# collabora/WhisperLive

Hardware: AMD Instinct MI355X
Metric: real-time factor (xRT), Whisper-small 30 s window (p50 chunk latency in p50_chunk_latency_ms) (higher is better)
Workload: dtype f16 (MFMA operands; f32 accumulate, f32 residual stream, f32 log-mel); 1 GPU; configs[1]: Whisper-small.en, 1 stream per GPU, one 30 s window per stream per step (480000 samples 16 kHz f32 resident in HBM -> log-mel -> encoder -> beam-5 decode, 64 generated tokens forced by suppressing EOT), seeded random weights; streams_per_gpu=1, beam_size=5, decode_steps=64

## Files before the change

include/wlx.h:

```cpp
#ifndef WLX_H
#define WLX_H

#include <stdint.h>

#ifdef __cplusplus
extern "C" {
#endif

#define WLX_ABI_VERSION 1

typedef enum {
    WLX_OK = 0,
    WLX_ERR_ARG = 1,
    WLX_ERR_HIP = 2,
    WLX_ERR_WEIGHT = 3,
    WLX_ERR_STATE = 4,
    WLX_ERR_NOMEM = 5
} wlx_status;

typedef struct {
    int32_t n_mels;
    int32_t d_model;
    int32_t n_heads;
    int32_t enc_layers;
// ... 66 lines not shown

int32_t wlx_generate(wlx_engine* e, int32_t slot, int32_t batch,
                     const int32_t* prompts, const int32_t* prompt_lens, int32_t prompt_stride,
                     const wlx_gen_opts* opts,
                     int32_t* tokens_out, int32_t tokens_stride ,
                     int32_t* n_tokens_out, float* scores_out, float* no_speech_prob_out);

int32_t wlx_generate_ex(wlx_engine* e, int32_t slot, int32_t batch, const int32_t* enc_items,
                        const int32_t* prompts, const int32_t* prompt_lens, int32_t prompt_stride,
                        const wlx_gen_opts* opts,
                        int32_t* tokens_out, int32_t tokens_stride,
                        int32_t* n_tokens_out, float* scores_out, float* no_speech_prob_out);

int32_t wlx_detect_language(wlx_engine* e, int32_t slot, int32_t batch, int32_t sot,
                            const int32_t* lang_ids, int32_t n_lang, float* probs_out);

int32_t wlx_timings_get(wlx_engine* e, int32_t slot, wlx_timings* out);
int32_t wlx_sync(wlx_engine* e, int32_t slot);

int32_t wlx_align(wlx_engine* e, int32_t slot, int32_t item, const int32_t* tokens, int32_t n_tokens, int32_t n_sot,
                  int32_t num_frames, int32_t median_filter_width, const int32_t* heads, int32_t n_heads, int32_t eot,
                  int32_t* text_indices, int32_t* time_indices, int32_t path_cap, int32_t* n_path_out,
                  float* text_token_probs);

typedef struct wlx_vad wlx_vad;
typedef struct {
    const float* stft_basis;
    const float* enc_w[4];
    const float* enc_b[4];
    const float* lstm_w_ih;
    const float* lstm_w_hh;
    const float* lstm_b_ih;
    const float* lstm_b_hh;
    const float* out_w;
    const float* out_b;
} wlx_vad_weights;
int32_t wlx_vad_create(const wlx_vad_weights* w, int32_t device, wlx_vad** out);
void    wlx_vad_destroy(wlx_vad* v);
int32_t wlx_vad_probs(wlx_vad* v, const float* pcm, int64_t n, float* probs_out, int32_t cap,
                      int32_t* n_windows_out, float* device_ms_out);

typedef struct wlx_ring wlx_ring;
int32_t wlx_ring_create(wlx_engine* e, int64_t capacity_samples , wlx_ring** out);
void    wlx_ring_destroy(wlx_ring* r);
int32_t wlx_ring_append(wlx_ring* r, const float* samples, int64_t n, int64_t max_resident, int64_t trim,
                        int64_t* dropped_out, int64_t* base_out, int64_t* resident_out);
int32_t wlx_ring_state(wlx_ring* r, int64_t* base_out, int64_t* resident_out);
int32_t wlx_vad_probs_resident(wlx_vad* v, wlx_ring* r, int64_t start, int64_t n, int32_t extra_zero_windows,
                               float* probs_out, int32_t cap, int32_t* n_windows_out, float* device_ms_out);
int32_t wlx_vad_segments(const float* probs, int32_t n_windows, int64_t n_samples, double thr, double neg, double min_speech,
                         double pad, double max_speech, double min_silence, double min_silence_at_max,
                         int64_t* start_end_out, int32_t cap, int32_t* n_out);
int32_t wlx_logmel_ring(wlx_engine* e, int32_t slot, int32_t item, wlx_ring* r, const int64_t* ranges, int32_t n_ranges,
                        int32_t* n_frames_out);

typedef struct {
    int32_t d_model, n_heads, enc_layers, dec_layers, ffn, vocab;
    int32_t max_positions;
    int32_t pad_id, eos_id, decoder_start_id;
    int32_t scale_embedding;
} wlx_mt_spec;
typedef struct wlx_mt wlx_mt;
typedef struct {
    int32_t num_beams;
    int32_t max_length;
    int32_t early_stopping;
    float   length_penalty;
    int32_t no_repeat_ngram_size;
    int32_t forced_eos_token_id;
} wlx_mt_gen_opts;
int32_t wlx_mt_create(const wlx_mt_spec* spec, const wlx_tensor* weights, int32_t n_weights, int32_t device, wlx_mt** out);
void    wlx_mt_destroy(wlx_mt* mt);
int32_t wlx_mt_slot_create(wlx_mt* mt, int32_t max_batch, int32_t max_rows_per_item, int32_t max_src, int32_t* slot_out);
int32_t wlx_mt_slot_destroy(wlx_mt* mt, int32_t slot);
int32_t wlx_mt_translate(wlx_mt* mt, int32_t slot, int32_t batch, const int32_t* src_ids, const int32_t* src_lens,
                         int32_t src_stride, const wlx_mt_gen_opts* opts, int32_t* tokens_out, int32_t tokens_stride,
                         int32_t* n_tokens_out, float* scores_out);

int32_t wlx_debug_logits_get(wlx_engine* e, int32_t slot, float* out, int32_t rows, int64_t cap_floats);
int32_t wlx_debug_decode_logits(wlx_engine* e, int32_t slot, const int32_t* tokens, int32_t n, float* out);
int32_t wlx_debug_search(wlx_engine* e, int32_t slot, const float* logits, int32_t steps,
                         const int32_t* prompt, int32_t prompt_len, const wlx_gen_opts* opts,
                         int32_t* tokens_out, int32_t tokens_stride, int32_t* n_tokens_out, float* scores_out);
int32_t wlx_debug_time_decode_step(wlx_engine* e, int32_t slot, int32_t rows, int32_t t, int32_t iters,
                                   float* avg_ms_out);

typedef struct {
    char name[64];
    float launches_per_step, avg_us, total_us_per_step;
    double bytes_per_launch;
} wlx_kernel_stat;
int32_t wlx_debug_trace_step(wlx_engine* e, int32_t slot, int32_t rows, int32_t t, int32_t with_search,
                             uint64_t* out, int64_t cap_u64, char* names, int32_t* n_launches_out);

int32_t wlx_debug_profile_step(wlx_engine* e, int32_t slot, int32_t rows, int32_t t, int32_t iters,
                               wlx_kernel_stat* out, int32_t cap, int32_t* n_out);

int32_t wlx_mt_debug_encode(wlx_mt* mt, int32_t slot, int32_t batch, const int32_t* src_ids, const int32_t* src_lens,
                            int32_t src_stride, float* out, int64_t cap_floats);
int32_t wlx_mt_debug_decode_logits(wlx_mt* mt, int32_t slot, const int32_t* src_ids, int32_t src_len, const int32_t* dec_tokens,
                                   int32_t n, float* out);
int32_t wlx_mt_debug_timings(wlx_mt* mt, int32_t slot, float* encode_ms, float* decode_ms, int32_t* steps);
int32_t wlx_mt_debug_attn(int32_t device, const uint16_t* q, int64_t ldq, int64_t q_rows, const uint16_t* k, int64_t ldk,
                          const uint16_t* v, int64_t ldv, int64_t kv_rows, const int32_t* groups, int32_t n_groups, int32_t max_nq,
                          int32_t heads, const int32_t* anc, int32_t ld_anc, int32_t tmax, uint16_t* o, int64_t ldo, int64_t o_rows);
int32_t wlx_mt_debug_topk(int32_t device, const float* logits, int32_t rows, int32_t vocab, const int32_t* ban, const int32_t* nban,
                          int32_t ban_ld, int32_t k, float* out_val, int32_t* out_idx);
int32_t wlx_mt_debug_embed(int32_t device, const float* E, int32_t vocab, int32_t d, const int32_t* tok, const int32_t* pos,
                           int32_t rows, float scale, const float* sinpos, int32_t n_pos, float* x);

int32_t wlx_debug_layernorm(int32_t device, const float* x, int64_t ldx, const float* gamma, const float* beta, int32_t M, int32_t d,
                            uint16_t* out16, float* out32, int64_t ldo);
int32_t wlx_debug_attn_encoder(int32_t device, const uint16_t* q, int64_t ldq, int64_t isq, const uint16_t* k, int64_t ldk, int64_t isk,
                               const uint16_t* vt, int64_t ldvt, int64_t isv, uint16_t* o, int64_t ldo, int64_t iso, int32_t T,
                               int32_t H, int32_t items);
typedef struct {
    int32_t zbatch, M, N, K, KT, conv3_cin, mode, force_form;
    int32_t d, rows_per_item;
    float qscale;
    int32_t reserved;
    int64_t lda, strideA, a_len;
    int64_t ldc, strideC, c_len;
    int64_t ldx, strideX, x_len;
    int64_t ldk, kv_item_stride_k, kv_layer_stride_k, k_len;
    int64_t ldvt, kv_item_stride_v, kv_layer_stride_v, v_len;
} wlx_debug_gemm_args;
int32_t wlx_debug_gemm(int32_t device, const wlx_debug_gemm_args* a, const uint16_t* A, const float* W, const float* bias,
                       const float* pos, uint16_t* C, float* X, uint16_t* kout, uint16_t* vt, int32_t* ran_out);
int32_t wlx_debug_dec_cross_attn(int32_t device, const uint16_t* q, int64_t ldq, const uint16_t* kp, const uint16_t* vp,
                                 int64_t item_stride, int32_t n_items, int32_t H, int32_t R, int32_t groups, int32_t rows,
                                 const int32_t* group_item, uint16_t* part_o, float* part_ml, uint16_t* out, int64_t ldo,
                                 int32_t align_item, int32_t align_head, float* align_out);
int32_t wlx_debug_dec_self_attn(int32_t device, const uint16_t* q, int64_t ldq, const uint16_t* kc, const uint16_t* vc,
                                int64_t cache_row_stride, int32_t cache_rows, int32_t d, int32_t H, int32_t rows, const int32_t* pos,
                                const int32_t* ancrow, const int16_t* anc, int32_t ident_ancestry, uint16_t* out, int64_t ldo);

#ifdef __cplusplus
}
#endif
#endif
```

whisperlive_amd/_lib.py:

```python
from __future__ import annotations

import ctypes as C
import os
import shutil
import subprocess
from pathlib import Path

import numpy as np

PKG_DIR = Path(__file__).resolve().parent
CSRC = PKG_DIR / "csrc"
DEFAULT_LIB = PKG_DIR / "libwlx.so"
LIB_PATH = Path(os.environ["WLX_LIB"]).resolve() if os.environ.get("WLX_LIB") else DEFAULT_LIB
SOURCES = ["pack.hip", "logmel.hip", "gemm.hip", "attention.hip", "decoder.hip", "search.hip", "host.hip", "engine.hip", "vad.hip", "mt.hip", "mt_engine.hip", "kernel_hooks.hip"]
EXPORTS = [
    "wlx_abi_version", "wlx_last_error", "wlx_engine_create", "wlx_engine_destroy", "wlx_engine_spec",
    "wlx_slot_create", "wlx_slot_destroy", "wlx_logmel", "wlx_pcm_put", "wlx_logmel_resident", "wlx_features_get", "wlx_features_set", "wlx_encode",
    "wlx_encoder_output_get", "wlx_generate", "wlx_generate_ex", "wlx_detect_language", "wlx_align", "wlx_timings_get", "wlx_sync",
    "wlx_vad_create", "wlx_vad_destroy", "wlx_vad_probs",
    "wlx_ring_create", "wlx_ring_destroy", "wlx_ring_append", "wlx_ring_state", "wlx_vad_probs_resident", "wlx_vad_segments", "wlx_logmel_ring",
    "wlx_mt_create", "wlx_mt_destroy", "wlx_mt_slot_create", "wlx_mt_slot_destroy", "wlx_mt_translate",
    "wlx_debug_logits_get", "wlx_debug_decode_logits", "wlx_debug_search", "wlx_debug_time_decode_step", "wlx_debug_profile_step", "wlx_debug_trace_step",
    "wlx_mt_debug_encode", "wlx_mt_debug_decode_logits", "wlx_mt_debug_timings", "wlx_mt_debug_attn", "wlx_mt_debug_topk",
    "wlx_mt_debug_embed",
    "wlx_debug_layernorm", "wlx_debug_attn_encoder", "wlx_debug_dec_cross_attn", "wlx_debug_dec_self_attn", "wlx_debug_gemm",
]


HIPCC_EXTRA = ["-mllvm", "-amdgpu-mfma-vgpr-form=1"]


class WlxError(RuntimeError):
    pass


class wlx_spec(C.Structure):
    _fields_ = [(n, C.c_int32) for n in
                ("n_mels", "d_model", "n_heads", "enc_layers", "dec_layers", "ffn", "vocab", "n_audio_ctx", "n_text_ctx")]


class wlx_tensor(C.Structure):
    _fields_ = [("name", C.c_char_p), ("data", C.c_void_p), ("ndim", C.c_int32), ("shape", C.c_int64 * 4),
                ("on_device", C.c_int32)]


class wlx_token_ids(C.Structure):
    _fields_ = [(n, C.c_int32) for n in ("sot", "eot", "no_timestamps", "timestamp_begin", "no_speech", "blank")]


class wlx_gen_opts(C.Structure):
    _fields_ = [
        ("beam_size", C.c_int32), ("patience", C.c_float), ("num_hypotheses", C.c_int32),
        ("length_penalty", C.c_float), ("repetition_penalty", C.c_float), ("no_repeat_ngram_size", C.c_int32),
        ("max_length", C.c_int32), ("suppress_blank", C.c_int32), ("suppress_tokens", C.POINTER(C.c_int32)),
        ("n_suppress_tokens", C.c_int32), ("max_initial_timestamp_index", C.c_int32), ("sampling_topk", C.c_int32),
        ("sampling_temperature", C.c_float), ("seed", C.c_uint64), ("ids", wlx_token_ids),
    ]


class wlx_timings(C.Structure):
    _fields_ = [("logmel_ms", C.c_float), ("encode_ms", C.c_float), ("generate_ms", C.c_float), ("decode_steps", C.c_int32)]


class wlx_kernel_stat(C.Structure):
    _fields_ = [("name", C.c_char * 64), ("launches_per_step", C.c_float), ("avg_us", C.c_float),
                ("total_us_per_step", C.c_float), ("bytes_per_launch", C.c_double)]


class wlx_vad_weights(C.Structure):
    _fields_ = [("stft_basis", C.POINTER(C.c_float)), ("enc_w", C.POINTER(C.c_float) * 4), ("enc_b", C.POINTER(C.c_float) * 4),
                ("lstm_w_ih", C.POINTER(C.c_float)), ("lstm_w_hh", C.POINTER(C.c_float)), ("lstm_b_ih", C.POINTER(C.c_float)),
                ("lstm_b_hh", C.POINTER(C.c_float)), ("out_w", C.POINTER(C.c_float)), ("out_b", C.POINTER(C.c_float))]


class wlx_mt_spec(C.Structure):
    _fields_ = [(n, C.c_int32) for n in ("d_model", "n_heads", "enc_layers", "dec_layers", "ffn", "vocab", "max_positions",
                                         "pad_id", "eos_id", "decoder_start_id", "scale_embedding")]


class wlx_debug_gemm_args(C.Structure):
    _fields_ = ([(n, C.c_int32) for n in ("zbatch", "M", "N", "K", "KT", "conv3_cin", "mode", "force_form", "d", "rows_per_item")] +
                [("qscale", C.c_float), ("reserved", C.c_int32)] +
                [(n, C.c_int64) for n in ("lda", "strideA", "a_len", "ldc", "strideC", "c_len", "ldx", "strideX", "x_len",
                                          "ldk", "kv_item_stride_k", "kv_layer_stride_k", "k_len",
                                          "ldvt", "kv_item_stride_v", "kv_layer_stride_v", "v_len")])


class wlx_mt_gen_opts(C.Structure):
    _fields_ = [("num_beams", C.c_int32), ("max_length", C.c_int32), ("early_stopping", C.c_int32),
                ("length_penalty", C.c_float), ("no_repeat_ngram_size", C.c_int32), ("forced_eos_token_id", C.c_int32)]


_extra_ok = None


def _hipcc() -> str:
    hipcc = shutil.which("hipcc") or "/opt/rocm/bin/hipcc"
    if not os.path.exists(hipcc):
        raise WlxError("hipcc not found: cannot build libwlx.so (ROCm toolchain required)")
    return hipcc


def _compile(out: Path, defines=(), verbose: bool = False, force: bool = False) -> Path:
    global _extra_ok
    from concurrent.futures import ThreadPoolExecutor
# ... 54 lines not shown
    deps = [CSRC / s for s in SOURCES] + list(CSRC.glob("*.h")) + [PKG_DIR.parent / "include" / "wlx.h"]
    return out.exists() and all(out.stat().st_mtime >= d.stat().st_mtime for d in deps)


def build_trace() -> Path:
    out = PKG_DIR / "libwlx_trace.so"
    return out if _fresh(out) else _compile(out, ["WLX_TRACE"])


def build_ab() -> Path:
    out = PKG_DIR / "libwlx_ab.so"
    return out if _fresh(out) else _compile(out, ["WLX_AB"])


def build_variant(name: str, defines) -> Path:
    out = PKG_DIR / name
    return out if _fresh(out) else _compile(out, list(defines))


def build(force: bool = False, verbose: bool = False) -> Path:
    if not force and _fresh(DEFAULT_LIB):
        return DEFAULT_LIB
    return _compile(DEFAULT_LIB, (), verbose, force=force)


_lib = None


def load() -> C.CDLL:
    global _lib
    if _lib is not None:
        return _lib
    if not LIB_PATH.exists():
        raise WlxError(f"{LIB_PATH} not built: run `python -c 'import __graft_entry__ as g; g.build()'` "
                       "(hipcc --offload-arch=gfx950). whisperlive_amd has no CPU fallback.")
    try:
        lib = C.CDLL(str(LIB_PATH))
    except OSError as e:
        raise WlxError(f"cannot load {LIB_PATH}: {e}") from e
    missing = [s for s in EXPORTS if not hasattr(lib, s)]
    if missing:
        raise WlxError(f"libwlx.so lacks symbols {missing}")
    i32, i64, f32p, i32p, vp = C.c_int32, C.c_int64, C.POINTER(C.c_float), C.POINTER(C.c_int32), C.c_void_p
    lib.wlx_abi_version.restype = i32
    lib.wlx_last_error.restype = C.c_char_p
    lib.wlx_engine_create.argtypes = [C.POINTER(wlx_spec), C.POINTER(wlx_tensor), i32, i32, C.POINTER(vp)]
    lib.wlx_engine_destroy.argtypes = [vp]
    lib.wlx_engine_destroy.restype = None
    lib.wlx_engine_spec.argtypes = [vp, C.POINTER(wlx_spec)]
    lib.wlx_slot_create.argtypes = [vp, i32, i32, i32p]
    lib.wlx_slot_destroy.argtypes = [vp, i32]
    lib.wlx_logmel.argtypes = [vp, i32, i32, f32p, i64, i32p]
    lib.wlx_pcm_put.argtypes = [vp, i32, i32, f32p, i64]
    lib.wlx_logmel_resident.argtypes = [vp, i32, i32, i32p]
    lib.wlx_features_get.argtypes = [vp, i32, i32, f32p, i64, i32p]
    lib.wlx_features_set.argtypes = [vp, i32, i32, f32p, i32, i32]
    lib.wlx_encode.argtypes = [vp, i32, i32, i32p, i32p]
    lib.wlx_encoder_output_get.argtypes = [vp, i32, i32, f32p, i64]
    lib.wlx_generate.argtypes = [vp, i32, i32, i32p, i32p, i32, C.POINTER(wlx_gen_opts), i32p, i32, i32p, f32p, f32p]
    lib.wlx_generate_ex.argtypes = [vp, i32, i32, i32p, i32p, i32p, i32, C.POINTER(wlx_gen_opts), i32p, i32, i32p, f32p, f32p]
    lib.wlx_detect_language.argtypes = [vp, i32, i32, i32, i32p, i32, f32p]
    lib.wlx_align.argtypes = [vp, i32, i32, i32p, i32, i32, i32, i32, i32p, i32, i32, i32p, i32p, i32, i32p, f32p]
    lib.wlx_timings_get.argtypes = [vp, i32, C.POINTER(wlx_timings)]
    lib.wlx_sync.argtypes = [vp, i32]
    lib.wlx_vad_create.argtypes = [C.POINTER(wlx_vad_weights), i32, C.POINTER(vp)]
    lib.wlx_vad_destroy.argtypes = [vp]
    lib.wlx_vad_destroy.restype = None
    lib.wlx_vad_probs.argtypes = [vp, f32p, i64, f32p, i32, i32p, f32p]
    i64p = C.POINTER(C.c_int64)
    lib.wlx_ring_create.argtypes = [vp, i64, C.POINTER(vp)]
    lib.wlx_ring_destroy.argtypes = [vp]
    lib.wlx_ring_destroy.restype = None
    lib.wlx_ring_append.argtypes = [vp, f32p, i64, i64, i64, i64p, i64p, i64p]
    lib.wlx_ring_state.argtypes = [vp, i64p, i64p]
    lib.wlx_vad_probs_resident.argtypes = [vp, vp, i64, i64, i32, f32p, i32, i32p, f32p]
    lib.wlx_vad_segments.argtypes = [f32p, i32, i64, C.c_double, C.c_double, C.c_double, C.c_double, C.c_double, C.c_double, C.c_double, i64p, i32, i32p]
    lib.wlx_logmel_ring.argtypes = [vp, i32, i32, vp, i64p, i32, i32p]
    lib.wlx_debug_logits_get.argtypes = [vp, i32, f32p, i32, i64]
    lib.wlx_debug_decode_logits.argtypes = [vp, i32, i32p, i32, f32p]
    lib.wlx_debug_search.argtypes = [vp, i32, f32p, i32, i32p, i32, C.POINTER(wlx_gen_opts), i32p, i32, i32p, f32p]
    lib.wlx_debug_time_decode_step.argtypes = [vp, i32, i32, i32, i32, f32p]
    lib.wlx_debug_profile_step.argtypes = [vp, i32, i32, i32, i32, C.POINTER(wlx_kernel_stat), i32, i32p]
    lib.wlx_debug_trace_step.argtypes = [vp, i32, i32, i32, i32, C.POINTER(C.c_uint64), i64, C.c_char_p, i32p]
    lib.wlx_mt_create.argtypes = [C.POINTER(wlx_mt_spec), C.POINTER(wlx_tensor), i32, i32, C.POINTER(vp)]
    lib.wlx_mt_destroy.argtypes = [vp]
    lib.wlx_mt_destroy.restype = None
    lib.wlx_mt_slot_create.argtypes = [vp, i32, i32, i32, i32p]
    lib.wlx_mt_slot_destroy.argtypes = [vp, i32]
    lib.wlx_mt_translate.argtypes = [vp, i32, i32, i32p, i32p, i32, C.POINTER(wlx_mt_gen_opts), i32p, i32, i32p, f32p]
    lib.wlx_mt_debug_encode.argtypes = [vp, i32, i32, i32p, i32p, i32, f32p, i64]
    lib.wlx_mt_debug_decode_logits.argtypes = [vp, i32, i32p, i32, i32p, i32, f32p]
    lib.wlx_mt_debug_timings.argtypes = [vp, i32, f32p, f32p, i32p]
    u16p = C.POINTER(C.c_uint16)
    lib.wlx_mt_debug_attn.argtypes = [i32, u16p, i64, i64, u16p, i64, u16p, i64, i64, i32p, i32, i32, i32, i32p, i32, i32, u16p, i64, i64]
    lib.wlx_mt_debug_topk.argtypes = [i32, f32p, i32, i32, i32p, i32p, i32, i32, f32p, i32p]
    lib.wlx_mt_debug_embed.argtypes = [i32, f32p, i32, i32, i32p, i32p, i32, C.c_float, f32p, i32, f32p]
    lib.wlx_debug_layernorm.argtypes = [i32, f32p, i64, f32p, f32p, i32, i32, u16p, f32p, i64]
    lib.wlx_debug_attn_encoder.argtypes = [i32, u16p, i64, i64, u16p, i64, i64, u16p, i64, i64, u16p, i64, i64, i32, i32, i32]
    lib.wlx_debug_dec_cross_attn.argtypes = [i32, u16p, i64, u16p, u16p, i64, i32, i32, i32, i32, i32, i32p, u16p, f32p, u16p, i64,
                                             i32, i32, f32p]
    lib.wlx_debug_dec_self_attn.argtypes = [i32, u16p, i64, u16p, u16p, i64, i32, i32, i32, i32, i32p, i32p, C.POINTER(C.c_int16), i32,
                                            u16p, i64]
    lib.wlx_debug_gemm.argtypes = [i32, C.POINTER(wlx_debug_gemm_args), u16p, f32p, f32p, f32p, u16p, f32p, u16p, u16p, i32p]
    for name in EXPORTS:
        fn = getattr(lib, name)
        if name not in ("wlx_last_error", "wlx_engine_destroy", "wlx_vad_destroy", "wlx_ring_destroy", "wlx_mt_destroy"):
            fn.restype = i32
    if lib.wlx_abi_version() != 1:
        raise WlxError("libwlx.so ABI version mismatch")
    _lib = lib
    return lib


def tensor_array(weights):
    keep = []
    arr = (wlx_tensor * len(weights))()
    for i, (name, t) in enumerate(weights.items()):
        on_dev = 0
        if hasattr(t, "data_ptr"):
            import torch
            t = t.detach().to(torch.float32).contiguous()
            on_dev = 1 if t.is_cuda else 0
            ptr, shape = t.data_ptr(), tuple(t.shape)
        else:
            t = np.ascontiguousarray(t, dtype=np.float32)
            ptr, shape = t.ctypes.data, t.shape
        keep.append(t)
        arr[i].name = name.encode()
        arr[i].data = ptr
        arr[i].ndim = len(shape)
        for j, s in enumerate(shape):
            arr[i].shape[j] = s
        arr[i].on_device = on_dev
    return arr, keep


def check(rc: int):
    if rc != 0:
        msg = load().wlx_last_error()
        raise WlxError(f"libwlx error {rc}: {msg.decode() if msg else '?'}")
```

whisperlive_amd/csrc/decoder.h:

```cpp
#pragma once
#include "kernels.h"

namespace wlx {

#define WLX_MAX_MT 4
#define WLX_MAX_DEC_ROWS 320
#define WLX_XSPLIT 8
#define WLX_MAX_CAND 32
#define WLX_MAX_HYP 32

struct RowTables {
    const int* token; const int* pos; const int* cache; const int* ancrow;
    const short* anc;
    int* intok;
};

void launch_dec_embed(const half_t* tok_emb, const float* pos_emb, int d, const RowTables& rt, int rows,
                      float* x, const int* done, hipStream_t s);

enum GemvIn : int { GEMV_IN_LN = 0, GEMV_IN_F16 = 1, GEMV_IN_XATTN = 2 };
enum GemvOut : int { GEMV_OUT_F16 = 0, GEMV_OUT_GELU_F16 = 1, GEMV_OUT_F32 = 2, GEMV_OUT_RESID = 3, GEMV_OUT_QKV = 4,
                     GEMV_OUT_SLAB = 5 };
enum GemvXsrc : int { GEMV_X_PLAIN = 0, GEMV_X_SLABS = 1, GEMV_X_EMBED = 2 };
#ifndef WLX_CQ_GB_LDS
#define WLX_CQ_GB_LDS 1
#endif
#ifndef WLX_CQ_SWAP
#define WLX_CQ_SWAP 1
#endif
#ifndef WLX_STAGE_WAVE
#define WLX_STAGE_WAVE 1
#endif
#ifndef WLX_XCOMB_WAVE
#define WLX_XCOMB_WAVE 1
#endif
#ifndef WLX_FC2_KS
#define WLX_FC2_KS 2
#endif

struct GemvParams {
    int in_mode, out_mode;
    int M;
    int Mtot;
    int chunk;
    int busy_device;
    int rt_nz, rt_tiles, rt_magic;
    int K, KT, N;
    int KTW;
    int NCH;
    int nwm;
    int xstage;
    const half_t* Wp; const float* bias;
    const float* X; long ldx; const float* gamma; const float* beta;
    const half_t* Xh; long ldxh;
    const half_t* part_o; const float* part_ml; int H; int R;
    half_t* Yh; long ldyh;
    float* Y; long ldy;
    float* Xres; long ldxres;
    int d; float qscale; half_t* Kc; half_t* Vc; long cache_row_stride;
    const int* row_cache; const int* row_pos;
    const int* done;
    int xsrc;
    float* slab; long slab_stride;
    int KTS;
    const half_t* tok_emb; const float* pos_emb; const int* emb_token; int* intok;
    WLX_TR_FIELD
};
#ifdef WLX_TRACE
extern unsigned long long* g_trace_buf;
extern int g_trace_seq;
extern const char* g_trace_names[512];
static inline WlxTrace trace_next(const char* name) {
    WlxTrace t{g_trace_buf, g_trace_seq};
    if (g_trace_seq < 512) g_trace_names[g_trace_seq] = name;
    ++g_trace_seq;
    return t;
}
#define WLX_TR_ARG(name) , trace_next(name)
#else
#define WLX_TR_ARG(name)
#endif
void launch_dec_gemv(const GemvParams& p, hipStream_t s);
const char* dec_gemv_kernel_name(const GemvParams& p);
extern bool g_decode_v1;
bool dec_gemv_is_lean(const GemvParams& p);
int dec_gemv_slab_split(int M, int K, int N);

void launch_dec_self_attn(const half_t* q, long ldq, const half_t* Kc, const half_t* Vc, long cache_row_stride,
                          int d, int H, const RowTables& rt, int rows, half_t* out, long ldo,
                          const int* done, bool ident_ancestry, hipStream_t s);
void launch_dec_cross_attn(const half_t* q, long ldq, const half_t* Kp, const half_t* Vp, long item_stride, int H, int R,
                           int groups, int rows, const int* group_item, half_t* part_o, float* part_ml, hipStream_t s);

bool dec_cq_cross_attn_eligible(int d, int H, int R);
void launch_dec_cq_cross_attn(const float* X, long ldx, const float* gamma, const float* beta, const half_t* Wp, const float* bias,
                              float qscale, int d, const half_t* Kp, const half_t* Vp, long item_stride, int H, int R, int groups,
                              int rows, const int* group_item, half_t* part_o, float* part_ml, hipStream_t s);
void launch_dec_xattn_combine(const half_t* part_o, const float* part_ml, int M, int H, int R, half_t* out, long ldo, hipStream_t s);
void launch_dec_align_scores(const half_t* q, long ldq, const half_t* Kp_item, int h, int rows, float* out, hipStream_t s);

struct SearchState {
    int* step;
    int* done;
    int* done_host;
    int* n_finished;
    int* item_done;
    int* plen;
    float* cum;
    int* row_done;
    float* cand_score; int* cand_tok;
    int* samp_tok; float* samp_lp;
    int* hyp_tokens;
    int* hyp_len;
    float* hyp_score;
    int* n_hyp;
    int* n_hyp_host;
    float* no_speech;
    int* nsp_row;
    int* token; int* pos; short* anc; int* intok;
    float* scan_stats;
    float* scan_cv; int* scan_ci;
    int* rule;
};
#define SC_THREADS 256
#define SC_NPT 8
#define SC_CHUNK (SC_THREADS * SC_NPT)
#define SC_MAXCH 27
#define SC_NSTAT 8
struct SearchParams {
    int V; long ldl;
    int items, R, rows;
    int sampling;
    int beam, ncand, max_cand_hyp , num_hyp;
    int allow_early_exit;
    float length_penalty, rep_penalty, temperature;
    int no_repeat_ngram, topk;
    int suppress_blank, apply_ts_rules, max_initial_ts;
    int sot, eot, no_timestamps, ts_begin, no_speech, blank;
    int max_length;
    unsigned long long seed;
    const unsigned* suppress_mask;
};
void launch_search_rows(const float* logits, const SearchParams* sp_dev, int rows, const SearchState& st, hipStream_t s);
void launch_search_update(const SearchParams* sp_dev, int items, const SearchState& st, hipStream_t s);
void launch_search_scan3(const float* logits, long ldl, int V, const SearchParams* sp_dev, int rows, const SearchState& st,
                         hipStream_t s);
void launch_search_merge_update3(const float* logits, long ldl, int V, const SearchParams* sp_dev, int items, int R,
                                 const SearchState& st, hipStream_t s);
void launch_search_reset(const SearchState& st, int items, int rows, hipStream_t s);
void launch_token_prob_rows(const float* logits, long ldl, int vlim, int rows, const int* toks, float* out, hipStream_t s);
void launch_token_prob(const float* logits, long ldl, int V, int rows, int tok, float* out, hipStream_t s);
void launch_lang_probs(const float* logits, long ldl, int rows, const int* ids, int n, float* probs, hipStream_t s);

}
```

whisperlive_amd/csrc/decoder.hip:

```cpp
#include "decoder.h"
#include <algorithm>
#include <cstdlib>
#include <cstdio>
#include <atomic>

namespace wlx {

__global__ __launch_bounds__(256) void dec_embed_kernel(const half_t* __restrict__ tok_emb,
                                                        const float* __restrict__ pos_emb, int d,
                                                        const int* __restrict__ token,
                                                        const int* __restrict__ pos,
                                                        const int* __restrict__ cache, int* __restrict__ intok,
                                                        float* __restrict__ x, const int* __restrict__ done WLX_TR_PARAM) {
    if (done && *done) return;
    WLX_TR_BEGIN();
    const int r = blockIdx.x;
    const int tok = token[r], p = pos[r];
    if (threadIdx.x == 0) intok[(long)cache[r] * WLX_T_TEXT + p] = tok;
    const half_t* te = tok_emb + (long)tok * d;
    const float* pe = pos_emb + (long)p * d;
    for (int i = threadIdx.x * 4; i < d; i += 256 * 4) {
        f16x4 t = ld_f16x4(te + i);
        float4 pv = *reinterpret_cast<const float4*>(pe + i);
        *reinterpret_cast<float4*>(x + (long)r * d + i) =
// ... 1151 lines not shown
}
static bool gemv2_ok(const GemvParams& p, Gemv2Cfg* out) {
    const Gemv2Cfg c = gemv2_cfg(p);
    if (!c.ok) return false;
    if (p.in_mode == GEMV_IN_LN && p.xsrc != GEMV_X_PLAIN) {
        const bool pair = (c.CH == 4 && c.LNV == 3) || (c.CH == 3 && c.LNV == 3) || (c.CH == 2 && c.LNV == 2) || (c.CH == 4 && c.LNV == 4) || (c.CH == 5 && c.LNV == 5) ||
                          (c.MT == 1 && ((c.CH == 6 && c.LNV == 3) || (c.CH == 8 && c.LNV == 4) || (c.CH == 10 && c.LNV == 5))) ||
                          (c.CH == 2 && c.LNV == 15 && c.MT == 1);
        if (!pair) return false;
    } else if (p.in_mode == GEMV_IN_LN) {
        const bool pair = (c.CH == 6 && c.LNV == 3) || (c.CH == 5 && c.LNV == 5) || (c.CH == 4 && c.LNV == 2) || (c.CH == 4 && c.LNV == 4) ||
                          (c.CH == 10 && c.LNV == 5 && c.MT == 1) || (c.CH == 8 && c.LNV == 4 && c.MT == 1) ||
                          (c.CH == 2 && c.LNV == 15 && c.MT == 1);
        if (!pair) return false;
    }
    if (out) *out = c;
    return true;
}
static GemvParams gemv_chunked(const GemvParams& p) {
    static const bool rt_on = [] { const char* e = wlx_ab("WLX_ROWTILE"); return !(e && e[0] == '0'); }();
    constexpr int rt_max = WLX_MAX_DEC_ROWS;
    static const int rt_chunk_env = [] { const char* e = wlx_ab("WLX_ROWTILE_CHUNK"); const int v = e ? atoi(e) : 0; return (v == 16 || v == 32 || v == 48) ? v : 0; }();
    int rt_chunk = 16;
    if (p.in_mode == GEMV_IN_F16 && p.out_mode == GEMV_OUT_RESID && p.xsrc == GEMV_X_PLAIN && !p.busy_device && p.M > 64) {
        static const int n_cu = [] { int dev = 0, n = 256; (void)hipGetDevice(&dev); hipDeviceProp_t pr; if (hipGetDeviceProperties(&pr, dev) == hipSuccess && pr.multiProcessorCount > 0) n = pr.multiProcessorCount; return n; }();
        const int tiles = (p.N + 15) / 16;
        double best = 1e300;
        for (int mt = 1; mt <= 3; ++mt) {
            const long wgs = (long)tiles * ((p.M + 16 * mt - 1) / (16 * mt));
            const double cost = (double)((wgs + n_cu - 1) / n_cu) * (1.0 + 0.35 * (mt - 1));
            if (cost < best - 1e-9) { best = cost; rt_chunk = 16 * mt; }
        }
    }
    if (rt_chunk_env) rt_chunk = rt_chunk_env;
    GemvParams q = p;
    if (p.Mtot != 0 || p.in_mode == GEMV_IN_XATTN) return q;
    const bool ln_wide4 = rt_chunk == 16 && p.M > 32 && p.in_mode == GEMV_IN_LN && p.xsrc == GEMV_X_PLAIN && (p.out_mode == GEMV_OUT_QKV || p.out_mode == GEMV_OUT_GELU_F16) &&
                          (p.N & 15) == 0 && ((p.N >> 4) & 3) == 0;
    const bool rt_shape = p.N <= 1536 || (long)p.N * p.K <= 3200000L || ln_wide4;
    if (rt_on && !g_decode_v1 && p.M > rt_chunk && p.M <= rt_max && rt_shape) { q.Mtot = p.M; q.M = rt_chunk; q.chunk = rt_chunk; q.rt_nz = (p.M + rt_chunk - 1) / rt_chunk; }
    else if (p.M > 48 && p.xsrc != GEMV_X_EMBED) { q.Mtot = p.M; q.M = 48; q.chunk = 48; }
    return q;
}
static bool vocab2_ok(const GemvParams& p);
bool dec_gemv_is_lean(const GemvParams& p) { return vocab2_ok(p) || gemv2_ok(gemv_chunked(p), nullptr); }

int dec_gemv_slab_split(int M, int K, int N) {
    if (WLX_FC2_KS < 2) return 0;
    if (g_decode_v1 || M < 1 || K % 32 || (K / 32) % WLX_FC2_KS || K < 2048) return 0;
    GemvParams p0{};
    p0.in_mode = GEMV_IN_F16; p0.out_mode = GEMV_OUT_SLAB; p0.M = M; p0.K = K; p0.KT = K / 32; p0.N = N; p0.KTS = p0.KT / WLX_FC2_KS;
    static const float dummy_bias = 0.f;
    p0.bias = &dummy_bias;
    const GemvParams p = gemv_chunked(p0);
    Gemv2Cfg c;
    if (!gemv2_ok(p, &c) || (p.M <= 16 && !c.xstage)) return 0;
    return WLX_FC2_KS;
}

static bool vocab2_ok(const GemvParams& p);
static int vocab2_chunk_rows(int K);
const char* dec_gemv_kernel_name(const GemvParams& p_any) {
    static thread_local char buf[64];
    if (vocab2_ok(p_any)) {
        snprintf(buf, sizeof(buf), "dec_vocab_kernel<%d, %d, %d>", p_any.KT, p_any.KT == 24 ? 6 : p_any.KT == 40 ? 5 : p_any.KT == 12 ? 3 : 4, (std::min(p_any.M, vocab2_chunk_rows(p_any.K)) + 15) / 16);
        return buf;
    }
    const GemvParams p = gemv_chunked(p_any);
    const int MT = (p.M + 15) / 16;
    Gemv2Cfg c2;
    if (gemv2_ok(p, &c2)) {
        snprintf(buf, sizeof(buf), "dec_gemv2_kernel<%d, %d, %d, %d, %d, %d, %d>", c2.CH, c2.LNV ? c2.LNV : 1, p.in_mode, p.out_mode, c2.NTB, c2.MT, p.xsrc);
        return buf;
    }
    snprintf(buf, sizeof(buf), "dec_gemv_kernel<%d, %d, %d>", MT > 4 ? 4 : MT, MT == 1 ? 2 : 1, p.in_mode);
    return buf;
}

struct VocabParams {
    const float* X; long ldx; const float* gamma; const float* beta;
    const half_t* Wp; int M, N, NT;
    float* Y; long ldy;
    const float* slab; long slab_stride;
    WLX_TR_FIELD
};
template <int KT, int KC, int MT, bool SLABS>
__global__ __launch_bounds__(512) void dec_vocab_kernel(VocabParams p) {
    static_assert(!SLABS || MT == 1, "slab rows: decode steps of one row tile");
    constexpr int K = KT * 32, LNV = (K + 255) / 256, NC = KT / KC, LDXS = K + 8;
    constexpr bool LNT = (K % 256) != 0;
    static_assert((K % 256 == 0 || K == 384) && KT % KC == 0 && NC % 2 == 0, "d_model a multiple of 256 (or 384); an even number of K chunks");
    constexpr int RPT = (MT == 1) ? 2 : 4;
    constexpr int NTRIP = (MT * 16 + 8 * RPT - 1) / (8 * RPT);
    extern __shared__ __attribute__((aligned(16))) half_t vxs[];
    const int tid = threadIdx.x, lane = tid & 63, c = lane & 15, g = lane >> 4;
    const int wave = __builtin_amdgcn_readfirstlane(tid >> 6);
    WLX_TR_BEGIN();
    const int pair = blockIdx.x * 8 + wave;
    const int t0 = (2 * pair < p.NT) ? 2 * pair : p.NT - 1, t1 = (2 * pair + 1 < p.NT) ? 2 * pair + 1 : p.NT - 1;
    const bool tail_on = !LNT || lane < 32;
    const int tback = LNT ? (tail_on ? 0 : lane) : 0;
    float4 x[RPT][LNV];
#pragma unroll
    for (int i = 0; i < RPT; ++i) {
        const int r = (wave + 8 * i < p.M) ? wave + 8 * i : p.M - 1;
        const float4* x4 = reinterpret_cast<const float4*>(p.X + (long)r * p.ldx) + lane;
#pragma unroll
        for (int j = 0; j < LNV; ++j) x[i][j] = x4[64 * j - ((j == LNV - 1) ? tback : 0)];
    }
    float4 xsl[SLABS ? WLX_FC2_KS : 1][RPT][LNV];
    if constexpr (SLABS) {
#pragma unroll
        for (int q = 0; q < WLX_FC2_KS; ++q)
#pragma unroll
            for (int i = 0; i < RPT; ++i) {
                const int r = (wave + 8 * i < p.M) ? wave + 8 * i : p.M - 1;
                const float4* s4 = reinterpret_cast<const float4*>(p.slab + q * p.slab_stride + (long)r * p.ldx) + lane;
#pragma unroll
                for (int j = 0; j < LNV; ++j) xsl[q][i][j] = s4[64 * j - ((j == LNV - 1) ? tback : 0)];
            }
    }
    float4 gq[LNV], bq[LNV];
    {
        const float4* g4 = reinterpret_cast<const float4*>(p.gamma) + lane;
        const float4* b4 = reinterpret_cast<const float4*>(p.beta) + lane;
#pragma unroll
        for (int j = 0; j < LNV; ++j) { const int tb = (j == LNV - 1) ? tback : 0; gq[j] = g4[64 * j - tb]; bq[j] = b4[64 * j - tb]; }
    }
    asm volatile("" ::: "memory");
    const half_t* wq[2] = {p.Wp + (long)t0 * KT * 512 + lane * 8, p.Wp + (long)t1 * KT * 512 + lane * 8};
    f16x8 wf[2][KC][2];
#pragma unroll
    for (int b = 0; b < 2; ++b)
#pragma unroll
        for (int j = 0; j < KC; ++j)
#pragma unroll
            for (int i = 0; i < 2; ++i) wf[b][j][i] = ld_nt_f16x8(wq[i] + (b * KC + j) * 512);
    constexpr float invK = 1.0f / (float)K;
    auto ln_row = [&](float4 (&xr)[LNV], int r, bool keep) {
        if constexpr (LNT) { if (!tail_on) xr[LNV - 1] = make_float4(0.f, 0.f, 0.f, 0.f); }
        float sm = 0.f;
#pragma unroll
        for (int j = 0; j < LNV; ++j) sm += (xr[j].x + xr[j].y) + (xr[j].z + xr[j].w);
        const float mean = dpp_wave_sum(sm) * invK;
        float q = 0.f;
#pragma unroll
        for (int j = 0; j < LNV; ++j) {
            xr[j].x -= mean; xr[j].y -= mean; xr[j].z -= mean; xr[j].w -= mean;
            if constexpr (LNT) { if (j == LNV - 1 && !tail_on) xr[j] = make_float4(0.f, 0.f, 0.f, 0.f); }
            q += (xr[j].x * xr[j].x + xr[j].y * xr[j].y) + (xr[j].z * xr[j].z + xr[j].w * xr[j].w);
        }
        const float rstd = rsqrtf(dpp_wave_sum(q) * invK + 1e-5f);
        half_t* dst = vxs + (long)r * LDXS + lane * 4;
#pragma unroll
        for (int j = 0; j < LNV; ++j) {
            const f16x4 hv = {(half_t)(xr[j].x * rstd * gq[j].x + bq[j].x), (half_t)(xr[j].y * rstd * gq[j].y + bq[j].y),
                              (half_t)(xr[j].z * rstd * gq[j].z + bq[j].z), (half_t)(xr[j].w * rstd * gq[j].w + bq[j].w)};
            if (keep && (j < LNV - 1 || tail_on)) *reinterpret_cast<f16x4*>(dst + 256 * j) = hv;
        }
    };
    if constexpr (SLABS) {
#pragma unroll
        for (int q = 0; q < WLX_FC2_KS; ++q)
#pragma unroll
            for (int i = 0; i < RPT; ++i)
#pragma unroll
                for (int j = 0; j < LNV; ++j) { x[i][j].x += xsl[q][i][j].x; x[i][j].y += xsl[q][i][j].y; x[i][j].z += xsl[q][i][j].z; x[i][j].w += xsl[q][i][j].w; }
    }
#pragma unroll
    for (int i = 0; i < RPT; ++i) ln_row(x[i], (wave + 8 * i < p.M) ? wave + 8 * i : p.M - 1, wave + 8 * i < p.M);
#pragma unroll 1
    for (int tr = 1; tr < NTRIP; ++tr) {
        const int rb = wave + 8 * RPT * tr;
        if (rb >= p.M) break;
        float4 y[RPT][LNV];
#pragma unroll
        for (int i = 0; i < RPT; ++i) {
            const int r = (rb + 8 * i < p.M) ? rb + 8 * i : p.M - 1;
            const float4* x4 = reinterpret_cast<const float4*>(p.X + (long)r * p.ldx) + lane;
#pragma unroll
            for (int j = 0; j < LNV; ++j) y[i][j] = x4[64 * j - ((j == LNV - 1) ? tback : 0)];
        }
#pragma unroll
        for (int i = 0; i < RPT; ++i) ln_row(y[i], (rb + 8 * i < p.M) ? rb + 8 * i : p.M - 1, rb + 8 * i < p.M);
    }
    WLX_TR_MARK(1);
    __syncthreads();
    const half_t* xr[MT];
#pragma unroll
    for (int mt = 0; mt < MT; ++mt) xr[mt] = vxs + (long)((mt * 16 + c < p.M) ? mt * 16 + c : p.M - 1) * LDXS + g * 8;
    f32x4 acc[2][MT];
#pragma unroll
    for (int i = 0; i < 2; ++i)
#pragma unroll
        for (int mt = 0; mt < MT; ++mt) acc[i][mt] = (f32x4){0.f, 0.f, 0.f, 0.f};
#pragma unroll
    for (int ch = 0; ch < NC; ++ch) {
#pragma unroll
        for (int j = 0; j < KC; ++j) {
            f16x8 xf[MT];
#pragma unroll
            for (int mt = 0; mt < MT; ++mt) xf[mt] = *reinterpret_cast<const f16x8*>(xr[mt] + (ch * KC + j) * 32);
#pragma unroll
            for (int i = 0; i < 2; ++i)
#pragma unroll
                for (int mt = 0; mt < MT; ++mt) acc[i][mt] = mfma16(wf[ch & 1][j][i], xf[mt], acc[i][mt]);
        }
        if (ch + 2 < NC) {
#pragma unroll
            for (int j = 0; j < KC; ++j)
#pragma unroll
                for (int i = 0; i < 2; ++i) wf[ch & 1][j][i] = ld_nt_f16x8(wq[i] + ((ch + 2) * KC + j) * 512);
        }
    }
    WLX_TR_MARK(2);
#pragma unroll
    for (int i = 0; i < 2; ++i) {
        const int nt = 2 * pair + i;
        if (nt >= p.NT) continue;
        const int n = nt * 16 + g * 4;
#pragma unroll
        for (int mt = 0; mt < MT; ++mt) {
            const int row = mt * 16 + c;
            if (row >= p.M) continue;
            float* yp = p.Y + (long)row * p.ldy + n;
            const f32x4 v = acc[i][mt];
            if (n + 3 < p.N) *reinterpret_cast<float4*>(yp) = make_float4(v[0], v[1], v[2], v[3]);
            else { if (n < p.N) yp[0] = v[0]; if (n + 1 < p.N) yp[1] = v[1]; if (n + 2 < p.N) yp[2] = v[2]; }
        }
    }
    WLX_TR_END(p.trc);
}

template <int KT, int KC, int MT, bool SLABS = false>
static void vocab_go(const VocabParams& p, hipStream_t s) {
    const size_t shm = (size_t)p.M * (KT * 32 + 8) * sizeof(half_t);
    if (shm > 64 * 1024) {
        static std::atomic<signed char> granted[64] = {};
        int dev = 0;
        (void)hipGetDevice(&dev);
        if (dev >= 0 && dev < 64 && granted[dev].load(std::memory_order_acquire) == 0) {
            if (hipFuncSetAttribute(reinterpret_cast<const void*>(&dec_vocab_kernel<KT, KC, MT, SLABS>), hipFuncAttributeMaxDynamicSharedMemorySize,
                                    WLX_G2_LDS_MAX) == hipSuccess) granted[dev].store(1, std::memory_order_release);
            else {
                (void)hipGetLastError();
                g_lds_optin_refused.store(true);
                fprintf(stderr, "[wlx] device %d refused %d KiB of dynamic LDS: the batched vocabulary projection falls back to the general kernel\n", dev, WLX_G2_LDS_MAX / 1024);
            }
        }
    }
    const int pairs = (p.NT + 1) / 2;
    hipLaunchKernelGGL((dec_vocab_kernel<KT, KC, MT, SLABS>), dim3((pairs + 7) / 8), dim3(512), shm, s, p);
}
template <int KT, int KC>
static void vocab_go_mt(const VocabParams& p, hipStream_t s) {
    if (p.slab) { vocab_go<KT, KC, 1, true>(p, s); return; }
    switch ((p.M + 15) / 16) {
        case 1: vocab_go<KT, KC, 1>(p, s); break;
        case 2: vocab_go<KT, KC, 2>(p, s); break;
        case 3: vocab_go<KT, KC, 3>(p, s); break;
        default: vocab_go<KT, KC, 4>(p, s); break;
    }
}
static int vocab2_chunk_rows(int K) {
    int r = 64;
    while (r > 16 && (size_t)r * (K + 8) * sizeof(half_t) > WLX_G2_LDS_MAX) r -= 16;
    return r;
}
static bool vocab2_ok(const GemvParams& p) {
    if (g_decode_v1 || p.in_mode != GEMV_IN_LN || p.out_mode != GEMV_OUT_F32 || p.bias || p.Mtot != 0) return false;
    if (p.xsrc != GEMV_X_PLAIN && !(p.xsrc == GEMV_X_SLABS && p.M <= 16 && p.slab != nullptr)) return false;
    if (p.M < 1 || p.M > WLX_MAX_DEC_ROWS || p.K != p.KT * 32 || p.N < 256) return false;
    if (!(p.KT == 12 || p.KT == 16 || p.KT == 24 || p.KT == 32 || p.KT == 40)) return false;
    const int rows = std::min(p.M, vocab2_chunk_rows(p.K));
    const size_t shm = (size_t)rows * (p.K + 8) * sizeof(half_t);
    if (shm > 64 * 1024 && g_lds_optin_refused.load(std::memory_order_relaxed)) return false;
    return shm <= WLX_G2_LDS_MAX;
}
static void vocab2_launch(const GemvParams& g, hipStream_t s) {
    const int CH = vocab2_chunk_rows(g.K);
    for (int r0 = 0; r0 < g.M; r0 += CH) {
        VocabParams p{};
        p.X = g.X + (long)r0 * g.ldx; p.ldx = g.ldx; p.gamma = g.gamma; p.beta = g.beta; p.Wp = g.Wp; p.M = std::min(CH, g.M - r0); p.N = g.N; p.NT = (g.N + 15) / 16;
        p.Y = g.Y + (long)r0 * g.ldy; p.ldy = g.ldy;
        if (g.xsrc == GEMV_X_SLABS) { p.slab = g.slab; p.slab_stride = g.slab_stride; }
#ifdef WLX_TRACE
        p.trc = trace_next("vocab2");
#endif
        switch (g.KT) {
            case 12: vocab_go_mt<12, 3>(p, s); break;
            case 16: vocab_go_mt<16, 4>(p, s); break;
            case 24: vocab_go_mt<24, 6>(p, s); break;
            case 32: vocab_go_mt<32, 4>(p, s); break;
            default: vocab_go_mt<40, 5>(p, s); break;
        }
    }
}

template <int MT, int NTB>
static void gemv_dispatch_in(const GemvParams& p, dim3 grid, dim3 block, size_t shm, hipStream_t s) {
    switch (p.in_mode) {
        case GEMV_IN_LN: hipLaunchKernelGGL((dec_gemv_kernel<MT, NTB, GEMV_IN_LN>), grid, block, shm, s, p); break;
        case GEMV_IN_F16: hipLaunchKernelGGL((dec_gemv_kernel<MT, NTB, GEMV_IN_F16>), grid, block, shm, s, p); break;
        default: hipLaunchKernelGGL((dec_gemv_kernel<MT, NTB, GEMV_IN_XATTN>), grid, block, shm, s, p); break;
    }
}

void launch_dec_gemv(const GemvParams& p_any, hipStream_t s) {
    if (vocab2_ok(p_any)) { vocab2_launch(p_any, s); return; }
    Gemv2Cfg c2;
    const GemvParams pc = gemv_chunked(p_any);
    if (gemv2_ok(pc, &c2) && gemv2_launch(pc, c2, s)) return;
    if (p_any.M > 16 * WLX_MAX_MT) {
        const int CHK = (p_any.in_mode == GEMV_IN_XATTN && p_any.R > 0) ? (16 * WLX_MAX_MT / p_any.R) * p_any.R : 16 * WLX_MAX_MT;
        for (int r0 = 0; r0 < p_any.M; r0 += CHK) {
            GemvParams q = p_any;
            q.M = std::min(CHK, p_any.M - r0);
            if (q.X) q.X += (long)r0 * q.ldx;
            if (q.Xh) q.Xh += (long)r0 * q.ldxh;
            if (q.Yh) q.Yh += (long)r0 * q.ldyh;
            if (q.Y) q.Y += (long)r0 * q.ldy;
            if (q.Xres) q.Xres += (long)r0 * q.ldxres;
            if (q.row_cache) q.row_cache += r0;
            if (q.row_pos) q.row_pos += r0;
            if (q.in_mode == GEMV_IN_XATTN) {
                const int items0 = r0 / q.R;
                q.part_o += (long)items0 * q.H * WLX_XSPLIT * 16 * 64;
                q.part_ml += (long)items0 * q.H * 16 * WLX_XSPLIT * 2;
            }
            launch_dec_gemv(q, s);
        }
        return;
    }
    const GemvParams& p0 = p_any;
    const GemvParams& p = p0;
    const int MT = (p.M + 15) / 16;
    const int NT_total = (p.N + 15) / 16;
    int nw = (p.KT + GV_CH - 1) / GV_CH;
    if (nw < 1) nw = 1;
    if (nw > 8) nw = 8;
    const int NTB = (MT == 1) ? 2 : 1;
    dim3 grid((NT_total + NTB - 1) / NTB), block(nw * 64);
    const size_t shm = sizeof(float) * ((size_t)2 * nw * MT * 16 + (size_t)nw * NTB * MT * 256);
    switch (MT) {
        case 1: gemv_dispatch_in<1, 2>(p, grid, block, shm, s); break;
        case 2: gemv_dispatch_in<2, 1>(p, grid, block, shm, s); break;
        case 3: gemv_dispatch_in<3, 1>(p, grid, block, shm, s); break;
        default: gemv_dispatch_in<4, 1>(p, grid, block, shm, s); break;
    }
}

#define SA_PF_NW 4
#ifndef SA_NW
#define SA_NW 8
#endif
template <bool IDENT, int NW>
__global__ __launch_bounds__(64 * NW) void dec_self_attn2_kernel(const half_t* __restrict__ q, long ldq,
                                                                    const half_t* __restrict__ Kc,
                                                                    const half_t* __restrict__ Vc, long crs, int d,
                                                                    const int* __restrict__ pos,
                                                                    const int* __restrict__ ancrow,
                                                                    const short* __restrict__ anc,
                                                                    half_t* __restrict__ out, long ldo WLX_TR_PARAM) {
    __shared__ int crow_s[NW][64];
    __shared__ float part_s[NW][8][64];
    __shared__ float ml_s[NW][2];
    const int lane = threadIdx.x & 63;
    const int w = __builtin_amdgcn_readfirstlane(threadIdx.x >> 6);
// ... 507 lines not shown
```

whisperlive_amd/csrc/engine.h:

```cpp
#pragma once
#include <hip/hip_runtime.h>
#include <map>
#include <mutex>
#include <string>
#include <vector>
#include "../../include/wlx.h"
#include "decoder.h"
#include "host.h"

namespace wlx {

struct StepGraphKey {
    int rows, R, groups;
    bool operator<(const StepGraphKey& o) const {
        if (rows != o.rows) return rows < o.rows;
        if (R != o.R) return R < o.R;
        return groups < o.groups;
    }
};

struct ProfRec { std::string name; double bytes; };
struct Prof { std::vector<ProfRec> recs; bool list_only = true; std::string only; int t = 0; };

struct Slot {
    std::mutex call_mu;
    int B = 0, R = 0, rows_cap = 0, cache_rows = 0, groups_cap = 0;
    hipStream_t stream = nullptr;
    bool dedicated_queue = false;
    int device_of = -1;
    bool counted = false;
    unsigned promote_epoch = 0;
    hipEvent_t ev0 = nullptr, ev1 = nullptr;
    hipEvent_t ev_lm0 = nullptr, ev_lm1 = nullptr;
    hipEvent_t ev_en0 = nullptr, ev_en1 = nullptr;
    bool en_pending = false;
    bool lm_pending = false;
    bool gen_pending = false;
    std::vector<int> lm_items;
    bool busy_variant = false;
    std::vector<void*> allocs, host_allocs;
    float* pcm = nullptr; size_t pcm_cap = 0;
    float* feats = nullptr; long feat_ld = 0;
    std::vector<int> nframes;
    std::vector<int64_t> npcm;
    unsigned* gmax = nullptr;
    long long* d_rng = nullptr;
    half_t *featT = nullptr, *h1 = nullptr, *ln = nullptr, *q = nullptr, *k = nullptr, *vt = nullptr,
           *attn = nullptr, *h2 = nullptr, *enc16 = nullptr;
    float *x = nullptr, *enc32 = nullptr;
    long featT_stride = 0, h1_stride = 0;
    half_t *ck = nullptr, *cvt = nullptr;
    int enc_batch = 0;
    half_t *kc = nullptr, *vc = nullptr;
    float* xd = nullptr; half_t *qd = nullptr, *attnd = nullptr, *hd = nullptr;
    float* slab = nullptr;
    half_t* part_o = nullptr;
    float *part_ml = nullptr, *logits = nullptr;
    long ldl = 0;
    int *d_token = nullptr, *d_pos = nullptr, *d_cache = nullptr, *d_ancrow = nullptr, *d_group_item = nullptr;
    struct DecBufs {
        float* xd; half_t *qd, *attnd, *hd; float* slab; int slab_rows; half_t* part_o; float* part_ml;
        int *d_token, *d_pos, *d_cache, *d_ancrow, *d_group_item;
    };
    DecBufs pf{};
    bool pf_one_pass = false;
    bool pf_ok = false;
    short* d_anc = nullptr; int* d_intok = nullptr;
    bool anc_ident = false;
    SearchState st{};
    SearchParams* d_sp = nullptr;
    unsigned* d_suppress = nullptr;
    int* d_lang_ids = nullptr; float* d_probs = nullptr; float* d_tokprob = nullptr;
    int* h_stage = nullptr; size_t h_stage_ints = 0;
    unsigned char* h_gen = nullptr; size_t h_gen_bytes = 0;
    int* h_pf = nullptr; bool h_pf_used = false;
    int* h_hyp = nullptr;
    int max_items = 0;
    std::vector<int> last_suppress; bool suppress_valid = false;
    std::map<StepGraphKey, hipGraphExec_t> graphs;
    wlx_timings tm{};
    Prof* prof = nullptr;
    struct AlignCapture { float* scores; const int32_t* heads; int n_heads, n_tok, row0, item; }* align = nullptr;
    float* align_scores = nullptr; size_t align_cap = 0;
    int* d_align_tgt = nullptr; float* d_align_prob = nullptr;
};

struct Ring {
    std::mutex mu;
    int device = 0;
    float* buf = nullptr; size_t cap = 0;
    int64_t base = 0, resident = 0;
    hipStream_t stream = nullptr;
    hipEvent_t last_read = nullptr; bool read_pending = false; hipStream_t last_read_stream = nullptr;
};

struct Engine {
    wlx_spec spec{};
    int device = 0;
    int H = 0;
    std::vector<void*> allocs;
    LogmelConsts lm{};
    half_t *conv1_w = nullptr, *conv2_w = nullptr;
    float *conv1_b = nullptr, *conv2_b = nullptr, *enc_pos = nullptr, *enc_ln_g = nullptr, *enc_ln_b = nullptr;
    int conv1_KT = 0;
    std::vector<LayerW> enc;
    half_t* Wckv = nullptr; float* bckv = nullptr;
    half_t *tok_emb16 = nullptr, *Wvocab = nullptr;
    float *dec_pos = nullptr, *dec_ln_g = nullptr, *dec_ln_b = nullptr;
    std::vector<LayerW> dec;
    std::mutex mu;
    std::vector<Slot*> slots;
    bool use_graph = true;
};

}

struct wlx_engine : public wlx::Engine {};
struct wlx_ring : public wlx::Ring {};
```

whisperlive_amd/csrc/engine.hip:

```cpp
#include "engine.h"
#include <sched.h>
#include <atomic>
#include <limits>
#include <algorithm>
#include <cmath>
#include <cstdio>
#include <cstdlib>
#include <cstring>
#include <chrono>
#include <thread>

using namespace wlx;

static inline void cpu_relax() {
#if defined(__x86_64__) || defined(__i386__)
    __builtin_ia32_pause();
#elif defined(__aarch64__)
    asm volatile("yield" ::: "memory");
#else
    asm volatile("" ::: "memory");
#endif
}
extern "C" int32_t wlx_abi_version(void) { return WLX_ABI_VERSION; }

static void build_mel_filters(int n_mels, std::vector<float>& w, std::vector<int>& range) {
    const int nb = 201;
    std::vector<double> fft(nb), melf(n_mels + 2);
    for (int i = 0; i < nb; ++i) fft[i] = (double)i * 8000.0 / 200.0;
    const double max_mel = 45.245640471924965, f_sp = 200.0 / 3.0, min_log_hz = 1000.0;
    const double min_log_mel = min_log_hz / f_sp, logstep = std::log(6.4) / 27.0;
    const double step = max_mel / (double)(n_mels + 1);
    for (int i = 0; i < n_mels + 2; ++i) {
        double m = (i == n_mels + 1) ? max_mel : (double)i * step;
        melf[i] = (m >= min_log_mel) ? min_log_hz * std::exp(logstep * (m - min_log_mel)) : f_sp * m;
    }
    w.assign((size_t)n_mels * nb, 0.f);
    range.assign((size_t)n_mels * 2, 0);
    for (int i = 0; i < n_mels; ++i) {
        const double fd0 = melf[i + 1] - melf[i], fd1 = melf[i + 2] - melf[i + 1];
        const double enorm = 2.0 / (melf[i + 2] - melf[i]);
        int lo = nb, hi = 0;
        for (int b = 0; b < nb; ++b) {
            const double lower = -(melf[i] - fft[b]) / fd0, upper = (melf[i + 2] - fft[b]) / fd1;
            const double v = std::max(0.0, std::min(lower, upper));
            const float f = (float)((double)(float)v * enorm);
            w[(size_t)i * nb + b] = f;
            if (f != 0.f) { lo = std::min(lo, b); hi = std::max(hi, b + 1); }
        }
        if (lo >= hi) { lo = 0; hi = 0; }
        range[2 * i] = lo; range[2 * i + 1] = hi;
    }
}

static int build_logmel_consts(Engine* e) {
    std::vector<float> win(400), tw(800), filt;
    std::vector<int> range;
    const double PI2 = 6.283185307179586476925286766559;
    for (int i = 0; i < 400; ++i) {
        win[i] = (float)(0.5 - 0.5 * std::cos(PI2 * (double)i / 400.0));
        tw[2 * i] = (float)std::cos(PI2 * (double)i / 400.0);
        tw[2 * i + 1] = (float)std::sin(PI2 * (double)i / 400.0);
    }
    build_mel_filters(e->spec.n_mels, filt, range);
    float *dwin, *dtw, *dfilt; int* drange;
    CKR(dalloc(e->allocs, &dwin, 400, true)); CKR(dalloc(e->allocs, &dtw, 800, true));
    CKR(dalloc(e->allocs, &dfilt, filt.size(), true)); CKR(dalloc(e->allocs, &drange, range.size(), true));
    CKR(upload_sync(dwin, win.data(), 400 * 4));
    CKR(upload_sync(dtw, tw.data(), 800 * 4));
    CKR(upload_sync(dfilt, filt.data(), filt.size() * 4));
    CKR(upload_sync(drange, range.data(), range.size() * 4));
    e->lm.window = dwin; e->lm.twiddle = dtw; e->lm.filters = dfilt; e->lm.frange = drange;
    return WLX_OK;
}

static int engine_load(Engine* e, const wlx_tensor* weights, int n_weights) {
    const wlx_spec& sp = e->spec;
    const int d = sp.d_model, F = sp.ffn, V = sp.vocab;
    std::vector<void*>& A = e->allocs;
    Weights ws;
    CKR(ws.open(weights, n_weights));
    CKR(build_logmel_consts(e));
    const wlx_tensor* t; const float* src;
    auto conv = [&](const char* name, int cin, half_t** W, int* KT) -> int {
        CKR(ws.need(name, {d, cin, 3}, &t));
        CKR(alloc_packed(A, d, 3 * cin, W, KT, true));
        CKR(ws.device_f32(t, &src));
        launch_pack_conv3(src, d, cin, *W, *KT, ws.st);
        return WLX_OK;
    };
    auto positions = [&](const char* name, int rows, float** out) -> int {
        CKR(ws.need(name, {rows, d}, &t));
        CKR(dalloc(A, out, (size_t)rows * d, true));
        CKR(ws.device_f32(t, &src));
        CK(hipMemcpyAsync(*out, src, (size_t)rows * d * 4, hipMemcpyDeviceToDevice, ws.st));
        return WLX_OK;
    };
    int KT;
    CKR(conv("model.encoder.conv1.weight", sp.n_mels, &e->conv1_w, &e->conv1_KT));
    CKR(conv("model.encoder.conv2.weight", d, &e->conv2_w, &KT));
    CKR(ws.alloc_vec(A, "model.encoder.conv1.bias", d, &e->conv1_b, true));
    CKR(ws.alloc_vec(A, "model.encoder.conv2.bias", d, &e->conv2_b, true));
    CKR(positions("model.encoder.embed_positions.weight", sp.n_audio_ctx, &e->enc_pos));
    LayerOpts o{false, 1.f, true};
    e->enc.resize(sp.enc_layers);
    for (int l = 0; l < sp.enc_layers; ++l)
        CKR(load_layer(ws, A, "model.encoder.layers." + std::to_string(l) + ".", d, F, o, e->enc[l]));
    CKR(ws.alloc_vec(A, "model.encoder.layer_norm.weight", d, &e->enc_ln_g, true));
    CKR(ws.alloc_vec(A, "model.encoder.layer_norm.bias", d, &e->enc_ln_b, true));
    CKR(ws.need("model.decoder.embed_tokens.weight", {V, d}, &t));
    CKR(dalloc(A, &e->tok_emb16, (size_t)V * d, true));
    CKR(ws.device_f32(t, &src));
    launch_f32_to_f16(src, e->tok_emb16, (long)V * d, ws.st);
    CKR(alloc_packed(A, V, d, &e->Wvocab, &KT, true));
    launch_pack_linear(src, V, d, d, e->Wvocab, KT, 0, ws.st);
    CKR(positions("model.decoder.embed_positions.weight", sp.n_text_ctx, &e->dec_pos));
    CKR(alloc_packed(A, (int64_t)sp.dec_layers * 2 * d, d, &e->Wckv, nullptr, true));
    CKR(dalloc(A, &e->bckv, (size_t)sp.dec_layers * 2 * d, true));
    o.Wckv = e->Wckv; o.bckv = e->bckv;
    e->dec.resize(sp.dec_layers);
    for (o.l = 0; o.l < sp.dec_layers; ++o.l)
        CKR(load_layer(ws, A, "model.decoder.layers." + std::to_string(o.l) + ".", d, F, o, e->dec[o.l]));
    CKR(ws.alloc_vec(A, "model.decoder.layer_norm.weight", d, &e->dec_ln_g, true));
    CKR(ws.alloc_vec(A, "model.decoder.layer_norm.bias", d, &e->dec_ln_b, true));
    return ws.finish();
}

static std::atomic<bool> g_embedded_device_memory{false};
extern "C" int32_t wlx_engine_create(const wlx_spec* spec, const wlx_tensor* weights, int32_t n_weights,
                                     int32_t device, wlx_engine** out) {
    if (!spec || !weights || !out) return set_error(WLX_ERR_ARG, "null argument");
    if (spec->d_model % 64 || spec->d_model / 64 != spec->n_heads)
        return set_error(WLX_ERR_ARG, "d_model must be 64*n_heads");
    if (spec->d_model % 128 || spec->d_model > 1536) return set_error(WLX_ERR_ARG, "d_model must be a multiple of 128, <= 1536");
    if (spec->ffn % 128) return set_error(WLX_ERR_ARG, "ffn must be a multiple of 128");
    if (spec->n_mels != 80 && spec->n_mels != 128) return set_error(WLX_ERR_ARG, "n_mels must be 80 or 128");
    if (spec->n_audio_ctx != WLX_T_AUDIO || spec->n_text_ctx != WLX_T_TEXT)
        return set_error(WLX_ERR_ARG, "n_audio_ctx/n_text_ctx must be 1500/448");
    if (spec->vocab > 1024 * 52) return set_error(WLX_ERR_ARG, "vocab too large");
    int ndev = 0;
    CK(hipGetDeviceCount(&ndev));
    if (device < 0 || device >= ndev) return set_error(WLX_ERR_ARG, "device %d out of range (%d)", device, ndev);
    CK(hipSetDevice(device));
    if (int pe = gemm_prepare_device()) return set_error(WLX_ERR_HIP, "GEMM kernel set-up failed on device %d (hip error %d)", device, pe);
    wlx_engine* e = new wlx_engine();
    e->spec = *spec;
    e->device = device;
    e->H = spec->n_heads;
    for (int i = 0; i < n_weights; ++i)
        if (weights[i].on_device) { g_embedded_device_memory.store(true); break; }
    const char* ng = getenv("WLX_NO_GRAPH");
    e->use_graph = !(ng && ng[0] == '1');
    const char* v1 = wlx_ab("WLX_DECODE_V1");
    g_decode_v1 = (v1 && v1[0] == '1');
    int rc = engine_load(e, weights, n_weights);
    if (rc != WLX_OK) {
        for (void* p : e->allocs) (void)hipFree(p);
        delete e;
        return rc;
    }
    *out = e;
    return WLX_OK;
}

static int max_dedicated_queues() {
    static const int v = [] { const char* e = getenv("WLX_DEDICATED_QUEUES"); return e ? atoi(e) : 4; }();
    return v;
}
static std::atomic<int> g_dedicated_live[64];
static std::atomic<int> g_slots_live[64];
static std::atomic<bool> g_demote[64];
static std::atomic<unsigned> g_promote_epoch[64];
static void slot_free(Slot* s) {
    if (!s) return;
    if (s->device_of >= 0 && s->device_of < 64) {
        if (s->dedicated_queue) g_dedicated_live[s->device_of].fetch_sub(1);
        if (s->counted && g_slots_live[s->device_of].fetch_sub(1) - 1 <= max_dedicated_queues()) {
            if (g_demote[s->device_of].exchange(false)) g_promote_epoch[s->device_of].fetch_add(1);
        }
    }
    if (s->align_scores) (void)hipFree(s->align_scores);
    for (auto& kv : s->graphs) (void)hipGraphExecDestroy(kv.second);
    for (void* p : s->allocs) (void)hipFree(p);
    for (void* p : s->host_allocs) (void)hipHostFree(p);
    if (s->ev0) (void)hipEventDestroy(s->ev0);
    if (s->ev1) (void)hipEventDestroy(s->ev1);
    if (s->ev_lm0) (void)hipEventDestroy(s->ev_lm0);
    if (s->ev_lm1) (void)hipEventDestroy(s->ev_lm1);
    if (s->ev_en0) (void)hipEventDestroy(s->ev_en0);
    if (s->ev_en1) (void)hipEventDestroy(s->ev_en1);
    if (s->stream) (void)hipStreamDestroy(s->stream);
    delete s;
}

extern "C" void wlx_engine_destroy(wlx_engine* e) {
    if (!e) return;
    (void)hipSetDevice(e->device);
    (void)hipDeviceSynchronize();
    for (Slot* s : e->slots) slot_free(s);
    for (void* p : e->allocs) (void)hipFree(p);
    delete e;
}

extern "C" int32_t wlx_engine_spec(const wlx_engine* e, wlx_spec* out) {
    if (!e || !out) return set_error(WLX_ERR_ARG, "null argument");
    *out = e->spec;
    return WLX_OK;
}

struct SlotGuard {
    Slot* s = nullptr;
    ~SlotGuard() { if (s) s->call_mu.unlock(); }
};
static int create_slot_stream(int device, hipStream_t* out, bool* dedicated_out);
static bool dedicated_streams_possible();
static int slot_acquire(wlx_engine* e, int slot, SlotGuard& g) {
    if (!e) return set_error(WLX_ERR_ARG, "null engine");
    Slot* s = nullptr;
    {
        std::lock_guard<std::mutex> lk(e->mu);
        if (slot < 0 || slot >= (int)e->slots.size() || !e->slots[slot]) return set_error(WLX_ERR_ARG, "bad slot %d", slot);
        s = e->slots[slot];
        if (!s->call_mu.try_lock())
            return set_error(WLX_ERR_STATE, "slot %d is busy in another call (a slot serves one call at a time)", slot);
        g.s = s;
    }
    const int dv = s->device_of;
    if (dv < 0 || dv >= 64) return WLX_OK;
    if (s->dedicated_queue && (g_demote[dv].load() || !dedicated_streams_possible())) {
        hipStream_t ns = nullptr;
        if (hipSetDevice(dv) == hipSuccess && hipStreamSynchronize(s->stream) == hipSuccess &&
            hipStreamCreateWithFlags(&ns, hipStreamNonBlocking) == hipSuccess) {
            (void)hipStreamDestroy(s->stream);
            s->stream = ns;
            s->dedicated_queue = false;
            g_dedicated_live[dv].fetch_sub(1);
        } else {
// ... 131 lines not shown
            CKR(create_slot_stream(e->device, &s->stream, &s->dedicated_queue));
        }
        CK(hipEventCreate(&s->ev0)); CK(hipEventCreate(&s->ev1));
        CK(hipEventCreate(&s->ev_lm0)); CK(hipEventCreate(&s->ev_lm1));
        CK(hipEventCreate(&s->ev_en0)); CK(hipEventCreate(&s->ev_en1));
        CKR(slot_grow_audio(e, s, 480000));
        CKR(dalloc(s->allocs, &s->gmax, (size_t)B, true));
        CKR(dalloc(s->allocs, &s->d_rng, (size_t)2 * WLX_LM_MAXRANGES, true));
        s->featT_stride = (long)(WLX_N_FRAMES + 2) * sp.n_mels + 64;
        s->h1_stride = (long)(WLX_N_FRAMES + 2) * d;
        CKR(dalloc(s->allocs, &s->featT, (size_t)B * s->featT_stride, true));
        CKR(dalloc(s->allocs, &s->h1, (size_t)B * s->h1_stride, true));
        const size_t TB = (size_t)B * WLX_T_AUDIO;
        CKR(dalloc(s->allocs, &s->x, TB * d, true));
        CKR(dalloc(s->allocs, &s->ln, TB * d, true));
        CKR(dalloc(s->allocs, &s->q, TB * d, true));
        CKR(dalloc(s->allocs, &s->k, (size_t)B * WLX_T_AUDIO_PAD * d, true));
        CKR(dalloc(s->allocs, &s->vt, (size_t)B * d * WLX_T_AUDIO_PAD, true));
        CKR(dalloc(s->allocs, &s->attn, TB * d, true));
        CKR(dalloc(s->allocs, &s->h2, TB * F, true));
        CKR(dalloc(s->allocs, &s->enc16, TB * d, true));
        CKR(dalloc(s->allocs, &s->enc32, TB * d, true));
        CKR(dalloc(s->allocs, &s->ck, (size_t)L * B * WLX_T_AUDIO_PAD * d, true));
        CKR(dalloc(s->allocs, &s->cvt, (size_t)L * B * d * WLX_T_AUDIO_PAD, true));
        CKR(dalloc(s->allocs, &s->kc, (size_t)L * s->cache_rows * WLX_T_TEXT * d, true));
        CKR(dalloc(s->allocs, &s->vc, (size_t)L * s->cache_rows * WLX_T_TEXT * d, true));
        const int RC = s->rows_cap;
        CKR(dalloc(s->allocs, &s->xd, (size_t)RC * d, true));
        CKR(dalloc(s->allocs, &s->qd, (size_t)RC * d, true));
        CKR(dalloc(s->allocs, &s->attnd, (size_t)RC * d, true));
        CKR(dalloc(s->allocs, &s->hd, (size_t)RC * F, true));
        CKR(dalloc(s->allocs, &s->slab, (size_t)WLX_FC2_KS * RC * d, true));
        CKR(dalloc(s->allocs, &s->part_o, (size_t)s->groups_cap * e->H * WLX_XSPLIT * 16 * 64, true));
        CKR(dalloc(s->allocs, &s->part_ml, (size_t)s->groups_cap * e->H * WLX_XSPLIT * 16 * 2, true));
        {
            const size_t PR = WLX_T_TEXT, PG = (WLX_T_TEXT + 15) / 16;
            Slot::DecBufs& b = s->pf;
            b.slab_rows = (int)PR;
            CKR(dalloc(s->allocs, &b.xd, PR * d, true)); CKR(dalloc(s->allocs, &b.qd, PR * d, true)); CKR(dalloc(s->allocs, &b.attnd, PR * d, true));
            CKR(dalloc(s->allocs, &b.hd, PR * F, true)); CKR(dalloc(s->allocs, &b.slab, (size_t)WLX_FC2_KS * PR * d, true));
            CKR(dalloc(s->allocs, &b.part_o, PG * e->H * WLX_XSPLIT * 16 * 64, true));
            CKR(dalloc(s->allocs, &b.part_ml, PG * e->H * WLX_XSPLIT * 16 * 2, true));
            CKR(dalloc(s->allocs, &b.d_token, PR, true)); CKR(dalloc(s->allocs, &b.d_pos, PR, true)); CKR(dalloc(s->allocs, &b.d_cache, PR, true));
            CKR(dalloc(s->allocs, &b.d_ancrow, PR, true)); CKR(dalloc(s->allocs, &b.d_group_item, PG, true));
            GemvParams q{};
            static const float dummy_bias = 0.f;
            q.M = 96; q.bias = &dummy_bias; q.xsrc = GEMV_X_PLAIN;
            auto lean = [&](int in, int out, int N, int K) { q.in_mode = in; q.out_mode = out; q.N = N; q.K = K; q.KT = K / 32; return dec_gemv_is_lean(q); };
            s->pf_ok = lean(GEMV_IN_LN, GEMV_OUT_QKV, 3 * d, d) && lean(GEMV_IN_F16, GEMV_OUT_RESID, d, d) && lean(GEMV_IN_LN, GEMV_OUT_F16, d, d) &&
                       lean(GEMV_IN_LN, GEMV_OUT_GELU_F16, F, d) && lean(GEMV_IN_F16, GEMV_OUT_RESID, d, F);
        }
        s->ldl = ((sp.vocab + 15) / 16) * 16;
        CKR(dalloc(s->allocs, &s->logits, (size_t)RC * s->ldl, true));
        CKR(dalloc(s->allocs, &s->d_token, (size_t)RC, true));
        CKR(dalloc(s->allocs, &s->d_pos, (size_t)RC, true));
        CKR(dalloc(s->allocs, &s->d_cache, (size_t)RC, true));
        CKR(dalloc(s->allocs, &s->d_ancrow, (size_t)RC, true));
        CKR(dalloc(s->allocs, &s->d_group_item, (size_t)RC, true));
        const int CR = std::max(s->cache_rows, RC);
        CKR(dalloc(s->allocs, &s->d_anc, (size_t)CR * WLX_T_TEXT, true));
        CKR(dalloc(s->allocs, &s->d_intok, (size_t)CR * WLX_T_TEXT, true));
        SearchState& st = s->st;
        CKR(dalloc(s->allocs, &st.step, 1, true)); CKR(dalloc(s->allocs, &st.done, 1, true)); CKR(dalloc(s->allocs, &st.n_finished, 1, true));
        CKR(dalloc(s->allocs, &st.item_done, (size_t)B, true)); CKR(dalloc(s->allocs, &st.plen, (size_t)B, true));
        CKR(dalloc(s->allocs, &st.cum, (size_t)RC, true)); CKR(dalloc(s->allocs, &st.row_done, (size_t)RC, true));
        CKR(dalloc(s->allocs, &st.cand_score, (size_t)RC * WLX_MAX_CAND, true));
        CKR(dalloc(s->allocs, &st.cand_tok, (size_t)RC * WLX_MAX_CAND, true));
        CKR(dalloc(s->allocs, &st.samp_tok, (size_t)RC, true)); CKR(dalloc(s->allocs, &st.samp_lp, (size_t)RC, true));
        {
            const size_t ints = (size_t)B * (2 + 2 * WLX_MAX_HYP + (size_t)WLX_MAX_HYP * WLX_T_TEXT);
            CKR(halloc(s->host_allocs, &s->h_hyp, ints));
            memset(s->h_hyp, 0, ints * sizeof(int));
            s->max_items = B;
            CKR(halloc(s->host_allocs, &s->h_pf, (size_t)(5 * WLX_T_TEXT + 64)));
            st.n_hyp_host = s->h_hyp;
            st.hyp_len = st.n_hyp_host + B;
            st.hyp_score = reinterpret_cast<float*>(st.hyp_len + (size_t)B * WLX_MAX_HYP);
            st.no_speech = st.hyp_score + (size_t)B * WLX_MAX_HYP;
            st.hyp_tokens = reinterpret_cast<int*>(st.no_speech + B);
        }
        CKR(dalloc(s->allocs, &st.n_hyp, (size_t)B, true));
        CKR(dalloc(s->allocs, &st.nsp_row, (size_t)RC, true));
        st.token = s->d_token; st.pos = s->d_pos; st.anc = s->d_anc; st.intok = s->d_intok;
        CKR(dalloc(s->allocs, &st.scan_stats, (size_t)RC * SC_MAXCH * SC_NSTAT, true));
        CKR(dalloc(s->allocs, &st.scan_cv, (size_t)RC * (SC_MAXCH + 1) * WLX_MAX_CAND, true));
        CKR(dalloc(s->allocs, &st.scan_ci, (size_t)RC * (SC_MAXCH + 1) * WLX_MAX_CAND, true));
        CKR(dalloc(s->allocs, &st.rule, (size_t)RC * 4, true));
        CKR(dalloc(s->allocs, &s->d_align_tgt, (size_t)WLX_T_TEXT, true));
        CKR(dalloc(s->allocs, &s->d_align_prob, (size_t)WLX_T_TEXT, true));
        CKR(dalloc(s->allocs, &s->d_sp, 1, true));
        CKR(dalloc(s->allocs, &s->d_suppress, (size_t)(1024 * 52 / 32), true));
        CKR(dalloc(s->allocs, &s->d_lang_ids, 256, true));
        CKR(dalloc(s->allocs, &s->d_probs, (size_t)B * 256, true));
        CKR(dalloc(s->allocs, &s->d_tokprob, (size_t)RC, true));
        s->h_stage_ints = 1 << 16;
        CKR(halloc(s->host_allocs, &s->h_stage, s->h_stage_ints));
        s->st.done_host = s->h_stage + (s->h_stage_ints - 4);
        s->h_gen_bytes = 4096 + (size_t)RC * (4 + 16 + 4) + (size_t)B * 4 + (size_t)RC * WLX_T_TEXT * 2 + 256 + ((size_t)RC * 4 + B) * 4 + 128 +
                         (size_t)B * (4 + WLX_MAX_HYP * 8 + 4) + 64 + (size_t)B * WLX_MAX_HYP * WLX_T_TEXT * 4;
        CKR(halloc(s->host_allocs, &s->h_gen, s->h_gen_bytes));
        CK(hipStreamSynchronize(s->stream));
        return WLX_OK;
    }();
    if (rc != WLX_OK) { slot_free(s); return rc; }
    std::lock_guard<std::mutex> g(e->mu);
    e->slots.push_back(s);
    const int id = (int)e->slots.size() - 1;
    *slot_out = id;
    return WLX_OK;
}

extern "C" int32_t wlx_slot_destroy(wlx_engine* e, int32_t slot) {
    if (!e) return set_error(WLX_ERR_ARG, "null engine");
    Slot* s = nullptr;
    for (;;) {
        {
            std::lock_guard<std::mutex> g(e->mu);
            if (slot < 0 || slot >= (int)e->slots.size() || !e->slots[slot]) return set_error(WLX_ERR_ARG, "bad slot %d", slot);
            if (e->slots[slot]->call_mu.try_lock()) {
                s = e->slots[slot];
                e->slots[slot] = nullptr;
                break;
            }
        }
        std::this_thread::sleep_for(std::chrono::milliseconds(1));
    }
    s->call_mu.unlock();
    (void)hipSetDevice(e->device);
    (void)hipStreamSynchronize(s->stream);
    slot_free(s);
    return WLX_OK;
}

static int flush_logmel(Engine* e, Slot* s) {
    if (s->lm_items.empty()) return WLX_OK;
    CK(hipSetDevice(e->device));
    CK(hipEventRecord(s->ev_lm0, s->stream));
    for (size_t i0 = 0; i0 < s->lm_items.size(); i0 += WLX_LM_MAXB) {
        LogmelBatch lb{};
        for (size_t i = i0; i < s->lm_items.size() && i < i0 + WLX_LM_MAXB; ++i) {
            const int item = s->lm_items[i], k = lb.n_items++;
            const int64_t n = s->npcm[item];
            lb.pcm[k] = s->pcm + (size_t)item * s->pcm_cap; lb.n[k] = (long)n;
            lb.feats[k] = s->feats + (size_t)item * e->spec.n_mels * s->feat_ld; lb.T[k] = (int)((n + 160) / 160);
            lb.gmax[k] = s->gmax + item;
        }
        launch_logmel_batch(lb, e->spec.n_mels, e->lm, s->feat_ld, s->stream);
    }
    s->lm_items.clear();
    CK(hipGetLastError());
    CK(hipEventRecord(s->ev_lm1, s->stream));
    s->lm_pending = true;
    return WLX_OK;
}

extern "C" int32_t wlx_sync(wlx_engine* e, int32_t slot) {
    SlotGuard sg_;
    CKR(slot_acquire(e, slot, sg_));
    Slot* s = sg_.s;
    CK(hipSetDevice(e->device));
    CKR(flush_logmel(e, s));
    CK(hipStreamSynchronize(s->stream));
    return WLX_OK;
}

extern "C" int32_t wlx_timings_get(wlx_engine* e, int32_t slot, wlx_timings* out) {
// ... 289 lines not shown
    launch_layernorm_f16_f32(s->x, d, e->enc_ln_g, e->enc_ln_b, s->enc16, s->enc32, d, M, d, st);
    g = GemmParams{};
    g.A = s->enc16; g.lda = d; g.Wp = e->Wckv; g.KT = d / 32; g.M = M; g.N = sp.dec_layers * 2 * d; g.mode = GEMM_CROSS_KV;
    g.bias = e->bckv; g.d = d; g.Kout = s->ck; g.ldk = d; g.Vt = s->cvt; g.ldvt = WLX_T_AUDIO_PAD; g.rows_per_item = T;
    g.kv_item_stride_k = (long)WLX_T_AUDIO_PAD * d; g.kv_item_stride_v = (long)d * WLX_T_AUDIO_PAD;
    g.kv_layer_stride_k = (long)s->B * WLX_T_AUDIO_PAD * d; g.kv_layer_stride_v = (long)s->B * d * WLX_T_AUDIO_PAD;
    launch_gemm(g, 1, st);
    CK(hipGetLastError());
    CK(hipEventRecord(s->ev_en1, st));
    s->en_pending = true;
    s->enc_batch = batch;
    return WLX_OK;
}

extern "C" int32_t wlx_encoder_output_get(wlx_engine* e, int32_t slot, int32_t item, float* out, int64_t cap_floats) {
    SlotGuard sg_;
    CKR(slot_acquire(e, slot, sg_));
    Slot* s = sg_.s;
    if (item < 0 || item >= s->enc_batch) return set_error(WLX_ERR_STATE, "item %d not encoded", item);
    const size_t n = (size_t)WLX_T_AUDIO * e->spec.d_model;
    if (!out || (int64_t)n > cap_floats) return set_error(WLX_ERR_ARG, "output buffer too small");
    CK(hipSetDevice(e->device));
    CK(hipMemcpyAsync(out, s->enc32 + (size_t)item * n, n * 4, hipMemcpyDeviceToHost, s->stream));
    CK(hipStreamSynchronize(s->stream));
    return WLX_OK;
}

template <class F>
static inline void plaunch(Slot* s, const char* name, double bytes, F&& f) {
    if (!s->prof) { f(); return; }
    if (s->prof->list_only) { s->prof->recs.push_back(ProfRec{name, bytes}); return; }
    if (s->prof->only == name) f();
}
static double gemv_bytes(const GemvParams& p) { return 2.0 * (double)p.N * (double)p.K + (p.bias ? 4.0 * p.N : 0.0); }
static bool device_is_busy(const Slot* s) {
    return s->device_of >= 0 && s->device_of < 64 && g_slots_live[s->device_of].load(std::memory_order_relaxed) >= 3;
}
static void pgemv(Slot* s, const GemvParams& p0) {
    GemvParams p = p0;
    p.busy_device = s->busy_variant ? 1 : 0;
    if (!s->prof) { launch_dec_gemv(p, s->stream); return; }
    const std::string nm = dec_gemv_kernel_name(p);
    plaunch(s, nm.c_str(), gemv_bytes(p), [&] { launch_dec_gemv(p, s->stream); });
}

static void decoder_pass(Engine* e, Slot* s_, int rows, int R, int groups, bool with_logits, bool check_done, const Slot::DecBufs* alt = nullptr) {
    const wlx_spec& sp = e->spec;
    const int d = sp.d_model, F = sp.ffn, H = e->H;
    struct View {
        Slot* base; float* xd; half_t *qd, *attnd, *hd; float* slab; long slab_rows; half_t* part_o; float* part_ml;
        int *d_token, *d_pos, *d_cache, *d_ancrow, *d_group_item;
        Slot* operator->() const { return base; }
    } s{s_, alt ? alt->xd : s_->xd, alt ? alt->qd : s_->qd, alt ? alt->attnd : s_->attnd, alt ? alt->hd : s_->hd,
        alt ? alt->slab : s_->slab, alt ? (long)alt->slab_rows : (long)s_->rows_cap, alt ? alt->part_o : s_->part_o, alt ? alt->part_ml : s_->part_ml,
        alt ? alt->d_token : s_->d_token, alt ? alt->d_pos : s_->d_pos, alt ? alt->d_cache : s_->d_cache,
        alt ? alt->d_ancrow : s_->d_ancrow, alt ? alt->d_group_item : s_->d_group_item};
    hipStream_t st = s->stream;
    const int* done = (check_done && g_decode_v1) ? s->st.done : nullptr;
    RowTables rt{s.d_token, s.d_pos, s.d_cache, s.d_ancrow, s->d_anc, s->d_intok};
    const long crs = (long)WLX_T_TEXT * d;
    auto qkv_params = [&](int l, int xsrc) {
        const LayerW& w = e->dec[l];
        GemvParams p{};
        p.in_mode = GEMV_IN_LN; p.out_mode = GEMV_OUT_QKV; p.M = rows; p.K = d; p.KT = d / 32; p.N = 3 * d;
        p.Wp = w.Wqkv; p.bias = w.bqkv; p.X = s.xd; p.ldx = d; p.gamma = w.ln1_g; p.beta = w.ln1_b;
        p.Yh = s.qd; p.ldyh = d; p.d = d; p.qscale = 0.125f;
        p.Kc = s->kc + (size_t)l * s->cache_rows * crs; p.Vc = s->vc + (size_t)l * s->cache_rows * crs; p.cache_row_stride = crs;
        p.row_cache = s.d_cache; p.row_pos = s.d_pos; p.done = done;
        p.xsrc = xsrc; p.slab = s.slab; p.slab_stride = s.slab_rows * d;
        if (xsrc == GEMV_X_EMBED) {
            p.tok_emb = e->tok_emb16; p.pos_emb = e->dec_pos; p.emb_token = s.d_token; p.intok = s->d_intok;
            p.Xres = s.xd; p.ldxres = d;
        }
        return p;
    };
    auto oproj_params = [&](int l, int xsrc) {
        const LayerW& w = e->dec[l];
        GemvParams p{};
        p.in_mode = GEMV_IN_F16; p.out_mode = GEMV_OUT_RESID; p.M = rows; p.K = d; p.KT = d / 32; p.N = d;
        p.Wp = w.Wo; p.bias = w.bo; p.Xh = s.attnd; p.ldxh = d; p.Xres = s.xd; p.ldxres = d; p.qscale = 1.f; p.done = done;
        p.xsrc = xsrc; p.slab = s.slab; p.slab_stride = s.slab_rows * d;
        return p;
    };
    auto vocab_params = [&](int xsrc) {
        GemvParams p{};
        p.in_mode = GEMV_IN_LN; p.out_mode = GEMV_OUT_F32; p.M = rows; p.K = d; p.KT = d / 32; p.N = sp.vocab;
        p.Wp = e->Wvocab; p.bias = nullptr; p.X = s.xd; p.ldx = d; p.gamma = e->dec_ln_g; p.beta = e->dec_ln_b;
        p.Y = s->logits; p.ldy = s->ldl; p.qscale = 1.f; p.done = done;
        p.xsrc = xsrc; p.slab = s.slab; p.slab_stride = s.slab_rows * d;
        return p;
    };
    int KS = dec_gemv_slab_split(rows, F, d);
    if (rows > s.slab_rows) KS = 0;
    if (rows > 16 && !alt) KS = 0;
    if (alt && s->pf_one_pass) KS = 0;
    if (KS && !(dec_gemv_is_lean(qkv_params(0, GEMV_X_SLABS)) && dec_gemv_is_lean(oproj_params(0, GEMV_X_SLABS)))) KS = 0;
    const bool fold_embed = (rows <= 16 || (alt != nullptr && rows <= 64)) && dec_gemv_is_lean(qkv_params(0, GEMV_X_EMBED));
    if (!fold_embed)
        plaunch(s.base, "dec_embed_kernel", (double)rows * d * (2 + 4), [&] { launch_dec_embed(e->tok_emb16, e->dec_pos, d, rt, rows, s.xd, done, st); });
    bool slabs_pending = false;
    for (int l = 0; l < sp.dec_layers; ++l) {
        const LayerW& w = e->dec[l];
        half_t* kc = s->kc + (size_t)l * s->cache_rows * crs;
        half_t* vc = s->vc + (size_t)l * s->cache_rows * crs;
        {
            GemvParams pq = qkv_params(l, (l == 0 && fold_embed) ? GEMV_X_EMBED : (slabs_pending ? GEMV_X_SLABS : GEMV_X_PLAIN));
            pgemv(s.base, pq);
        }
        plaunch(s.base, "dec_self_attn2_kernel", 4.0 * rows * d * (s->prof ? s->prof->t + 1 : 1), [&] { launch_dec_self_attn(s.qd, d, kc, vc, crs, d, H, rt, rows, s.attnd, d, done, s->anc_ident, st); });
        pgemv(s.base, oproj_params(l, slabs_pending ? GEMV_X_SLABS : GEMV_X_PLAIN));
        slabs_pending = false;
        GemvParams p{};
        const half_t* ckl = s->ck + (size_t)l * s->B * WLX_T_AUDIO_PAD * d;
        const half_t* cvl = s->cvt + (size_t)l * s->B * d * WLX_T_AUDIO_PAD;
        const bool fused = !s->align && rows <= 48 && dec_cq_cross_attn_eligible(d, H, R);
        if (fused)
            plaunch(s.base, "dec_cq_cross_attn_kernel", 2.0 * d * d + 4.0 * groups * WLX_T_AUDIO * d, [&] {
                launch_dec_cq_cross_attn(s.xd, d, w.ln2_g, w.ln2_b, w.Wcq, w.bcq, 0.125f, d, ckl, cvl, (long)WLX_T_AUDIO_PAD * d, H, R,
                                         groups, rows, s.d_group_item, s.part_o, s.part_ml, st);
            });
        if (!fused) {
            p = GemvParams{};
            p.in_mode = GEMV_IN_LN; p.out_mode = GEMV_OUT_F16; p.M = rows; p.K = d; p.KT = d / 32; p.N = d;
            p.Wp = w.Wcq; p.bias = w.bcq; p.X = s.xd; p.ldx = d; p.gamma = w.ln2_g; p.beta = w.ln2_b;
            p.Yh = s.qd; p.ldyh = d; p.qscale = 0.125f; p.done = done;
            pgemv(s.base, p);
            if (s->align) {
                const Slot::AlignCapture& a = *s->align;
                for (int hi = 0; hi < a.n_heads; ++hi)
                    if (a.heads[2 * hi] == l)
                        launch_dec_align_scores(s.qd, d, s->ck + ((size_t)l * s->B + a.item) * WLX_T_AUDIO_PAD * d, a.heads[2 * hi + 1], rows,
                                                a.scores + ((size_t)hi * a.n_tok + a.row0) * WLX_T_AUDIO_PAD, st);
            }
            plaunch(s.base, "dec_cross_attn_kernel", 4.0 * groups * WLX_T_AUDIO * d, [&] {
                launch_dec_cross_attn(s.qd, d, ckl, cvl, (long)WLX_T_AUDIO_PAD * d, H, R, groups, rows, s.d_group_item, s.part_o, s.part_ml, st);
            });
        }
        p = GemvParams{};
        p.in_mode = GEMV_IN_XATTN; p.out_mode = GEMV_OUT_RESID; p.M = rows; p.K = d; p.KT = d / 32; p.N = d;
        p.Wp = w.Wco; p.bias = w.bco; p.part_o = s.part_o; p.part_ml = s.part_ml; p.H = H; p.R = R;
        p.Xres = s.xd; p.ldxres = d; p.qscale = 1.f; p.done = done;
        if (rows > 16) {
            plaunch(s.base, "dec_xattn_combine_kernel", 0.0, [&] { launch_dec_xattn_combine(s.part_o, s.part_ml, rows, H, R, s.attnd, d, st); });
            p.in_mode = GEMV_IN_F16; p.Xh = s.attnd; p.ldxh = d;
        }
        pgemv(s.base, p);
        p = GemvParams{};
        p.in_mode = GEMV_IN_LN; p.out_mode = GEMV_OUT_GELU_F16; p.M = rows; p.K = d; p.KT = d / 32; p.N = F;
        p.Wp = w.W1; p.bias = w.b1; p.X = s.xd; p.ldx = d; p.gamma = w.ln3_g; p.beta = w.ln3_b;
        p.Yh = s.hd; p.ldyh = F; p.qscale = 1.f; p.done = done;
        pgemv(s.base, p);
        p = GemvParams{};
        p.in_mode = GEMV_IN_F16; p.out_mode = GEMV_OUT_RESID; p.M = rows; p.K = F; p.KT = F / 32; p.N = d;
        p.Wp = w.W2; p.bias = w.b2; p.Xh = s.hd; p.ldxh = F; p.Xres = s.xd; p.ldxres = d; p.qscale = 1.f; p.done = done;
        const bool last_split = with_logits && dec_gemv_is_lean(vocab_params(GEMV_X_SLABS));
        if (KS && (l + 1 < sp.dec_layers || last_split)) {
            p.out_mode = GEMV_OUT_SLAB; p.KTS = p.KT / KS; p.slab = s.slab; p.slab_stride = s.slab_rows * d;
            slabs_pending = true;
        }
        pgemv(s.base, p);
    }
    if (with_logits) pgemv(s.base, vocab_params(slabs_pending ? GEMV_X_SLABS : GEMV_X_PLAIN));
}

static int upload_rows(Slot* s, const std::vector<int>& token, const std::vector<int>& pos,
                       const std::vector<int>& cache, const std::vector<int>& ancrow, const std::vector<int>& group_item,
                       int* own_staging = nullptr) {
    const size_t rows = token.size(), ng = group_item.size();
    if (4 * rows + ng > s->h_stage_ints) return set_error(WLX_ERR_ARG, "row table too large");
    s->anc_ident = true;
    for (size_t i = 0; i < rows; ++i) s->anc_ident = s->anc_ident && ancrow[i] == (int)i;
    if (!own_staging) CK(hipStreamSynchronize(s->stream));
    int* h = own_staging ? own_staging : s->h_stage;
    memcpy(h, token.data(), rows * 4); memcpy(h + rows, pos.data(), rows * 4);
    memcpy(h + 2 * rows, cache.data(), rows * 4); memcpy(h + 3 * rows, ancrow.data(), rows * 4);
    memcpy(h + 4 * rows, group_item.data(), ng * 4);
    CK(hipMemcpyAsync(s->d_token, h, rows * 4, hipMemcpyHostToDevice, s->stream));
    CK(hipMemcpyAsync(s->d_pos, h + rows, rows * 4, hipMemcpyHostToDevice, s->stream));
    CK(hipMemcpyAsync(s->d_cache, h + 2 * rows, rows * 4, hipMemcpyHostToDevice, s->stream));
    CK(hipMemcpyAsync(s->d_ancrow, h + 3 * rows, rows * 4, hipMemcpyHostToDevice, s->stream));
    CK(hipMemcpyAsync(s->d_group_item, h + 4 * rows, ng * 4, hipMemcpyHostToDevice, s->stream));
    return WLX_OK;
}

static int prefill_tokens(Engine* e, Slot* s, int item, int crow, const int* tokens, int pos0, int n,
                          float* logits_host, int nsp_index, int nsp_token, float* nsp_out) {
    const bool one_pass = [] { const char* v = getenv("WLX_PREFILL_ONE_PASS"); return !(v && v[0] == '0'); }();
    if (one_pass && s->pf_ok && !logits_host && !s->align && !s->prof && n > 48 && n <= WLX_T_TEXT && !g_decode_v1) {
        const int rows = n, groups = (rows + 15) / 16;
        if (s->h_pf_used) CK(hipStreamSynchronize(s->stream));
        s->h_pf_used = true;
        int* h = s->h_pf;
        for (int i = 0; i < rows; ++i) { h[i] = tokens[i]; h[rows + i] = pos0 + i; h[2 * rows + i] = crow; h[3 * rows + i] = crow; }
        for (int g = 0; g < groups; ++g) h[4 * rows + g] = item;
        const Slot::DecBufs& b = s->pf;
        CK(hipMemcpyAsync(b.d_token, h, rows * 4, hipMemcpyHostToDevice, s->stream));
        CK(hipMemcpyAsync(b.d_pos, h + rows, rows * 4, hipMemcpyHostToDevice, s->stream));
        CK(hipMemcpyAsync(b.d_cache, h + 2 * rows, rows * 4, hipMemcpyHostToDevice, s->stream));
        CK(hipMemcpyAsync(b.d_ancrow, h + 3 * rows, rows * 4, hipMemcpyHostToDevice, s->stream));
        CK(hipMemcpyAsync(b.d_group_item, h + 4 * rows, groups * 4, hipMemcpyHostToDevice, s->stream));
        s->anc_ident = false;
        s->pf_one_pass = true;
        decoder_pass(e, s, rows, 16, groups, false, false, &b);
        s->pf_one_pass = false;
        CK(hipGetLastError());
        if (nsp_index >= 0 && nsp_index < rows) {
            const int d = e->spec.d_model;
            GemvParams p{};
            p.in_mode = GEMV_IN_LN; p.out_mode = GEMV_OUT_F32; p.M = 1; p.K = d; p.KT = d / 32; p.N = e->spec.vocab;
            p.Wp = e->Wvocab; p.bias = nullptr; p.X = b.xd + (size_t)nsp_index * d; p.ldx = d; p.gamma = e->dec_ln_g; p.beta = e->dec_ln_b;
            p.Y = s->logits; p.ldy = s->ldl; p.qscale = 1.f; p.xsrc = GEMV_X_PLAIN;
            launch_dec_gemv(p, s->stream);
            launch_token_prob(s->logits, s->ldl, e->spec.vocab, 1, nsp_token, s->d_tokprob, s->stream);
            CK(hipMemcpyAsync(nsp_out, s->d_tokprob, 4, hipMemcpyDefault, s->stream));
            CK(hipGetLastError());
        }
        return WLX_OK;
    }
    const int chunk = std::min(s->rows_cap, [] { const char* v = getenv("WLX_PREFILL_ROWS"); const int c = v ? atoi(v) : 48; return (c >= 16 && c <= WLX_MAX_DEC_ROWS) ? c : 48; }());
    for (int c0 = 0; c0 < n; c0 += chunk) {
        const int rows = std::min(chunk, n - c0);
        const int groups = (rows + 15) / 16;
        std::vector<int> tk(rows), ps(rows), ca(rows, crow), an(rows, crow), gi(groups, item);
        for (int i = 0; i < rows; ++i) { tk[i] = tokens[c0 + i]; ps[i] = pos0 + c0 + i; }
        CKR(upload_rows(s, tk, ps, ca, an, gi));
        const bool want_nsp = nsp_index >= c0 && nsp_index < c0 + rows;
        const bool lg = (logits_host != nullptr) || want_nsp;
        decoder_pass(e, s, rows, 16, groups, lg, false);
        CK(hipGetLastError());
        if (logits_host) {
            CK(hipMemcpy2DAsync(logits_host + (size_t)c0 * e->spec.vocab, (size_t)e->spec.vocab * 4, s->logits,
                                (size_t)s->ldl * 4, (size_t)e->spec.vocab * 4, rows, hipMemcpyDeviceToHost, s->stream));
        }
        if (want_nsp) {
            launch_token_prob(s->logits + (size_t)(nsp_index - c0) * s->ldl, s->ldl, e->spec.vocab, 1, nsp_token,
                              s->d_tokprob, s->stream);
            CK(hipMemcpyAsync(nsp_out, s->d_tokprob, 4, hipMemcpyDeviceToDevice, s->stream));
        }
    }
    return WLX_OK;
}

static int set_anc_rows(Slot* s, const std::vector<short>& anc_host, int first_row, int nrows) {
    CK(hipMemcpyAsync(s->d_anc + (size_t)first_row * WLX_T_TEXT, anc_host.data(), (size_t)nrows * WLX_T_TEXT * sizeof(short),
                      hipMemcpyHostToDevice, s->stream));
    CK(hipStreamSynchronize(s->stream));
    return WLX_OK;
}

static void launch_search(Engine* e, Slot* s, int rows, int R, int groups, bool sampling) {
    if (sampling || g_decode_v1) {
        launch_search_rows(s->logits, s->d_sp, rows, s->st, s->stream);
        launch_search_update(s->d_sp, groups, s->st, s->stream);
    } else {
        launch_search_scan3(s->logits, s->ldl, e->spec.vocab, s->d_sp, rows, s->st, s->stream);
        launch_search_merge_update3(s->logits, s->ldl, e->spec.vocab, s->d_sp, groups, R, s->st, s->stream);
    }
}

static int graph_steps_for(const Slot* s, int rows) {
    static const int env = [] { const char* v = wlx_ab("WLX_GRAPH_STEPS"); const int n = v ? atoi(v) : 2; return (n == 1 || n == 2) ? n : 2; }();
    if (env == 1 || rows > 16) return 1;
    const bool alone = s->device_of >= 0 && s->device_of < 64 && g_slots_live[s->device_of].load(std::memory_order_relaxed) <= 1;
    return alone ? 2 : 1;
}

static int get_step_graph(Engine* e, Slot* s, int rows, int R, int groups, bool sampling, int nsteps, hipGraphExec_t* out) {
    s->busy_variant = device_is_busy(s);
    StepGraphKey key{rows, R, groups * 8 + (nsteps == 2 ? 4 : 0) + (s->busy_variant ? 2 : 0) + (sampling ? 1 : 0)};
    auto it = s->graphs.find(key);
    if (it != s->graphs.end()) { *out = it->second; return WLX_OK; }
    hipGraph_t graph;
    decoder_pass(e, s, rows, R, groups, true, true);
    CK(hipGetLastError());
    CK(hipStreamBeginCapture(s->stream, hipStreamCaptureModeThreadLocal));
    for (int k = 0; k < nsteps; ++k) {
        decoder_pass(e, s, rows, R, groups, true, true);
        launch_search(e, s, rows, R, groups, sampling);
    }
    const hipError_t ce = hipStreamEndCapture(s->stream, &graph);
    if (ce != hipSuccess) {
        (void)hipGetLastError();
        hipStream_t ns = nullptr;
        bool ded = false;
        if (s->dedicated_queue) { g_dedicated_live[e->device].fetch_sub(1); s->dedicated_queue = false; }
        if (create_slot_stream(e->device, &ns, &ded) == WLX_OK) {
            s->dedicated_queue = ded;
            (void)hipStreamDestroy(s->stream);
            s->stream = ns;
        }
        return set_error(WLX_ERR_HIP, "decode-step graph capture failed: %s (slot stream replaced)", hipGetErrorString(ce));
    }
    hipGraphExec_t exec;
    CK(hipGraphInstantiate(&exec, graph, nullptr, nullptr, 0));
    CK(hipGraphDestroy(graph));
    s->graphs[key] = exec;
    *out = exec;
    return WLX_OK;
}

static int run_step(Engine* e, Slot* s, int rows, int R, int groups, bool sampling, int nsteps = 1) {
    if (e->use_graph) {
        hipGraphExec_t exec;
        CKR(get_step_graph(e, s, rows, R, groups, sampling, nsteps, &exec));
        CK(hipGraphLaunch(exec, s->stream));
    } else {
        s->busy_variant = device_is_busy(s);
        for (int k = 0; k < nsteps; ++k) {
            decoder_pass(e, s, rows, R, groups, true, true);
            launch_search(e, s, rows, R, groups, sampling);
        }
        CK(hipGetLastError());
    }
    return WLX_OK;
}

static int fill_search_params(Engine* e, Slot* s, int batch, int R, const wlx_gen_opts* o, bool apply_ts, SearchParams* sp) {
    memset(sp, 0, sizeof(*sp));
    sp->V = e->spec.vocab; sp->ldl = s->ldl; sp->items = batch; sp->R = R; sp->rows = batch * R;
    sp->sampling = (o->sampling_temperature > 0.f || o->beam_size <= 1) ? 1 : 0;
    sp->beam = sp->sampling ? 1 : o->beam_size;
    sp->ncand = sp->sampling ? 1 : 2 * o->beam_size;
    sp->max_cand_hyp = std::max(1, (int)std::lround((double)o->beam_size * (double)o->patience));
    sp->num_hyp = std::max(1, o->num_hypotheses);
    sp->allow_early_exit = (o->length_penalty == 0.f) ? 1 : 0;
    sp->length_penalty = o->length_penalty; sp->rep_penalty = (o->repetition_penalty > 0.f) ? o->repetition_penalty : 1.f;
    sp->temperature = o->sampling_temperature; sp->no_repeat_ngram = o->no_repeat_ngram_size;
    sp->topk = (o->sampling_temperature > 0.f) ? o->sampling_topk : 1;
    sp->suppress_blank = o->suppress_blank; sp->apply_ts_rules = apply_ts ? 1 : 0;
    sp->max_initial_ts = o->max_initial_timestamp_index;
    sp->sot = o->ids.sot; sp->eot = o->ids.eot; sp->no_timestamps = o->ids.no_timestamps; sp->ts_begin = o->ids.timestamp_begin;
    sp->no_speech = o->ids.no_speech; sp->blank = o->ids.blank;
    sp->max_length = o->max_length; sp->seed = o->seed; sp->suppress_mask = s->d_suppress;
    return WLX_OK;
}

static int validate_opts(Engine* e, Slot* s, int batch, const wlx_gen_opts* o) {
    if (!o) return set_error(WLX_ERR_ARG, "null opts");
    const int V = e->spec.vocab;
    auto bad = [&](int id) { return id < 0 || id >= V; };
    if (bad(o->ids.sot) || bad(o->ids.eot) || bad(o->ids.no_timestamps) || bad(o->ids.timestamp_begin) || bad(o->ids.no_speech))
        return set_error(WLX_ERR_ARG, "token ids out of vocabulary");
    if (o->max_length < 2 || o->max_length > WLX_T_TEXT) return set_error(WLX_ERR_ARG, "max_length must be 2..448");
    const bool sampling = (o->sampling_temperature > 0.f || o->beam_size <= 1);
    const int R = sampling ? std::max(1, o->num_hypotheses) : o->beam_size;
    if (R < 1 || R > s->R) return set_error(WLX_ERR_ARG, "beam_size/num_hypotheses %d exceeds slot rows per item %d", R, s->R);
    if (!sampling && o->num_hypotheses > o->beam_size) return set_error(WLX_ERR_ARG, "num_hypotheses > beam_size");
    if (!sampling && 2 * o->beam_size > WLX_MAX_CAND) return set_error(WLX_ERR_ARG, "beam_size too large");
    if (batch * R > s->rows_cap) return set_error(WLX_ERR_ARG, "too many decoder rows");
    if (o->n_suppress_tokens < 0 || (o->n_suppress_tokens > 0 && !o->suppress_tokens)) return set_error(WLX_ERR_ARG, "bad suppress_tokens");
    return WLX_OK;
}

static int upload_suppress(Engine* e, Slot* s, const wlx_gen_opts* o) {
    const int V = e->spec.vocab, words = (V + 31) / 32;
    if (s->suppress_valid && (int)s->last_suppress.size() == o->n_suppress_tokens &&
        (o->n_suppress_tokens == 0 || memcmp(s->last_suppress.data(), o->suppress_tokens, (size_t)o->n_suppress_tokens * 4) == 0))
        return WLX_OK;
    s->suppress_valid = false;
    std::vector<unsigned> mask(words, 0u);
    for (int i = 0; i < o->n_suppress_tokens; ++i) {
        const int id = o->suppress_tokens[i];
        if (id >= 0 && id < V) mask[id >> 5] |= 1u << (id & 31);
    }
    CK(hipMemcpyAsync(s->d_suppress, mask.data(), words * 4, hipMemcpyHostToDevice, s->stream));
    CK(hipStreamSynchronize(s->stream));
    s->last_suppress.assign(o->suppress_tokens, o->suppress_tokens + o->n_suppress_tokens);
    s->suppress_valid = true;
    return WLX_OK;
}

struct HypOut { std::vector<int> tokens; float score; };

static int generate_impl(Engine* e, Slot* s, int batch, const int32_t* prompts, const int32_t* plens, int pstride,
                         const int32_t* enc_items, const wlx_gen_opts* o, bool injected_logits, const float* inj, int inj_steps,
                         int32_t* tokens_out, int tstride, int32_t* n_tokens_out, float* scores_out, float* nsp_out) {
    CKR(validate_opts(e, s, batch, o));
    static const bool gen_trace = getenv("WLX_GEN_TRACE") != nullptr;
    auto now_us = [] { return std::chrono::duration<double, std::micro>(std::chrono::steady_clock::now().time_since_epoch()).count(); };
    const double tg0 = now_us();
    double tg_launch = 0.0, tg_wait = 0.0;
    s->h_pf_used = false;
    const bool sampling = (o->sampling_temperature > 0.f || o->beam_size <= 1);
    const int R = sampling ? std::max(1, o->num_hypotheses) : o->beam_size;
    const int rows = batch * R, V = e->spec.vocab;
    hipStream_t st = s->stream;
    int max_steps = 0;
    bool apply_ts = true;
    for (int b = 0; b < batch; ++b) {
        const int pl = plens[b];
        if (pl < 1 || pl >= o->max_length) return set_error(WLX_ERR_ARG, "item %d: prompt length %d vs max_length %d", b, pl, o->max_length);
        const int32_t* pr = prompts + (size_t)b * pstride;
        for (int i = 0; i < pl; ++i) {
            if (pr[i] < 0 || pr[i] >= V) return set_error(WLX_ERR_ARG, "prompt token out of vocabulary");
            if (pr[i] == o->ids.no_timestamps) apply_ts = false;
        }
        max_steps = std::max(max_steps, o->max_length - pl);
    }
    CK(hipEventRecord(s->ev0, st));
    CKR(upload_suppress(e, s, o));
    SearchState& S = s->st;
    unsigned char* hg = s->h_gen;
    SearchParams* h_sp = reinterpret_cast<SearchParams*>(hg);                       hg += 4096;
    float* h_cum = reinterpret_cast<float*>(hg);                                    hg += (size_t)s->rows_cap * 4;
    int* h_rule = reinterpret_cast<int*>(hg);                                       hg += (size_t)s->rows_cap * 16;
    int* h_nsp = reinterpret_cast<int*>(hg);                                        hg += (size_t)s->rows_cap * 4;
    int* h_plen = reinterpret_cast<int*>(hg);                                       hg += (size_t)s->B * 4;
    short* h_anc = reinterpret_cast<short*>(hg);                                    hg += (size_t)s->rows_cap * WLX_T_TEXT * 2 + 192;
    int* h_rows = reinterpret_cast<int*>(hg);                                       hg += ((size_t)s->rows_cap * 4 + s->B) * 4 + 64;
    unsigned char* h_res = s->h_gen + ((hg - s->h_gen + 63) / 64) * 64;
    static_assert(sizeof(SearchParams) <= 4096, "SearchParams staging");
    CKR(fill_search_params(e, s, batch, R, o, apply_ts, h_sp));
    CK(hipMemcpyAsync(s->d_sp, h_sp, sizeof(SearchParams), hipMemcpyHostToDevice, st));
    launch_search_reset(S, batch, rows, st);
    std::vector<int> nsp(rows, 0), pl(batch);
    memset(h_anc, 0, (size_t)rows * WLX_T_TEXT * 2);
    for (int b = 0; b < batch; ++b) {
        pl[b] = plens[b];
        h_plen[b] = plens[b];
        for (int r = 0; r < R; ++r) {
            const int row = b * R + r;
            h_cum[row] = (sampling || r == 0) ? 0.f : -INFINITY;
            short* a = h_anc + (size_t)row * WLX_T_TEXT;
            for (int p = 0; p < pl[b] - 1; ++p) a[p] = (short)(b * R);
            a[pl[b] - 1] = (short)row;
            h_rule[4 * row] = 0; h_rule[4 * row + 1] = 1; h_rule[4 * row + 2] = -1; h_rule[4 * row + 3] = 0;
        }
    }
    CK(hipMemcpyAsync(S.cum, h_cum, rows * 4, hipMemcpyHostToDevice, st));
    CK(hipMemcpyAsync(S.rule, h_rule, (size_t)rows * 16, hipMemcpyHostToDevice, st));
    CK(hipMemcpyAsync(S.plen, h_plen, batch * 4, hipMemcpyHostToDevice, st));
    CK(hipMemcpyAsync(s->d_anc, h_anc, (size_t)rows * WLX_T_TEXT * sizeof(short), hipMemcpyHostToDevice, st));
    if (!injected_logits) {
        std::vector<int> sot_at(batch, -1);
        int longest = 0, with_prompt = 0;
        for (int b = 0; b < batch; ++b) {
            const int32_t* pr = prompts + (size_t)b * pstride;
            for (int i = 0; i < pl[b]; ++i) if (pr[i] == o->ids.sot) sot_at[b] = i;
            if (sot_at[b] == pl[b] - 1) { for (int r = 0; r < (sampling ? R : 1); ++r) nsp[b * R + r] = (r == 0) ? 1 : 0; }
            longest = std::max(longest, pl[b] - 1);
            with_prompt += pl[b] > 1 ? 1 : 0;
        }
        static const bool joint = [] { const char* v = wlx_ab("WLX_PREFILL_JOINT"); return !(v && v[0] == '0'); }();
        if (joint && batch > 1 && with_prompt > 1 && longest <= 16 && s->pf_ok && !s->align && !s->prof && !g_decode_v1) {
            const int IB = WLX_T_TEXT / 16;
            const Slot::DecBufs& pb = s->pf;
            const int d = e->spec.d_model;
            for (int b0 = 0; b0 < batch; b0 += IB) {
                const int nb = std::min(IB, batch - b0), prow = 16 * nb;
                if ((size_t)(4 * prow + nb) > s->h_stage_ints - 8) return set_error(WLX_ERR_ARG, "batch too large");
                CK(hipStreamSynchronize(st));
                int* h = s->h_stage;
                for (int bi = 0; bi < nb; ++bi) {
                    const int b = b0 + bi;
                    const int32_t* pr = prompts + (size_t)b * pstride;
                    const int np_ = pl[b] - 1;
                    for (int i = 0; i < 16; ++i) {
                        const int j = np_ > 0 ? std::min(i, np_ - 1) : 0;
                        h[bi * 16 + i] = pr[j]; h[prow + bi * 16 + i] = j; h[2 * prow + bi * 16 + i] = b * R; h[3 * prow + bi * 16 + i] = b * R;
                    }
                    h[4 * prow + bi] = enc_items ? enc_items[b] : b;
                }
                CK(hipMemcpyAsync(pb.d_token, h, prow * 4, hipMemcpyHostToDevice, st));
                CK(hipMemcpyAsync(pb.d_pos, h + prow, prow * 4, hipMemcpyHostToDevice, st));
                CK(hipMemcpyAsync(pb.d_cache, h + 2 * prow, prow * 4, hipMemcpyHostToDevice, st));
                CK(hipMemcpyAsync(pb.d_ancrow, h + 3 * prow, prow * 4, hipMemcpyHostToDevice, st));
                CK(hipMemcpyAsync(pb.d_group_item, h + 4 * prow, nb * 4, hipMemcpyHostToDevice, st));
                s->anc_ident = false;
                decoder_pass(e, s, prow, 16, nb, false, false, &pb);
                CK(hipGetLastError());
                for (int bi = 0; bi < nb; ++bi) {
                    const int b = b0 + bi;
                    if (!(sot_at[b] >= 0 && sot_at[b] < pl[b] - 1)) continue;
                    GemvParams p{};
                    p.in_mode = GEMV_IN_LN; p.out_mode = GEMV_OUT_F32; p.M = 1; p.K = d; p.KT = d / 32; p.N = V;
                    p.Wp = e->Wvocab; p.bias = nullptr; p.X = pb.xd + (size_t)(bi * 16 + sot_at[b]) * d; p.ldx = d; p.gamma = e->dec_ln_g; p.beta = e->dec_ln_b;
                    p.Y = s->logits; p.ldy = s->ldl; p.qscale = 1.f; p.xsrc = GEMV_X_PLAIN;
                    launch_dec_gemv(p, st);
                    launch_token_prob(s->logits, s->ldl, V, 1, o->ids.no_speech, s->d_tokprob, st);
                    CK(hipMemcpyAsync(S.no_speech + b, s->d_tokprob, 4, hipMemcpyDefault, st));
                }
                CK(hipGetLastError());
            }
        } else {
            for (int b = 0; b < batch; ++b) {
                const int32_t* pr = prompts + (size_t)b * pstride;
                if (pl[b] > 1)
                    CKR(prefill_tokens(e, s, enc_items ? enc_items[b] : b, b * R, pr, 0, pl[b] - 1, nullptr, (sot_at[b] >= 0 && sot_at[b] < pl[b] - 1) ? sot_at[b] : -1,
                                       o->ids.no_speech, S.no_speech + b));
            }
        }
    }
    {
        std::vector<int> tk(rows), ps(rows), ca(rows), an(rows), gi(batch);
        for (int b = 0; b < batch; ++b) {
// ... 258 lines not shown
    if (eot < 1 || eot > e->spec.vocab || median_filter_width < 1 || (median_filter_width & 1) == 0) return set_error(WLX_ERR_ARG, "align: bad eot / filter width");
    int nf = num_frames / 2;
    if (nf < 1) nf = 1;
    if (nf > WLX_T_AUDIO) nf = WLX_T_AUDIO;
    const int n_text = n_tokens - n_sot - 2;
    CK(hipSetDevice(e->device));
    hipStream_t st = s->stream;
    const size_t need = (size_t)n_heads * n_tokens * WLX_T_AUDIO_PAD;
    if (need > s->align_cap) {
        CK(hipStreamSynchronize(st));
        if (s->align_scores) CK(hipFree(s->align_scores));
        s->align_scores = nullptr; s->align_cap = 0;
        CK(hipMalloc(reinterpret_cast<void**>(&s->align_scores), need * sizeof(float)));
        s->align_cap = need;
    }
    const int crow = item * s->R;
    std::vector<short> anc((size_t)WLX_T_TEXT, (short)crow);
    CKR(set_anc_rows(s, anc, crow, 1));
    Slot::AlignCapture cap{s->align_scores, heads, n_heads, n_tokens, 0, item};
    std::vector<float> probs(n_tokens, 0.f);
    int rc = WLX_OK;
    s->align = &cap;
    for (int c0 = 0; c0 < n_tokens && rc == WLX_OK; c0 += 64) {
        const int rows = std::min(64, n_tokens - c0);
        const int groups = (rows + 15) / 16;
        std::vector<int> tk(rows), ps(rows), ca(rows, crow), an(rows, crow), gi(groups, item), tgt(rows, -1);
        for (int i = 0; i < rows; ++i) {
            tk[i] = tokens[c0 + i]; ps[i] = c0 + i;
            const int p = c0 + i;
            if (p >= n_sot && p < n_sot + n_text) tgt[i] = tokens[p + 1];
        }
        rc = upload_rows(s, tk, ps, ca, an, gi);
        if (rc != WLX_OK) break;
        cap.row0 = c0;
        decoder_pass(e, s, rows, 16, groups, true, false);
        if (hipMemcpyAsync(s->d_align_tgt, tgt.data(), (size_t)rows * 4, hipMemcpyHostToDevice, st) != hipSuccess) { rc = WLX_ERR_HIP; break; }
        launch_token_prob_rows(s->logits, s->ldl, eot, rows, s->d_align_tgt, s->d_align_prob, st);
        if (hipMemcpyAsync(probs.data() + c0, s->d_align_prob, (size_t)rows * 4, hipMemcpyDeviceToHost, st) != hipSuccess) { rc = WLX_ERR_HIP; break; }
        if (hipStreamSynchronize(st) != hipSuccess) { rc = WLX_ERR_HIP; break; }
    }
    s->align = nullptr;
    if (rc != WLX_OK) return set_error(rc, "align: decoder pass failed");
    CK(hipGetLastError());
    std::vector<float> scores(need);
    CK(hipMemcpyAsync(scores.data(), s->align_scores, need * sizeof(float), hipMemcpyDeviceToHost, st));
    CK(hipStreamSynchronize(st));
    std::vector<int32_t> ti, fi;
    align_postprocess(scores, n_heads, n_tokens, n_sot, nf, median_filter_width, ti, fi);
    if ((int)ti.size() > path_cap) return set_error(WLX_ERR_ARG, "align: path of %d steps exceeds the caller's capacity %d", (int)ti.size(), path_cap);
    memcpy(text_indices, ti.data(), ti.size() * 4);
    memcpy(time_indices, fi.data(), fi.size() * 4);
    *n_path_out = (int32_t)ti.size();
    for (int i = 0; i < n_text; ++i) text_token_probs[i] = probs[n_sot + i];
    return WLX_OK;
}

extern "C" int32_t wlx_debug_logits_get(wlx_engine* e, int32_t slot, float* out, int32_t rows, int64_t cap_floats) {
    SlotGuard sg_;
    CKR(slot_acquire(e, slot, sg_));
    Slot* s = sg_.s;
    const int V = e->spec.vocab;
    if (!out || rows < 1 || rows > s->rows_cap || (int64_t)rows * V > cap_floats) return set_error(WLX_ERR_ARG, "bad rows/cap");
    CK(hipSetDevice(e->device));
    CK(hipMemcpy2DAsync(out, (size_t)V * 4, s->logits, (size_t)s->ldl * 4, (size_t)V * 4, rows, hipMemcpyDeviceToHost, s->stream));
    CK(hipStreamSynchronize(s->stream));
    return WLX_OK;
}

extern "C" int32_t wlx_debug_decode_logits(wlx_engine* e, int32_t slot, const int32_t* tokens, int32_t n, float* out) {
    SlotGuard sg_;
    CKR(slot_acquire(e, slot, sg_));
    Slot* s = sg_.s;
    if (!tokens || !out || n < 1 || n > WLX_T_TEXT) return set_error(WLX_ERR_ARG, "bad tokens");
    if (s->enc_batch < 1) return set_error(WLX_ERR_STATE, "decode before encode");
    for (int i = 0; i < n; ++i) if (tokens[i] < 0 || tokens[i] >= e->spec.vocab) return set_error(WLX_ERR_ARG, "token out of vocabulary");
    CK(hipSetDevice(e->device));
    std::vector<short> anc(WLX_T_TEXT, 0);
    CKR(set_anc_rows(s, anc, 0, 1));
    CKR(prefill_tokens(e, s, 0, 0, tokens, 0, n, out, -1, 0, nullptr));
    CK(hipStreamSynchronize(s->stream));
    return WLX_OK;
}

extern "C" int32_t wlx_debug_time_decode_step(wlx_engine* e, int32_t slot, int32_t rows, int32_t t, int32_t iters,
                                              float* avg_ms_out) {
    SlotGuard sg_;
    CKR(slot_acquire(e, slot, sg_));
    Slot* s = sg_.s;
    if (rows < 1 || rows > s->cache_rows || rows > s->rows_cap || t < 0 || t >= WLX_T_TEXT || iters < 1 || !avg_ms_out)
        return set_error(WLX_ERR_ARG, "bad arguments");
    if (rows > 16 && (rows % s->R != 0 || rows / s->R > s->B)) return set_error(WLX_ERR_ARG, "more than 16 rows: a multiple of the slot's rows per item");
    if (s->enc_batch < 1) return set_error(WLX_ERR_STATE, "decode before encode");
    s->busy_variant = device_is_busy(s);
    CK(hipSetDevice(e->device));
    hipStream_t st = s->stream;
    const int tR = rows > 16 ? s->R : rows, tG = rows / tR;
    std::vector<int> tk(rows, 0), ps(rows, t), ca(rows), an(rows), gi(tG, 0);
    for (int g = 0; g < tG; ++g) gi[g] = g % std::max(1, s->enc_batch);
    std::vector<short> anc((size_t)rows * WLX_T_TEXT);
    for (int r = 0; r < rows; ++r) { ca[r] = an[r] = r; for (int p = 0; p < WLX_T_TEXT; ++p) anc[(size_t)r * WLX_T_TEXT + p] = (short)r; }
    CKR(set_anc_rows(s, anc, 0, rows));
    CKR(upload_rows(s, tk, ps, ca, an, gi));
    CK(hipMemsetAsync(s->st.done, 0, 4, st));
    hipGraph_t graph; hipGraphExec_t exec;
    decoder_pass(e, s, rows, tR, tG, true, true);
    constexpr int passes = 1;
    CK(hipStreamBeginCapture(st, hipStreamCaptureModeThreadLocal));
    for (int q = 0; q < passes; ++q) decoder_pass(e, s, rows, tR, tG, true, true);
    CK(hipStreamEndCapture(st, &graph));
    CK(hipGraphInstantiate(&exec, graph, nullptr, nullptr, 0));
    CK(hipGraphDestroy(graph));
    for (int i = 0; i < 3; ++i) CK(hipGraphLaunch(exec, st));
    CK(hipEventRecord(s->ev0, st));
    for (int i = 0; i < iters; ++i) CK(hipGraphLaunch(exec, st));
    CK(hipEventRecord(s->ev1, st));
    CK(hipStreamSynchronize(st));
    float ms = 0.f;
    CK(hipEventElapsedTime(&ms, s->ev0, s->ev1));
    *avg_ms_out = ms / (float)iters / (float)passes;
    CK(hipGraphExecDestroy(exec));
    return WLX_OK;
}

extern "C" int32_t wlx_debug_trace_step(wlx_engine* e, int32_t slot, int32_t rows, int32_t t, int32_t with_search,
                                        uint64_t* out, int64_t cap_u64, char* names, int32_t* n_launches_out) {
#ifndef WLX_TRACE
    (void)e; (void)slot; (void)rows; (void)t; (void)with_search; (void)out; (void)cap_u64; (void)names; (void)n_launches_out;
    return set_error(WLX_ERR_STATE, "libwlx.so was built without -DWLX_TRACE (use libwlx_trace.so, scripts/trace_step.py)");
#else
    SlotGuard sg_;
    CKR(slot_acquire(e, slot, sg_));
    Slot* s = sg_.s;
    if (rows < 1 || rows > s->cache_rows || rows > s->rows_cap || t < 0 || t >= WLX_T_TEXT || !out || !names || !n_launches_out)
        return set_error(WLX_ERR_ARG, "bad arguments");
    if (rows > 16 && (rows % s->R != 0 || rows / s->R > s->B)) return set_error(WLX_ERR_ARG, "more than 16 rows: a multiple of the slot's rows per item");
    if (s->enc_batch < 1) return set_error(WLX_ERR_STATE, "decode before encode");
    CK(hipSetDevice(e->device));
    hipStream_t st = s->stream;
    const int tR = rows > 16 ? s->R : rows, tG = rows / tR;
    std::vector<int> tk(rows, 0), ps(rows, t), ca(rows), an(rows), gi(tG, 0);
    for (int g = 0; g < tG; ++g) gi[g] = g % std::max(1, s->enc_batch);
    std::vector<short> anc((size_t)rows * WLX_T_TEXT);
    for (int r = 0; r < rows; ++r) { ca[r] = an[r] = r; for (int p = 0; p < WLX_T_TEXT; ++p) anc[(size_t)r * WLX_T_TEXT + p] = (short)r; }
    const size_t max_launch = 320;
    unsigned long long* buf = nullptr;
    CK(hipMalloc(&buf, max_launch * WLX_TR_STRIDE * 8));
    g_trace_buf = buf; g_trace_seq = 0;
    hipGraph_t graph; hipGraphExec_t exec;
    auto reset_state = [&]() -> int {
        CKR(set_anc_rows(s, anc, 0, rows));
        CKR(upload_rows(s, tk, ps, ca, an, gi));
        CK(hipMemsetAsync(s->st.done, 0, 4, st)); CK(hipMemsetAsync(s->st.item_done, 0, 4, st));
        CK(hipMemsetAsync(s->st.n_hyp, 0, 4, st)); CK(hipMemsetAsync(s->st.n_finished, 0, 4, st));
        static const int rule0[16 * 4] = {0, 1, -1, 0, 0, 1, -1, 0, 0, 1, -1, 0, 0, 1, -1, 0, 0, 1, -1, 0, 0, 1, -1, 0, 0, 1, -1, 0, 0, 1, -1, 0,
                                          0, 1, -1, 0, 0, 1, -1, 0, 0, 1, -1, 0, 0, 1, -1, 0, 0, 1, -1, 0, 0, 1, -1, 0, 0, 1, -1, 0, 0, 1, -1, 0};
        CK(hipMemcpyAsync(s->st.rule, rule0, (size_t)rows * 16, hipMemcpyHostToDevice, st));
        return WLX_OK;
    };
    CKR(reset_state());
    { const int seq0 = g_trace_seq; unsigned long long* b0 = g_trace_buf; g_trace_buf = nullptr;
      decoder_pass(e, s, rows, tR, tG, true, true); g_trace_seq = seq0; g_trace_buf = b0; }
    CK(hipStreamBeginCapture(st, hipStreamCaptureModeThreadLocal));
    decoder_pass(e, s, rows, tR, tG, true, true);
    if (with_search) launch_search(e, s, rows, tR, tG, false);
    CK(hipStreamEndCapture(st, &graph));
    CK(hipGraphInstantiate(&exec, graph, nullptr, nullptr, 0));
    CK(hipGraphDestroy(graph));
    const int n = g_trace_seq;
    g_trace_buf = nullptr;
    if (n > (int)max_launch) { (void)hipGraphExecDestroy(exec); (void)hipFree(buf); return set_error(WLX_ERR_ARG, "trace: %d launches exceed the trace buffer (%d)", n, (int)max_launch); }
    for (int i = 0; i < 3; ++i) { CKR(reset_state()); CK(hipGraphLaunch(exec, st)); }
    CKR(reset_state());
    CK(hipMemsetAsync(buf, 0, max_launch * WLX_TR_STRIDE * 8, st));
    CK(hipStreamSynchronize(st));
    CK(hipGraphLaunch(exec, st));
    CK(hipStreamSynchronize(st));
    CK(hipGraphExecDestroy(exec));
    if ((int64_t)n * WLX_TR_STRIDE > cap_u64) { (void)hipFree(buf); return set_error(WLX_ERR_ARG, "trace buffer too small"); }
    CK(hipMemcpyAsync(out, buf, (size_t)n * WLX_TR_STRIDE * 8, hipMemcpyDeviceToHost, st));
    CK(hipStreamSynchronize(st));
    CK(hipFree(buf));
    for (int i = 0; i < n; ++i) { strncpy(names + (size_t)i * 48, g_trace_names[i] ? g_trace_names[i] : "?", 47); names[(size_t)i * 48 + 47] = 0; }
    *n_launches_out = n;
    return WLX_OK;
#endif
}

extern "C" int32_t wlx_debug_profile_step(wlx_engine* e, int32_t slot, int32_t rows, int32_t t, int32_t iters,
                                          wlx_kernel_stat* out, int32_t cap, int32_t* n_out) {
    SlotGuard sg_;
    CKR(slot_acquire(e, slot, sg_));
    Slot* s = sg_.s;
    if (rows < 1 || rows > s->cache_rows || rows > s->rows_cap || t < 0 || t >= WLX_T_TEXT || iters < 1 || !out || !n_out || cap < 1)
        return set_error(WLX_ERR_ARG, "bad arguments");
    if (rows > 16 && (rows % s->R != 0 || rows / s->R > s->B)) return set_error(WLX_ERR_ARG, "more than 16 rows: a multiple of the slot's rows per item");
    if (s->enc_batch < 1) return set_error(WLX_ERR_STATE, "decode before encode");
    s->busy_variant = device_is_busy(s);
    CK(hipSetDevice(e->device));
    hipStream_t st = s->stream;
    const int tR = rows > 16 ? s->R : rows, tG = rows / tR;
    std::vector<int> tk(rows, 0), ps(rows, t), ca(rows), an(rows), gi(tG, 0);
    for (int g = 0; g < tG; ++g) gi[g] = g % std::max(1, s->enc_batch);
    std::vector<short> anc((size_t)rows * WLX_T_TEXT);
    for (int r = 0; r < rows; ++r) { ca[r] = an[r] = r; for (int p = 0; p < WLX_T_TEXT; ++p) anc[(size_t)r * WLX_T_TEXT + p] = (short)r; }
    CKR(set_anc_rows(s, anc, 0, rows));
    CKR(upload_rows(s, tk, ps, ca, an, gi));
    CK(hipMemsetAsync(s->st.done, 0, 4, st));
    for (int i = 0; i < 2; ++i) decoder_pass(e, s, rows, tR, tG, true, true);
    CK(hipStreamSynchronize(st));
    Prof prof;
    prof.t = t;
    s->prof = &prof;
    decoder_pass(e, s, rows, tR, tG, true, true);
    struct Agg { int launches = 0; double bytes = 0, us = 0; };
    std::map<std::string, Agg> agg;
    for (auto& r : prof.recs) { Agg& a = agg[r.name]; a.launches += 1; a.bytes += r.bytes; }
    prof.list_only = false;
    int rc = WLX_OK;
    for (auto& kv : agg) {
        prof.only = kv.first;
        hipGraph_t graph; hipGraphExec_t exec;
        if (hipStreamBeginCapture(st, hipStreamCaptureModeThreadLocal) != hipSuccess) { rc = WLX_ERR_HIP; break; }
        decoder_pass(e, s, rows, tR, tG, true, true);
        if (hipStreamEndCapture(st, &graph) != hipSuccess) { rc = WLX_ERR_HIP; break; }
        if (hipGraphInstantiate(&exec, graph, nullptr, nullptr, 0) != hipSuccess) { (void)hipGraphDestroy(graph); rc = WLX_ERR_HIP; break; }
        (void)hipGraphDestroy(graph);
        for (int i = 0; i < 3; ++i) (void)hipGraphLaunch(exec, st);
        (void)hipEventRecord(s->ev0, st);
        for (int i = 0; i < iters; ++i) (void)hipGraphLaunch(exec, st);
        (void)hipEventRecord(s->ev1, st);
        (void)hipStreamSynchronize(st);
        float ms = 0.f;
        (void)hipEventElapsedTime(&ms, s->ev0, s->ev1);
        (void)hipGraphExecDestroy(exec);
        kv.second.us = 1000.0 * ms / iters;
    }
    s->prof = nullptr;
    if (rc != WLX_OK) return set_error(rc, "profile capture failed");
    CK(hipGetLastError());
    int n = 0;
    for (auto& kv : agg) {
        if (n >= cap) break;
        wlx_kernel_stat& o = out[n++];
        memset(&o, 0, sizeof(o));
        snprintf(o.name, sizeof(o.name), "%s", kv.first.c_str());
        o.launches_per_step = (float)kv.second.launches;
        o.avg_us = (float)(kv.second.us / kv.second.launches);
// ... 7 lines not shown
```

whisperlive_amd/csrc/search.hip:

```cpp
#include "decoder.h"

namespace wlx {

#define SR_THREADS 1024
#define SR_NPT 52

__device__ __forceinline__ float block_max(float v, float* scratch) {
    v = wave_max(v);
    __syncthreads();
    if ((threadIdx.x & 63) == 0) scratch[threadIdx.x >> 6] = v;
    __syncthreads();
    float r = scratch[0];
#pragma unroll
    for (int w = 1; w < SR_THREADS / 64; ++w) r = fmaxf(r, scratch[w]);
    return r;
}
__device__ __forceinline__ float block_sum(float v, float* scratch) {
    v = wave_sum(v);
    __syncthreads();
    if ((threadIdx.x & 63) == 0) scratch[threadIdx.x >> 6] = v;
    __syncthreads();
    float r = 0.f;
#pragma unroll
    for (int w = 0; w < SR_THREADS / 64; ++w) r += scratch[w];
// ... 455 lines not shown
    else id = dpp_wave_min_i32((v == m) ? i : 0x7fffffff);
    i = id;
    v = m;
}
__device__ __forceinline__ void s3_row_argmax(float& v, int& i) {
    float m = v;
    WLX_DPP_REDUCE_ROW("v_max_f32_dpp", m);
    int t = (v == m) ? i : 0x7fffffff;
    WLX_DPP_REDUCE_ROW("v_min_i32_dpp", t);
    v = m; i = t;
}

__device__ __forceinline__ void s3_chunk(int chunk, int ts_begin, int V, int& id0, int& lim, int& nct, int& nch) {
    nct = (ts_begin + SC_CHUNK - 1) / SC_CHUNK;
    nch = nct + (V - ts_begin + SC_CHUNK - 1) / SC_CHUNK;
    const bool is_ts = chunk >= nct;
    id0 = is_ts ? ts_begin + (chunk - nct) * SC_CHUNK : chunk * SC_CHUNK;
    lim = is_ts ? V : ts_begin;
}

__global__ __launch_bounds__(SC_THREADS) void search_scan3_kernel(const float* __restrict__ logits, long ldl, int V,
                                                                  const SearchParams* __restrict__ spp, SearchState st WLX_TR_PARAM) {
    const int chunk = blockIdx.x, r = blockIdx.y, tid = threadIdx.x, lane = tid & 63;
    const int wave = __builtin_amdgcn_readfirstlane(tid >> 6);
    WLX_TR_BEGIN();
    const SearchParams sp = *spp;
    int id0, lim, nct, nch_;
    s3_chunk(chunk, sp.ts_begin, V, id0, lim, nct, nch_);
    if (chunk >= nch_) return;
    const float* lrow = logits + (long)r * ldl + id0 + tid;
    float v[SC_NPT];
#pragma unroll
    for (int i = 0; i < SC_NPT; ++i) v[i] = (id0 + i * SC_THREADS + tid < lim) ? lrow[i * SC_THREADS] : WLX_NEG_INF;
    const int item = r / sp.R;
    const int rb = r - item * sp.R;
    const int4 rule = *reinterpret_cast<const int4*>(st.rule + 4 * r);
    const int p = st.pos[r], plen = st.plen[item], nsp = st.nsp_row[r];
    if (st.item_done[item] || rb >= sp.beam) return;
    const int ngen = p + 1 - plen;

    __shared__ float fs[6][4];
    __shared__ float wv_s[4][WLX_MAX_CAND];
    __shared__ int wi_s[4][WLX_MAX_CAND];

    if (sp.rep_penalty != 1.0f || sp.no_repeat_ngram > 0) {
        __shared__ int hist[WLX_T_TEXT];
        const short* ar = st.anc + (long)r * WLX_T_TEXT;
        for (int j = tid; j < ngen; j += SC_THREADS) hist[j] = st.intok[(long)ar[plen + j] * WLX_T_TEXT + plen + j];
        __syncthreads();
        if (sp.rep_penalty != 1.0f) {
#pragma unroll
            for (int i = 0; i < SC_NPT; ++i) {
                const int id = id0 + i * SC_THREADS + tid;
                bool hit = false;
                for (int j = 0; j < ngen; ++j) hit = hit || (hist[j] == id);
                if (hit && id < lim) v[i] = (v[i] < 0.f) ? v[i] * sp.rep_penalty : v[i] / sp.rep_penalty;
            }
        }
        if (sp.no_repeat_ngram > 0 && ngen >= sp.no_repeat_ngram - 1) {
            const int n = sp.no_repeat_ngram;
            for (int j = 0; j + n - 1 < ngen; ++j) {
                bool match = true;
                for (int q = 0; q < n - 1; ++q) match = match && (hist[j + q] == hist[ngen - (n - 1) + q]);
                if (match) {
                    const int banned = hist[j + n - 1];
#pragma unroll
                    for (int i = 0; i < SC_NPT; ++i)
                        if (id0 + i * SC_THREADS + tid == banned) v[i] = WLX_NEG_INF;
                }
            }
        }
    }
    WLX_TR_MARK(1);

    float raw_m = WLX_NEG_INF, raw_s = 0.f;
    if (nsp > 0) {
        float mx = v[0];
#pragma unroll
        for (int i = 1; i < SC_NPT; ++i) mx = fmaxf(mx, v[i]);
        raw_m = mx;
    }
    const float raw_local = raw_m;

    const bool ts = sp.apply_ts_rules != 0;
    const bool last_was_ts = ts && rule.x != 0;
    const bool penult_was_ts = ts && rule.y != 0;
    int ts_last = -1;
    if (ts && rule.z >= 0) ts_last = (last_was_ts && !penult_was_ts) ? rule.z : rule.z + 1;
    const bool first = (ngen == 0);
    const int last_allowed = (sp.max_initial_ts >= 0) ? sp.ts_begin + sp.max_initial_ts : 0x7fffffff;
    float w[SC_NPT];
#pragma unroll
    for (int i = 0; i < SC_NPT; ++i) {
        const int id = id0 + i * SC_THREADS + tid;
        bool kill = id >= lim;
        if (!kill) kill = (sp.suppress_mask[id >> 5] >> (id & 31)) & 1u;
        if (first && sp.suppress_blank && (id == sp.blank || id == sp.eot)) kill = true;
        if (ts) {
            if (id == sp.no_timestamps) kill = true;
            if (last_was_ts) {
                if (penult_was_ts) { if (id >= sp.ts_begin) kill = true; }
                else if (id < sp.eot) kill = true;
            }
            if (id >= sp.ts_begin && id < ts_last) kill = true;
            if (first) {
                if (id < sp.ts_begin) kill = true;
                if (id > last_allowed) kill = true;
            }
        }
        w[i] = kill ? WLX_NEG_INF : v[i];
    }

    const bool ts_chunk = chunk >= nct;
    float mx = w[0];
#pragma unroll
    for (int i = 1; i < SC_NPT; ++i) mx = fmaxf(mx, w[i]);
    mx = s3_wave_max(mx);
    const float raw_wm = (nsp > 0) ? s3_wave_max(raw_local) : WLX_NEG_INF;
    if (lane == 0) { fs[0][wave] = mx; fs[2][wave] = raw_wm; }
    __syncthreads();
    mx = fmaxf(fmaxf(fs[0][0], fs[0][1]), fmaxf(fs[0][2], fs[0][3]));
    raw_m = fmaxf(fmaxf(fs[2][0], fs[2][1]), fmaxf(fs[2][2], fs[2][3]));
    float sm = 0.f;
#pragma unroll
    for (int i = 0; i < SC_NPT; ++i) {
        if (mx > WLX_NEG_INF) sm += __expf(w[i] - mx);
        if (nsp > 0 && raw_m > WLX_NEG_INF) raw_s += __expf(v[i] - raw_m);
    }
    sm = s3_wave_sum(sm);
    if (nsp > 0) raw_s = s3_wave_sum(raw_s);
    if (lane == 0) { fs[3][wave] = sm; fs[5][wave] = raw_s; }
    WLX_TR_MARK(2);

    float* cv = st.scan_cv + ((long)r * (SC_MAXCH + 1) + chunk) * WLX_MAX_CAND;
    int* ci = st.scan_ci + ((long)r * (SC_MAXCH + 1) + chunk) * WLX_MAX_CAND;
    {
        float bv = WLX_NEG_INF, cv2 = WLX_NEG_INF; int bi = 0x7fffffff, ci2 = 0x7fffffff;
#pragma unroll
        for (int i = 0; i < SC_NPT; ++i) {
            const int id = id0 + i * SC_THREADS + tid;
            if (w[i] > bv) { cv2 = bv; ci2 = bi; bv = w[i]; bi = id; }
            else if (w[i] > cv2) { cv2 = w[i]; ci2 = id; }
        }
        int won = 0;
#pragma unroll 1
        for (int k = 0; k < sp.ncand; ++k) {
            float gv = bv; int gi = bi;
            s3_wave_argmax(gv, gi);
            if (lane == 0) { wv_s[wave][k] = gv; wi_s[wave][k] = gi; }
            if (gi != 0x7fffffff && ((gi - id0) & (SC_THREADS - 1)) == tid) {
#pragma unroll
                for (int i = 0; i < SC_NPT; ++i)
                    if (id0 + i * SC_THREADS + tid == gi) w[i] = WLX_NEG_INF;
                if (won == 0) { bv = cv2; bi = ci2; }
                else {
                    float tv[SC_NPT]; int ti_[SC_NPT];
#pragma unroll
                    for (int i = 0; i < SC_NPT; ++i) {
                        const int id = id0 + i * SC_THREADS + tid;
                        tv[i] = w[i]; ti_[i] = (w[i] > WLX_NEG_INF) ? id : 0x7fffffff;
                    }
#pragma unroll
                    for (int stp = 1; stp < SC_NPT; stp <<= 1)
#pragma unroll
                        for (int i = 0; i + stp < SC_NPT; i += 2 * stp)
                            if (tv[i + stp] > tv[i]) { tv[i] = tv[i + stp]; ti_[i] = ti_[i + stp]; }
                    bv = tv[0]; bi = ti_[0];
                }
                ++won;
            }
        }
        WLX_TR_MARK(3);
        __syncthreads();
        WLX_TR_MARK(4);
        if (wave == 0) {
            if (lane == 0) {
                float* so = st.scan_stats + ((long)r * SC_MAXCH + chunk) * SC_NSTAT;
                const float ssum = fs[3][0] + fs[3][1] + fs[3][2] + fs[3][3];
                so[0] = ts_chunk ? WLX_NEG_INF : mx; so[1] = ts_chunk ? 0.f : ssum;
                so[2] = ts_chunk ? mx : WLX_NEG_INF; so[3] = ts_chunk ? ssum : 0.f;
                so[4] = raw_m;   so[5] = fs[5][0] + fs[5][1] + fs[5][2] + fs[5][3];
            }
            const int nc = sp.ncand;
            const int e0 = lane, e1 = lane + 64;
            float x0 = WLX_NEG_INF, x1 = WLX_NEG_INF; int i0 = 0x7fffffff, i1 = 0x7fffffff;
            if (e0 < 4 * nc) { const int q = e0 / nc, k = e0 - q * nc; x0 = wv_s[q][k]; i0 = wi_s[q][k]; }
            if (e1 < 4 * nc) { const int q = e1 / nc, k = e1 - q * nc; x1 = wv_s[q][k]; i1 = wi_s[q][k]; }
#pragma unroll 1
            for (int k = 0; k < nc; ++k) {
                const bool f1 = (x1 > x0) || (x1 == x0 && i1 < i0);
                float gv = f1 ? x1 : x0; int gi = f1 ? i1 : i0;
                s3_wave_argmax(gv, gi);
                if (lane == 0) { cv[k] = gv; ci[k] = gi; }
                if (gi != 0x7fffffff) {
                    if (i0 == gi) { x0 = WLX_NEG_INF; i0 = 0x7fffffff; }
                    if (i1 == gi) { x1 = WLX_NEG_INF; i1 = 0x7fffffff; }
                }
            }
        }
    }
    WLX_TR_MARK(5);
    WLX_TR_END(trc);
}

void launch_search_scan3(const float* logits, long ldl, int V, const SearchParams* sp_dev, int rows, const SearchState& st,
                         hipStream_t s) {
    hipLaunchKernelGGL(search_scan3_kernel, dim3(SC_MAXCH, rows), dim3(SC_THREADS), 0, s, logits, ldl, V, sp_dev, st WLX_TR_ARG("search_scan3"));
}

#define MU3_THREADS 384
__global__ __launch_bounds__(MU3_THREADS) void search_merge_update3_kernel(const float* __restrict__ logits, long ldl, int V,
                                                                           const SearchParams* __restrict__ spp, SearchState st, int R WLX_TR_PARAM) {
    const int item = blockIdx.x;
    const int tid = threadIdx.x, lane = tid & 63;
    const int wave = __builtin_amdgcn_readfirstlane(tid >> 6);
    constexpr int NW = MU3_THREADS / 64;
    constexpr int PQ = 3;
    const int r0 = item * R;
    const int done_v = *st.done;
    const int idone = st.item_done[item];
    const int plen = st.plen[item];
    const int p = st.pos[r0];
    const int n_hyp0 = st.n_hyp[item];
    const int rp = r0 + (wave < R ? wave : R - 1);
    const int lc = lane < SC_MAXCH ? lane : SC_MAXCH - 1;
    const float4* pso = reinterpret_cast<const float4*>(st.scan_stats + ((long)rp * SC_MAXCH + lc) * SC_NSTAT);
    const float4 ps0 = pso[0], ps1 = pso[1];
    const float4* pcv = reinterpret_cast<const float4*>(st.scan_cv + ((long)rp * (SC_MAXCH + 1) + lc) * WLX_MAX_CAND);
    const int4* pci = reinterpret_cast<const int4*>(st.scan_ci + ((long)rp * (SC_MAXCH + 1) + lc) * WLX_MAX_CAND);
    float4 pa[PQ]; int4 pb[PQ];
#pragma unroll
    for (int k = 0; k < PQ; ++k) { pa[k] = pcv[k]; pb[k] = pci[k]; }
    const float pcum = st.cum[rp];
    const int pnsp = st.nsp_row[rp];
    const SearchParams sp = *spp;
    if (done_v) return;
    WLX_TR_BEGIN();
    int step_no = 0;
    if (item == 0 && tid == 0) step_no = atomicAdd(st.step, 1) + 1;
    if (idone) { if (step_no) step_mirror(st, step_no); return; }
    int id0_, lim_, nct, nch;
    s3_chunk(0, sp.ts_begin, V, id0_, lim_, nct, nch);

    __shared__ float cand_s[16][WLX_MAX_CAND];
    __shared__ int cand_t[16][WLX_MAX_CAND];
    __shared__ float lv[NW][SC_MAXCH + 1][WLX_MAX_CAND];
    __shared__ int li[NW][SC_MAXCH + 1][WLX_MAX_CAND];
    __shared__ short anc_s[16 * WLX_T_TEXT];
    __shared__ int parent[16], newtok[16];
    __shared__ float newcum[16];
    __shared__ int hyp_src[16], hyp_extra[16], hyp_slot[16], hyp_n;
    __shared__ int n_active_s, finished_s;
    __shared__ int ord_b[WLX_MAX_CAND], ord_t[WLX_MAX_CAND];
    __shared__ float ord_s[WLX_MAX_CAND];
    __shared__ int4 rule_old[16];

    for (int i = tid; i < sp.beam * (p + 1); i += MU3_THREADS) {
        const int b = i / (p + 1), q = i - b * (p + 1);
        anc_s[b * WLX_T_TEXT + q] = st.anc[(long)(r0 + b) * WLX_T_TEXT + q];
    }
    if (tid < sp.beam) rule_old[tid] = *reinterpret_cast<const int4*>(st.rule + 4 * (r0 + tid));

    const bool ts = sp.apply_ts_rules != 0;
    const int nc4 = (sp.ncand + 3) >> 2;
#pragma unroll 1
    for (int rb = wave; rb < sp.beam; rb += NW) {
        const int r = r0 + rb;
        const bool first = rb == wave;
        const bool have = lane < nch;
        float4 s0 = make_float4(WLX_NEG_INF, 0.f, WLX_NEG_INF, 0.f), s1 = make_float4(WLX_NEG_INF, 0.f, 0.f, 0.f);
        float cum_r; int nsp_r;
        {
            const float4* cv = reinterpret_cast<const float4*>(st.scan_cv + ((long)r * (SC_MAXCH + 1) + lc) * WLX_MAX_CAND);
            const int4* ci = reinterpret_cast<const int4*>(st.scan_ci + ((long)r * (SC_MAXCH + 1) + lc) * WLX_MAX_CAND);
            float4 a[WLX_MAX_CAND / 4]; int4 b[WLX_MAX_CAND / 4];
            if (first) {
#pragma unroll
                for (int k = 0; k < PQ; ++k) { a[k] = pa[k]; b[k] = pb[k]; }
#pragma unroll
                for (int k = PQ; k < WLX_MAX_CAND / 4; ++k)
                    if (k < nc4) { a[k] = cv[k]; b[k] = ci[k]; }
                if (have) { s0 = ps0; s1 = ps1; }
                cum_r = pcum; nsp_r = pnsp;
            } else {
#pragma unroll
                for (int k = 0; k < WLX_MAX_CAND / 4; ++k)
                    if (k < nc4) { a[k] = cv[k]; b[k] = ci[k]; }
                const float4* so = reinterpret_cast<const float4*>(st.scan_stats + ((long)r * SC_MAXCH + lc) * SC_NSTAT);
                const float4 t0 = so[0], t1 = so[1];
                if (have) { s0 = t0; s1 = t1; }
                cum_r = st.cum[r]; nsp_r = st.nsp_row[r];
            }
#pragma unroll
            for (int k = 0; k < WLX_MAX_CAND / 4; ++k)
                if (k < nc4 && have) {
                    *reinterpret_cast<float4*>(&lv[wave][lane][4 * k]) = have ? a[k] : make_float4(WLX_NEG_INF, WLX_NEG_INF, WLX_NEG_INF, WLX_NEG_INF);
                    *reinterpret_cast<int4*>(&li[wave][lane][4 * k]) = have ? b[k] : make_int4(0x7fffffff, 0x7fffffff, 0x7fffffff, 0x7fffffff);
                }
        }
        const float mt = s0.x, st_ = s0.y, mts = s0.z, sts = s0.w, rm = s1.x, rs = s1.y;
        const float Mtext = s3_wave_max(mt), Mts = s3_wave_max(mts);
        if (nsp_r > 0) {
            const float RM = s3_wave_max(rm);
            const float RS = s3_wave_sum((rm > WLX_NEG_INF) ? rs * __expf(rm - RM) : 0.f);
            if (lane == 0) st.no_speech[item] = __expf(logits[(long)r * ldl + sp.no_speech] - RM) / RS;
        }
        const float S_ts = s3_wave_sum((mts > WLX_NEG_INF) ? sts * __expf(mts - Mts) : 0.f);
        const float lse_ts = (Mts > WLX_NEG_INF) ? Mts + __logf(S_ts) : WLX_NEG_INF;
        const bool text_masked = ts && (lse_ts > Mtext);
        float lse_sel;
        if (text_masked) {
            lse_sel = lse_ts;
        } else {
            const float mx_all = fmaxf(Mtext, Mts);
            const float a = ((mt > WLX_NEG_INF) ? st_ * __expf(mt - mx_all) : 0.f) +
                            ((mts > WLX_NEG_INF) ? sts * __expf(mts - mx_all) : 0.f);
            lse_sel = mx_all + __logf(s3_wave_sum(a));
        }
        const bool usable = (lane < nch) && (!text_masked || lane >= nct);
        const float base = cum_r - lse_sel;
        int hp = 0;
        float hv = usable ? lv[wave][lane][0] : WLX_NEG_INF;
        int hi = usable ? li[wave][lane][0] : 0x7fffffff;
#pragma unroll 1
        for (int k = 0; k < sp.ncand; ++k) {
            float gv = hv; int gi = hi;
            s3_wave_argmax(gv, gi);
            if (lane == 0) {
                cand_s[rb][k] = (gi < V) ? gv + base : WLX_NEG_INF;
                cand_t[rb][k] = (gi < V) ? gi : sp.eot;
            }
            if (usable && gi != 0x7fffffff && hi == gi) {
                ++hp;
                hv = (hp < sp.ncand) ? lv[wave][lane][hp] : WLX_NEG_INF;
                hi = (hp < sp.ncand) ? li[wave][lane][hp] : 0x7fffffff;
            }
        }
    }
    __syncthreads();
    WLX_TR_MARK(1);

    const int ngen = p + 1 - plen;
    const int max_new = sp.max_length - plen;
    const bool is_last = (ngen + 1 >= max_new);
    if (wave == 0) {
        const int b = lane;
        const bool own = b < sp.beam;
        int hp = 0;
#pragma unroll 1
        for (int k = 0; k < sp.ncand; ++k) {
            const bool alive = own && hp < sp.ncand;
            float kv = alive ? cand_s[b][hp] : WLX_NEG_INF;
            int kb = alive ? b : 0x7fffffff;
            s3_row_argmax(kv, kb);
            if (lane == 0) ord_b[k] = (kb == 0x7fffffff) ? -1 : kb;
            if (alive && b == kb) { ord_s[k] = cand_s[b][hp]; ord_t[k] = cand_t[b][hp]; ++hp; }
        }
        const int k = lane;
        const bool in_list = k < sp.ncand;
        const int bb = in_list ? ord_b[k] : -1;
        const float bs = in_list ? ord_s[k] : 0.f;
        const int tok = in_list ? ord_t[k] : 0;
        const unsigned long long stop = __ballot(!in_list || bb < 0);
        const bool live = k < (int)__builtin_ctzll(stop);
        const bool fin_k = live && (tok == sp.eot || is_last);
        const bool act_k = live && !fin_k;
        const unsigned long long below = (1ull << k) - 1ull;
        const unsigned long long finm = __ballot(fin_k && k < sp.beam);
        const unsigned long long actm = __ballot(act_k);
        int cap = WLX_MAX_HYP - n_hyp0; cap = cap < 16 ? cap : 16; cap = cap > 0 ? cap : 0;
        const int hidx = __builtin_popcountll(finm & below), aidx = __builtin_popcountll(actm & below);
        if (fin_k && k < sp.beam && hidx < cap) {
            const int len = ngen + ((tok == sp.eot) ? 0 : 1);
            const int slot = n_hyp0 + hidx;
            hyp_src[hidx] = bb;
            hyp_extra[hidx] = (tok == sp.eot) ? -1 : tok;
            hyp_slot[hidx] = slot;
            st.hyp_len[item * WLX_MAX_HYP + slot] = len;
            const float flen = (float)(len > 0 ? len : 1);
            const float denom = (sp.length_penalty == 1.0f) ? flen : powf(flen, sp.length_penalty);
            st.hyp_score[item * WLX_MAX_HYP + slot] = bs / denom;
        }
        if (act_k && aidx < sp.beam) { parent[aidx] = bb; newtok[aidx] = tok; newcum[aidx] = bs; }
        if (lane == 0) {
            int nh_new = __builtin_popcountll(finm); nh_new = nh_new < cap ? nh_new : cap;
            int n_active = __builtin_popcountll(actm); n_active = n_active < sp.beam ? n_active : sp.beam;
            const bool top_beam_finished = fin_k;
            const int n_hyp = n_hyp0 + nh_new;
            st.n_hyp[item] = n_hyp; st.n_hyp_host[item] = n_hyp;
            hyp_n = nh_new;
            n_active_s = n_active;
            bool fin = is_last || n_active == 0;
            if (sp.allow_early_exit) fin = fin || (top_beam_finished && n_hyp >= sp.num_hyp);
            else fin = fin || (n_hyp >= sp.max_cand_hyp);
            finished_s = fin ? 1 : 0;
        }
    }
    __syncthreads();
    WLX_TR_MARK(2);
    for (int hh = 0; hh < hyp_n; ++hh) {
        const int b = hyp_src[hh];
        int* dst = st.hyp_tokens + ((long)item * WLX_MAX_HYP + hyp_slot[hh]) * WLX_T_TEXT;
        for (int j = tid; j < ngen; j += MU3_THREADS)
            dst[j] = st.intok[(long)anc_s[b * WLX_T_TEXT + plen + j] * WLX_T_TEXT + plen + j];
        if (tid == 0 && hyp_extra[hh] >= 0) dst[ngen] = hyp_extra[hh];
    }
    if (finished_s) {
        __syncthreads();
        if (tid == 0) {
            if (step_no) step_mirror(st, step_no);
            finish_item(st, item, sp.items);
        }
        return;
    }
    const int na = n_active_s;
    for (int i = tid; i < na * (p + 1); i += MU3_THREADS) {
        const int j = i / (p + 1), q = i - j * (p + 1);
        st.anc[(long)(r0 + j) * WLX_T_TEXT + q] = anc_s[parent[j] * WLX_T_TEXT + q];
    }
    if (tid < sp.beam) {
        const int j = tid;
        st.anc[(long)(r0 + j) * WLX_T_TEXT + p + 1] = (short)(r0 + j);
        int4 ru = make_int4(0, 1, -1, 0);
        if (j < na) {
            const int tok = newtok[j];
            const int4 po = rule_old[parent[j]];
            const int is_ts = tok >= sp.ts_begin ? 1 : 0;
            ru.x = is_ts;
            ru.y = (ngen + 1 < 2) ? 1 : po.x;
            ru.z = is_ts ? tok : po.z;
            st.token[r0 + j] = tok; st.cum[r0 + j] = newcum[j];
        } else { st.token[r0 + j] = sp.eot; st.cum[r0 + j] = WLX_NEG_INF; }
        *reinterpret_cast<int4*>(st.rule + 4 * (r0 + j)) = ru;
        st.pos[r0 + j] = p + 1;
        st.nsp_row[r0 + j] = 0;
    }
    if (step_no) step_mirror(st, step_no);
    WLX_TR_END(trc);
}

void launch_search_merge_update3(const float* logits, long ldl, int V, const SearchParams* sp_dev, int items, int R,
                                 const SearchState& st, hipStream_t s) {
    hipLaunchKernelGGL(search_merge_update3_kernel, dim3(items), dim3(MU3_THREADS), 0, s, logits, ldl, V, sp_dev, st, R WLX_TR_ARG("search_merge_update3"));
}

__global__ __launch_bounds__(256) void search_reset_kernel(SearchState st, int items, int rows) {
    const int t = threadIdx.x;
    if (t == 0) { *st.step = 0; *st.done = 0; *st.n_finished = 0; step_mirror(st, 0); }
    for (int i = t; i < items; i += 256) { st.item_done[i] = 0; st.n_hyp[i] = 0; st.n_hyp_host[i] = 0; st.no_speech[i] = 0.f; }
    for (int i = t; i < rows; i += 256) st.row_done[i] = 0;
    for (int i = t; i < items * WLX_MAX_HYP; i += 256) st.hyp_len[i] = 0;
}
void launch_search_reset(const SearchState& st, int items, int rows, hipStream_t s) {
    hipLaunchKernelGGL(search_reset_kernel, dim3(1), dim3(256), 0, s, st, items, rows);
}

__global__ __launch_bounds__(SR_THREADS) void token_prob_kernel(const float* __restrict__ logits, long ldl, int V,
                                                               int tok, float* __restrict__ out) {
    __shared__ float fs[16];
    const float* lrow = logits + (long)blockIdx.x * ldl;
    float mx = WLX_NEG_INF;
    for (int i = threadIdx.x; i < V; i += SR_THREADS) mx = fmaxf(mx, lrow[i]);
    mx = block_max(mx, fs);
    float sm = 0.f;
    for (int i = threadIdx.x; i < V; i += SR_THREADS) sm += __expf(lrow[i] - mx);
    sm = block_sum(sm, fs);
    if (threadIdx.x == 0) out[blockIdx.x] = __expf(lrow[tok] - mx) / sm;
}
__global__ __launch_bounds__(SR_THREADS) void token_prob_rows_kernel(const float* __restrict__ logits, long ldl, int vlim,
                                                                     const int* __restrict__ toks, float* __restrict__ out) {
    __shared__ float fs[16];
    const int r = blockIdx.x, tid = threadIdx.x;
    const float* lrow = logits + (long)r * ldl;
    float mx = WLX_NEG_INF;
    for (int i = tid; i < vlim; i += SR_THREADS) mx = fmaxf(mx, lrow[i]);
    mx = block_max(mx, fs);
    float sm = 0.f;
    for (int i = tid; i < vlim; i += SR_THREADS) sm += __expf(lrow[i] - mx);
    sm = block_sum(sm, fs);
    if (tid == 0) { const int t = toks[r]; out[r] = (t >= 0 && t < vlim) ? __expf(lrow[t] - mx) / sm : 0.f; }
}
void launch_token_prob_rows(const float* logits, long ldl, int vlim, int rows, const int* toks, float* out, hipStream_t s) {
    hipLaunchKernelGGL(token_prob_rows_kernel, dim3(rows), dim3(SR_THREADS), 0, s, logits, ldl, vlim, toks, out);
}

void launch_token_prob(const float* logits, long ldl, int V, int rows, int tok, float* out, hipStream_t s) {
    hipLaunchKernelGGL(token_prob_kernel, dim3(rows), dim3(SR_THREADS), 0, s, logits, ldl, V, tok, out);
}

__global__ __launch_bounds__(256) void lang_probs_kernel(const float* __restrict__ logits, long ldl,
                                                         const int* __restrict__ ids, int n, float* __restrict__ probs) {
    __shared__ float red[4];
    const float* lrow = logits + (long)blockIdx.x * ldl;
    float mx = WLX_NEG_INF;
    for (int i = threadIdx.x; i < n; i += 256) mx = fmaxf(mx, lrow[ids[i]]);
    mx = wave_max(mx);
    if ((threadIdx.x & 63) == 0) red[threadIdx.x >> 6] = mx;
    __syncthreads();
    mx = fmaxf(fmaxf(red[0], red[1]), fmaxf(red[2], red[3]));
    __syncthreads();
    float sm = 0.f;
    for (int i = threadIdx.x; i < n; i += 256) sm += __expf(lrow[ids[i]] - mx);
    sm = wave_sum(sm);
    if ((threadIdx.x & 63) == 0) red[threadIdx.x >> 6] = sm;
    __syncthreads();
    sm = red[0] + red[1] + red[2] + red[3];
    for (int i = threadIdx.x; i < n; i += 256) probs[(long)blockIdx.x * n + i] = __expf(lrow[ids[i]] - mx) / sm;
}
void launch_lang_probs(const float* logits, long ldl, int rows, const int* ids, int n, float* probs, hipStream_t s) {
    hipLaunchKernelGGL(lang_probs_kernel, dim3(rows), dim3(256), 0, s, logits, ldl, ids, n, probs);
}

}
```

Before: 1154 xRT (audio s / wall s).

## Fuse beam-search logit masking and softmax stats into vocab GEMV epilogue

Moves the search scan work (suppression/timestamp rule masking, per-block max/sum-exp stats for text, timestamp and raw logits) into the epilogue of the vocab projection kernel. Masked logits go to a padded buffer and per-block stats to a small array. A templated merge kernel then picks top candidate blocks from the stats and reads only those blocks, which replaces the separate scan3 pass over the full vocab. This saves a kernel launch and a full re-read of the logits per decode step, at the cost of more registers and an extra store in the GEMV and more complex candidate selection.

New measurement: 1155 xRT (audio s / wall s) (median of 5 runs). About the same (+0.1%).

```diff
diff --git a/include/wlx.h b/include/wlx.h
--- a/include/wlx.h
+++ b/include/wlx.h
@@ -172,6 +172,7 @@
 int32_t wlx_debug_search(wlx_engine* e, int32_t slot, const float* logits, int32_t steps,
                          const int32_t* prompt, int32_t prompt_len, const wlx_gen_opts* opts,
                          int32_t* tokens_out, int32_t tokens_stride, int32_t* n_tokens_out, float* scores_out);
+int32_t wlx_debug_search_tail(int32_t mode, int32_t* mode_before_out, int64_t* fused_steps_out);
 int32_t wlx_debug_time_decode_step(wlx_engine* e, int32_t slot, int32_t rows, int32_t t, int32_t iters,
                                    float* avg_ms_out);
 
diff --git a/whisperlive_amd/_lib.py b/whisperlive_amd/_lib.py
--- a/whisperlive_amd/_lib.py
+++ b/whisperlive_amd/_lib.py
@@ -20,7 +20,7 @@
     "wlx_vad_create", "wlx_vad_destroy", "wlx_vad_probs",
     "wlx_ring_create", "wlx_ring_destroy", "wlx_ring_append", "wlx_ring_state", "wlx_vad_probs_resident", "wlx_vad_segments", "wlx_logmel_ring",
     "wlx_mt_create", "wlx_mt_destroy", "wlx_mt_slot_create", "wlx_mt_slot_destroy", "wlx_mt_translate",
-    "wlx_debug_logits_get", "wlx_debug_decode_logits", "wlx_debug_search", "wlx_debug_time_decode_step", "wlx_debug_profile_step", "wlx_debug_trace_step",
+    "wlx_debug_logits_get", "wlx_debug_decode_logits", "wlx_debug_search", "wlx_debug_time_decode_step", "wlx_debug_profile_step", "wlx_debug_trace_step", "wlx_debug_search_tail",
     "wlx_mt_debug_encode", "wlx_mt_debug_decode_logits", "wlx_mt_debug_timings", "wlx_mt_debug_attn", "wlx_mt_debug_topk",
     "wlx_mt_debug_embed",
     "wlx_debug_layernorm", "wlx_debug_attn_encoder", "wlx_debug_dec_cross_attn", "wlx_debug_dec_self_attn", "wlx_debug_gemm",
@@ -241,6 +241,7 @@
     lib.wlx_debug_time_decode_step.argtypes = [vp, i32, i32, i32, i32, f32p]
     lib.wlx_debug_profile_step.argtypes = [vp, i32, i32, i32, i32, C.POINTER(wlx_kernel_stat), i32, i32p]
     lib.wlx_debug_trace_step.argtypes = [vp, i32, i32, i32, i32, C.POINTER(C.c_uint64), i64, C.c_char_p, i32p]
+    lib.wlx_debug_search_tail.argtypes = [i32, i32p, i64p]
     lib.wlx_mt_create.argtypes = [C.POINTER(wlx_mt_spec), C.POINTER(wlx_tensor), i32, i32, C.POINTER(vp)]
     lib.wlx_mt_destroy.argtypes = [vp]
     lib.wlx_mt_destroy.restype = None
diff --git a/whisperlive_amd/csrc/decoder.h b/whisperlive_amd/csrc/decoder.h
--- a/whisperlive_amd/csrc/decoder.h
+++ b/whisperlive_amd/csrc/decoder.h
@@ -63,6 +63,7 @@
     int xsrc;
     float* slab; long slab_stride;
     int KTS;
+    const struct VocabTail* tail;
     const half_t* tok_emb; const float* pos_emb; const int* emb_token; int* intok;
     WLX_TR_FIELD
 };
@@ -81,6 +82,19 @@
 #define WLX_TR_ARG(name)
 #endif
 void launch_dec_gemv(const GemvParams& p, hipStream_t s);
+#define WLX_TAIL_BLK 256
+#define WLX_TAIL_MAXBLK 208
+#define WLX_TAIL_NSTAT 6
+#define WLX_TAIL_LD (WLX_TAIL_MAXBLK * WLX_TAIL_BLK)
+#define WLX_TAIL_MAX_BEAM 8
+struct VocabTail {
+    const struct SearchParams* spp; const unsigned* suppress_mask;
+    const int* rule; const int* pos; const int* plen; const int* item_done; const int* nsp_row;
+    float* stats;
+    float* wlog;
+    int R;
+};
+bool dec_vocab_tail_ok(int rows, int K, int N);
 const char* dec_gemv_kernel_name(const GemvParams& p);
 extern bool g_decode_v1;
 bool dec_gemv_is_lean(const GemvParams& p);
@@ -121,6 +135,7 @@
     float* scan_stats;
     float* scan_cv; int* scan_ci;
     int* rule;
+    float* tail_stats; float* tail_wlog;
 };
 #define SC_THREADS 256
 #define SC_NPT 8
@@ -141,12 +156,43 @@
     unsigned long long seed;
     const unsigned* suppress_mask;
 };
+struct SearchRule { bool ts, last_was_ts, penult_was_ts, first; int ts_last, last_allowed; };
+__device__ __forceinline__ SearchRule search_rule_of(const SearchParams& sp, const int4 rule, int ngen) {
+    SearchRule q;
+    q.ts = sp.apply_ts_rules != 0;
+    q.last_was_ts = q.ts && rule.x != 0;
+    q.penult_was_ts = q.ts && rule.y != 0;
+    q.ts_last = -1;
+    if (q.ts && rule.z >= 0) q.ts_last = (q.last_was_ts && !q.penult_was_ts) ? rule.z : rule.z + 1;
+    q.first = (ngen == 0);
+    q.last_allowed = (sp.max_initial_ts >= 0) ? sp.ts_begin + sp.max_initial_ts : 0x7fffffff;
+    return q;
+}
+__device__ __forceinline__ bool search_rule_kills(const SearchParams& sp, const SearchRule& q, int id, unsigned mask_word) {
+    bool kill = (mask_word >> (id & 31)) & 1u;
+    if (q.first && sp.suppress_blank && (id == sp.blank || id == sp.eot)) kill = true;
+    if (q.ts) {
+        if (id == sp.no_timestamps) kill = true;
+        if (q.last_was_ts) {
+            if (q.penult_was_ts) { if (id >= sp.ts_begin) kill = true; }
+            else if (id < sp.eot) kill = true;
+        }
+        if (id >= sp.ts_begin && id < q.ts_last) kill = true;
+        if (q.first) {
+            if (id < sp.ts_begin) kill = true;
+            if (id > q.last_allowed) kill = true;
+        }
+    }
+    return kill;
+}
 void launch_search_rows(const float* logits, const SearchParams* sp_dev, int rows, const SearchState& st, hipStream_t s);
 void launch_search_update(const SearchParams* sp_dev, int items, const SearchState& st, hipStream_t s);
 void launch_search_scan3(const float* logits, long ldl, int V, const SearchParams* sp_dev, int rows, const SearchState& st,
                          hipStream_t s);
 void launch_search_merge_update3(const float* logits, long ldl, int V, const SearchParams* sp_dev, int items, int R,
                                  const SearchState& st, hipStream_t s);
+void launch_search_merge_tail(const float* logits, long ldl, int V, const SearchParams* sp_dev, int items, int R,
+                              const SearchState& st, hipStream_t s);
 void launch_search_reset(const SearchState& st, int items, int rows, hipStream_t s);
 void launch_token_prob_rows(const float* logits, long ldl, int vlim, int rows, const int* toks, float* out, hipStream_t s);
 void launch_token_prob(const float* logits, long ldl, int V, int rows, int tok, float* out, hipStream_t s);
diff --git a/whisperlive_amd/csrc/decoder.hip b/whisperlive_amd/csrc/decoder.hip
--- a/whisperlive_amd/csrc/decoder.hip
+++ b/whisperlive_amd/csrc/decoder.hip
@@ -1257,6 +1257,7 @@
     const half_t* Wp; int M, N, NT;
     float* Y; long ldy;
     const float* slab; long slab_stride;
+    VocabTail tail;
     WLX_TR_FIELD
 };
 template <int KT, int KC, int MT, bool SLABS>
@@ -1302,6 +1303,19 @@
 #pragma unroll
         for (int j = 0; j < LNV; ++j) { const int tb = (j == LNV - 1) ? tback : 0; gq[j] = g4[64 * j - tb]; bq[j] = b4[64 * j - tb]; }
     }
+    const bool tail_on_ = MT == 1 && p.tail.spp != nullptr;
+    int4 e_rule = make_int4(0, 0, 0, 0); int e_pos = 0, e_plen = 0, e_idone = 0, e_nsp = 0; unsigned e_mw[2] = {0u, 0u};
+    if (tail_on_) {
+        const int er = (c < p.M) ? c : p.M - 1, ei = er / p.tail.R;
+        e_rule = *reinterpret_cast<const int4*>(p.tail.rule + 4 * er);
+        e_pos = p.tail.pos[er]; e_nsp = p.tail.nsp_row[er];
+        e_plen = p.tail.plen[ei]; e_idone = p.tail.item_done[ei];
+#pragma unroll
+        for (int i = 0; i < 2; ++i) {
+            const int n = (2 * pair + i) * 16 + g * 4;
+            if (n < p.N) e_mw[i] = p.tail.suppress_mask[n >> 5];
+        }
+    }
     asm volatile("" ::: "memory");
     const half_t* wq[2] = {p.Wp + (long)t0 * KT * 512 + lane * 8, p.Wp + (long)t1 * KT * 512 + lane * 8};
     f16x8 wf[2][KC][2];
@@ -1402,6 +1416,75 @@
             const f32x4 v = acc[i][mt];
             if (n + 3 < p.N) *reinterpret_cast<float4*>(yp) = make_float4(v[0], v[1], v[2], v[3]);
             else { if (n < p.N) yp[0] = v[0]; if (n + 1 < p.N) yp[1] = v[1]; if (n + 2 < p.N) yp[2] = v[2]; }
+        }
+    }
+    if constexpr (MT == 1) {
+        if (tail_on_) {
+            WLX_TR_MARK(3);
+            __shared__ float tred[8][WLX_TAIL_NSTAT][16];
+            const SearchParams sp = *p.tail.spp;
+            const SearchRule q = search_rule_of(sp, e_rule, e_pos + 1 - e_plen);
+            float wv[2][4], rv[2][4];
+            float m_tx = WLX_NEG_INF, m_ts = WLX_NEG_INF, m_raw = WLX_NEG_INF;
+#pragma unroll
+            for (int i = 0; i < 2; ++i) {
+                const int nt = 2 * pair + i, n = nt * 16 + g * 4;
+#pragma unroll
+                for (int j = 0; j < 4; ++j) {
+                    const int id = n + j;
+                    const bool real = nt < p.NT && id < p.N;
+                    const float v = acc[i][0][j];
+                    rv[i][j] = real ? v : WLX_NEG_INF;
+                    wv[i][j] = (real && !search_rule_kills(sp, q, id, e_mw[i])) ? v : WLX_NEG_INF;
+                    if (id < sp.ts_begin) m_tx = fmaxf(m_tx, wv[i][j]); else m_ts = fmaxf(m_ts, wv[i][j]);
+                    m_raw = fmaxf(m_raw, rv[i][j]);
+                }
+                if (nt < p.NT && c < p.M)
+                    *reinterpret_cast<float4*>(p.tail.wlog + (long)c * WLX_TAIL_LD + n) = make_float4(wv[i][0], wv[i][1], wv[i][2], wv[i][3]);
+            }
+            m_tx = fmaxf(m_tx, __shfl_xor(m_tx, 16, 64)); m_tx = fmaxf(m_tx, __shfl_xor(m_tx, 32, 64));
+            m_ts = fmaxf(m_ts, __shfl_xor(m_ts, 16, 64)); m_ts = fmaxf(m_ts, __shfl_xor(m_ts, 32, 64));
+            float s_tx = 0.f, s_ts = 0.f, s_raw = 0.f;
+#pragma unroll
+            for (int i = 0; i < 2; ++i)
+#pragma unroll
+                for (int j = 0; j < 4; ++j) {
+                    const int id = (2 * pair + i) * 16 + g * 4 + j;
+                    if (wv[i][j] > WLX_NEG_INF) { if (id < sp.ts_begin) s_tx += __expf(wv[i][j] - m_tx); else s_ts += __expf(wv[i][j] - m_ts); }
+                }
+            s_tx += __shfl_xor(s_tx, 16, 64); s_tx += __shfl_xor(s_tx, 32, 64);
+            s_ts += __shfl_xor(s_ts, 16, 64); s_ts += __shfl_xor(s_ts, 32, 64);
+            if (__any(e_nsp > 0)) {
+                m_raw = fmaxf(m_raw, __shfl_xor(m_raw, 16, 64)); m_raw = fmaxf(m_raw, __shfl_xor(m_raw, 32, 64));
+#pragma unroll
+                for (int i = 0; i < 2; ++i)
+#pragma unroll
+                    for (int j = 0; j < 4; ++j)
+                        if (rv[i][j] > WLX_NEG_INF) s_raw += __expf(rv[i][j] - m_raw);
+                s_raw += __shfl_xor(s_raw, 16, 64); s_raw += __shfl_xor(s_raw, 32, 64);
+            } else m_raw = WLX_NEG_INF;
+            if (g == 0) {
+                tred[wave][0][c] = m_tx; tred[wave][1][c] = s_tx; tred[wave][2][c] = m_ts; tred[wave][3][c] = s_ts;
+                tred[wave][4][c] = m_raw; tred[wave][5][c] = s_raw;
+            }
+            __syncthreads();
+            if (tid < 48) {
+                float mm = tred[0][2 * g][c];
+#pragma unroll
+                for (int w8 = 1; w8 < 8; ++w8) mm = fmaxf(mm, tred[w8][2 * g][c]);
+                float ss = 0.f;
+#pragma unroll
+                for (int w8 = 0; w8 < 8; ++w8) {
+                    const float mw = tred[w8][2 * g][c];
+                    if (mw > WLX_NEG_INF) ss += tred[w8][2 * g + 1][c] * __expf(mw - mm);
+                }
+                const int rb = c - (c / p.tail.R) * p.tail.R;
+                if (c < p.M && !e_idone && rb < sp.beam) {
+                    float* so = p.tail.stats + ((long)c * WLX_TAIL_NSTAT + 2 * g) * WLX_TAIL_MAXBLK + blockIdx.x;
+                    so[0] = mm; so[WLX_TAIL_MAXBLK] = ss;
+                }
+            }
+            WLX_TR_MARK(4);
         }
     }
     WLX_TR_END(p.trc);
@@ -1452,6 +1535,12 @@
     if (shm > 64 * 1024 && g_lds_optin_refused.load(std::memory_order_relaxed)) return false;
     return shm <= WLX_G2_LDS_MAX;
 }
+bool dec_vocab_tail_ok(int rows, int K, int N) {
+    GemvParams p{};
+    p.in_mode = GEMV_IN_LN; p.out_mode = GEMV_OUT_F32; p.M = rows; p.K = K; p.KT = K / 32; p.N = N; p.xsrc = GEMV_X_PLAIN;
+    const int blocks = (((N + 15) / 16 + 1) / 2 + 7) / 8;
+    return rows >= 1 && rows <= 16 && blocks <= WLX_TAIL_MAXBLK && vocab2_ok(p);
+}
 static void vocab2_launch(const GemvParams& g, hipStream_t s) {
     const int CH = vocab2_chunk_rows(g.K);
     for (int r0 = 0; r0 < g.M; r0 += CH) {
@@ -1459,6 +1548,7 @@
         p.X = g.X + (long)r0 * g.ldx; p.ldx = g.ldx; p.gamma = g.gamma; p.beta = g.beta; p.Wp = g.Wp; p.M = std::min(CH, g.M - r0); p.N = g.N; p.NT = (g.N + 15) / 16;
         p.Y = g.Y + (long)r0 * g.ldy; p.ldy = g.ldy;
         if (g.xsrc == GEMV_X_SLABS) { p.slab = g.slab; p.slab_stride = g.slab_stride; }
+        if (g.tail) p.tail = *g.tail;
 #ifdef WLX_TRACE
         p.trc = trace_next("vocab2");
 #endif
diff --git a/whisperlive_amd/csrc/engine.h b/whisperlive_amd/csrc/engine.h
--- a/whisperlive_amd/csrc/engine.h
+++ b/whisperlive_amd/csrc/engine.h
@@ -76,6 +76,8 @@
     int* h_pf = nullptr; bool h_pf_used = false;
     int* h_hyp = nullptr;
     int max_items = 0;
+    bool sp_plain = false;
+    bool tail_now = false;
     std::vector<int> last_suppress; bool suppress_valid = false;
     std::map<StepGraphKey, hipGraphExec_t> graphs;
     wlx_timings tm{};
diff --git a/whisperlive_amd/csrc/engine.hip b/whisperlive_amd/csrc/engine.hip
--- a/whisperlive_amd/csrc/engine.hip
+++ b/whisperlive_amd/csrc/engine.hip
@@ -21,6 +21,8 @@
     asm volatile("" ::: "memory");
 #endif
 }
+static std::atomic<int> g_search_tail{0};
+static std::atomic<long long> g_tail_steps{0};
 extern "C" int32_t wlx_abi_version(void) { return WLX_ABI_VERSION; }
 
 static void build_mel_filters(int n_mels, std::vector<float>& w, std::vector<int>& range) {
@@ -152,6 +154,7 @@
     e->use_graph = !(ng && ng[0] == '1');
     const char* v1 = wlx_ab("WLX_DECODE_V1");
     g_decode_v1 = (v1 && v1[0] == '1');
+    if (const char* tl = wlx_ab("WLX_SEARCH_TAIL")) g_search_tail.store(tl[0] == '0' ? 0 : 1);
     int rc = engine_load(e, weights, n_weights);
     if (rc != WLX_OK) {
         for (void* p : e->allocs) (void)hipFree(p);
@@ -449,6 +452,8 @@
         CKR(dalloc(s->allocs, &st.n_hyp, (size_t)B, true));
         CKR(dalloc(s->allocs, &st.nsp_row, (size_t)RC, true));
         st.token = s->d_token; st.pos = s->d_pos; st.anc = s->d_anc; st.intok = s->d_intok;
+        CKR(dalloc(s->allocs, &st.tail_stats, (size_t)16 * WLX_TAIL_NSTAT * WLX_TAIL_MAXBLK, true));
+        CKR(dalloc(s->allocs, &st.tail_wlog, (size_t)16 * WLX_TAIL_LD, true));
         CKR(dalloc(s->allocs, &st.scan_stats, (size_t)RC * SC_MAXCH * SC_NSTAT, true));
         CKR(dalloc(s->allocs, &st.scan_cv, (size_t)RC * (SC_MAXCH + 1) * WLX_MAX_CAND, true));
         CKR(dalloc(s->allocs, &st.scan_ci, (size_t)RC * (SC_MAXCH + 1) * WLX_MAX_CAND, true));
@@ -904,8 +909,15 @@
         p.xsrc = xsrc; p.slab = s.slab; p.slab_stride = s.slab_rows * d;
         return p;
     };
+    VocabTail vtail{};
+    if (with_logits && s->tail_now) {
+        vtail.spp = s->d_sp; vtail.suppress_mask = s->d_suppress;
+        vtail.rule = s->st.rule; vtail.pos = s->st.pos; vtail.plen = s->st.plen; vtail.item_done = s->st.item_done; vtail.nsp_row = s->st.nsp_row;
+        vtail.stats = s->st.tail_stats; vtail.wlog = s->st.tail_wlog; vtail.R = R;
+    }
     auto vocab_params = [&](int xsrc) {
         GemvParams p{};
+        p.tail = (with_logits && s->tail_now) ? &vtail : nullptr;
         p.in_mode = GEMV_IN_LN; p.out_mode = GEMV_OUT_F32; p.M = rows; p.K = d; p.KT = d / 32; p.N = sp.vocab;
         p.Wp = e->Wvocab; p.bias = nullptr; p.X = s.xd; p.ldx = d; p.gamma = e->dec_ln_g; p.beta = e->dec_ln_b;
         p.Y = s->logits; p.ldy = s->ldl; p.qscale = 1.f; p.done = done;
@@ -1070,7 +1082,13 @@
     return WLX_OK;
 }
 
+static bool search_tail_fused(const Engine* e, const Slot* s, int rows, int R, int groups, bool sampling) {
+    if (sampling || g_decode_v1 || g_search_tail.load(std::memory_order_relaxed) == 0) return false;
+    if (rows > 16 || rows != R * groups || R > WLX_TAIL_MAX_BEAM || !s->sp_plain) return false;
+    return dec_vocab_tail_ok(rows, e->spec.d_model, e->spec.vocab);
+}
 static void launch_search(Engine* e, Slot* s, int rows, int R, int groups, bool sampling) {
+    if (s->tail_now) { launch_search_merge_tail(s->logits, s->ldl, e->spec.vocab, s->d_sp, groups, R, s->st, s->stream); return; }
     if (sampling || g_decode_v1) {
         launch_search_rows(s->logits, s->d_sp, rows, s->st, s->stream);
         launch_search_update(s->d_sp, groups, s->st, s->stream);
@@ -1080,6 +1098,13 @@
     }
 }
 
+static void step_launches(Engine* e, Slot* s, int rows, int R, int groups, bool sampling, bool with_search = true) {
+    s->tail_now = search_tail_fused(e, s, rows, R, groups, sampling);
+    decoder_pass(e, s, rows, R, groups, true, true);
+    if (with_search) launch_search(e, s, rows, R, groups, sampling);
+    s->tail_now = false;
+}
+
 static int graph_steps_for(const Slot* s, int rows) {
     static const int env = [] { const char* v = wlx_ab("WLX_GRAPH_STEPS"); const int n = v ? atoi(v) : 2; return (n == 1 || n == 2) ? n : 2; }();
     if (env == 1 || rows > 16) return 1;
@@ -1089,17 +1114,15 @@
 
 static int get_step_graph(Engine* e, Slot* s, int rows, int R, int groups, bool sampling, int nsteps, hipGraphExec_t* out) {
     s->busy_variant = device_is_busy(s);
-    StepGraphKey key{rows, R, groups * 8 + (nsteps == 2 ? 4 : 0) + (s->busy_variant ? 2 : 0) + (sampling ? 1 : 0)};
+    const bool tail = search_tail_fused(e, s, rows, R, groups, sampling);
+    StepGraphKey key{rows, R, groups * 16 + (tail ? 8 : 0) + (nsteps == 2 ? 4 : 0) + (s->busy_variant ? 2 : 0) + (sampling ? 1 : 0)};
     auto it = s->graphs.find(key);
     if (it != s->graphs.end()) { *out = it->second; return WLX_OK; }
     hipGraph_t graph;
-    decoder_pass(e, s, rows, R, groups, true, true);
+    step_launches(e, s, rows, R, groups, sampling, false);
     CK(hipGetLastError());
     CK(hipStreamBeginCapture(s->stream, hipStreamCaptureModeThreadLocal));
-    for (int k = 0; k < nsteps; ++k) {
-        decoder_pass(e, s, rows, R, groups, true, true);
-        launch_search(e, s, rows, R, groups, sampling);
-    }
+    for (int k = 0; k < nsteps; ++k) step_launches(e, s, rows, R, groups, sampling);
     const hipError_t ce = hipStreamEndCapture(s->stream, &graph);
     if (ce != hipSuccess) {
         (void)hipGetLastError();
@@ -1128,12 +1151,10 @@
         CK(hipGraphLaunch(exec, s->stream));
     } else {
         s->busy_variant = device_is_busy(s);
-        for (int k = 0; k < nsteps; ++k) {
-            decoder_pass(e, s, rows, R, groups, true, true);
-            launch_search(e, s, rows, R, groups, sampling);
-        }
+        for (int k = 0; k < nsteps; ++k) step_launches(e, s, rows, R, groups, sampling);
         CK(hipGetLastError());
     }
+    if (search_tail_fused(e, s, rows, R, groups, sampling)) g_tail_steps.fetch_add(nsteps, std::memory_order_relaxed);
     return WLX_OK;
 }
 
@@ -1233,6 +1254,7 @@
     unsigned char* h_res = s->h_gen + ((hg - s->h_gen + 63) / 64) * 64;
     static_assert(sizeof(SearchParams) <= 4096, "SearchParams staging");
     CKR(fill_search_params(e, s, batch, R, o, apply_ts, h_sp));
+    s->sp_plain = h_sp->rep_penalty == 1.0f && h_sp->no_repeat_ngram <= 0;
     CK(hipMemcpyAsync(s->d_sp, h_sp, sizeof(SearchParams), hipMemcpyHostToDevice, st));
     launch_search_reset(S, batch, rows, st);
     std::vector<int> nsp(rows, 0), pl(batch);
@@ -1657,6 +1679,14 @@
     return WLX_OK;
 }
 
+extern "C" int32_t wlx_debug_search_tail(int32_t mode, int32_t* mode_before_out, int64_t* fused_steps_out) {
+    if (mode > 1) return set_error(WLX_ERR_ARG, "mode: 0, 1 or negative");
+    if (mode_before_out) *mode_before_out = g_search_tail.load();
+    if (mode >= 0) g_search_tail.store(mode);
+    if (fused_steps_out) *fused_steps_out = g_tail_steps.load();
+    return WLX_OK;
+}
+
 extern "C" int32_t wlx_debug_time_decode_step(wlx_engine* e, int32_t slot, int32_t rows, int32_t t, int32_t iters,
                                               float* avg_ms_out) {
     SlotGuard sg_;
@@ -1736,8 +1766,8 @@
     { const int seq0 = g_trace_seq; unsigned long long* b0 = g_trace_buf; g_trace_buf = nullptr;
       decoder_pass(e, s, rows, tR, tG, true, true); g_trace_seq = seq0; g_trace_buf = b0; }
     CK(hipStreamBeginCapture(st, hipStreamCaptureModeThreadLocal));
-    decoder_pass(e, s, rows, tR, tG, true, true);
-    if (with_search) launch_search(e, s, rows, tR, tG, false);
+    if (with_search) step_launches(e, s, rows, tR, tG, false);
+    else decoder_pass(e, s, rows, tR, tG, true, true);
     CK(hipStreamEndCapture(st, &graph));
     CK(hipGraphInstantiate(&exec, graph, nullptr, nullptr, 0));
     CK(hipGraphDestroy(graph));
diff --git a/whisperlive_amd/csrc/search.hip b/whisperlive_amd/csrc/search.hip
--- a/whisperlive_amd/csrc/search.hip
+++ b/whisperlive_amd/csrc/search.hip
@@ -561,32 +561,13 @@
     }
     const float raw_local = raw_m;
 
-    const bool ts = sp.apply_ts_rules != 0;
-    const bool last_was_ts = ts && rule.x != 0;
-    const bool penult_was_ts = ts && rule.y != 0;
-    int ts_last = -1;
-    if (ts && rule.z >= 0) ts_last = (last_was_ts && !penult_was_ts) ? rule.z : rule.z + 1;
-    const bool first = (ngen == 0);
-    const int last_allowed = (sp.max_initial_ts >= 0) ? sp.ts_begin + sp.max_initial_ts : 0x7fffffff;
+    const SearchRule q = search_rule_of(sp, rule, ngen);
     float w[SC_NPT];
 #pragma unroll
     for (int i = 0; i < SC_NPT; ++i) {
         const int id = id0 + i * SC_THREADS + tid;
         bool kill = id >= lim;
-        if (!kill) kill = (sp.suppress_mask[id >> 5] >> (id & 31)) & 1u;
-        if (first && sp.suppress_blank && (id == sp.blank || id == sp.eot)) kill = true;
-        if (ts) {
-            if (id == sp.no_timestamps) kill = true;
-            if (last_was_ts) {
-                if (penult_was_ts) { if (id >= sp.ts_begin) kill = true; }
-                else if (id < sp.eot) kill = true;
-            }
-            if (id >= sp.ts_begin && id < ts_last) kill = true;
-            if (first) {
-                if (id < sp.ts_begin) kill = true;
-                if (id > last_allowed) kill = true;
-            }
-        }
+        if (!kill) kill = search_rule_kills(sp, q, id, sp.suppress_mask[id >> 5]);
         w[i] = kill ? WLX_NEG_INF : v[i];
     }
 
@@ -688,6 +669,34 @@
 }
 
 #define MU3_THREADS 384
+#define MT_CAPB 16
+#define MT_CAP4 128
+static_assert(MT_CAPB >= 2 * WLX_TAIL_MAX_BEAM, "one fetched block per candidate");
+__device__ __noinline__ void tail_rounds_slow(const float* __restrict__ wrow, const int* sel, int nsel, int ncand, int V, int id_min,
+                                              float base, int eot, float* out_s, int* out_t) {
+    const int lane = threadIdx.x & 63;
+    float pv = __builtin_inff(); int pi = -1;
+    for (int k = 0; k < ncand; ++k) {
+        float bv = WLX_NEG_INF; int bi = 0x7fffffff;
+        for (int u = 0; u < nsel; ++u) {
+            const int n = sel[u] * WLX_TAIL_BLK + 4 * lane;
+            const float4 x = *reinterpret_cast<const float4*>(wrow + n);
+            const float xs[4] = {x.x, x.y, x.z, x.w};
+#pragma unroll
+            for (int j = 0; j < 4; ++j) {
+                const int id = n + j; const float v = xs[j];
+                const bool ok = id < V && id >= id_min && v > WLX_NEG_INF && (v < pv || (v == pv && id > pi));
+                if (ok && (v > bv || (v == bv && id < bi))) { bv = v; bi = id; }
+            }
+        }
+        s3_wave_argmax(bv, bi);
+        if (lane == 0) { out_s[k] = (bi < V) ? bv + base : WLX_NEG_INF; out_t[k] = (bi < V) ? bi : eot; }
+        pv = bv; pi = bi;
+        if (bi == 0x7fffffff) pv = WLX_NEG_INF;
+    }
+}
+
+template <bool TAIL>
 __global__ __launch_bounds__(MU3_THREADS) void search_merge_update3_kernel(const float* __restrict__ logits, long ldl, int V,
                                                                            const SearchParams* __restrict__ spp, SearchState st, int R WLX_TR_PARAM) {
     const int item = blockIdx.x;
@@ -703,13 +712,26 @@
     const int n_hyp0 = st.n_hyp[item];
     const int rp = r0 + (wave < R ? wave : R - 1);
     const int lc = lane < SC_MAXCH ? lane : SC_MAXCH - 1;
-    const float4* pso = reinterpret_cast<const float4*>(st.scan_stats + ((long)rp * SC_MAXCH + lc) * SC_NSTAT);
-    const float4 ps0 = pso[0], ps1 = pso[1];
-    const float4* pcv = reinterpret_cast<const float4*>(st.scan_cv + ((long)rp * (SC_MAXCH + 1) + lc) * WLX_MAX_CAND);
-    const int4* pci = reinterpret_cast<const int4*>(st.scan_ci + ((long)rp * (SC_MAXCH + 1) + lc) * WLX_MAX_CAND);
+    float4 ps0 = make_float4(0.f, 0.f, 0.f, 0.f), ps1 = ps0;
     float4 pa[PQ]; int4 pb[PQ];
-#pragma unroll
-    for (int k = 0; k < PQ; ++k) { pa[k] = pcv[k]; pb[k] = pci[k]; }
+    float pt[TAIL ? WLX_TAIL_NSTAT : 1][4];
+    const int nb = ((((V + 15) >> 4) + 1) / 2 + 7) / 8;
+    if constexpr (TAIL) {
+#pragma unroll
+        for (int sidx = 0; sidx < WLX_TAIL_NSTAT; ++sidx)
+#pragma unroll
+            for (int qd = 0; qd < 4; ++qd) {
+                const int j = lane + 64 * qd;
+                pt[sidx][qd] = st.tail_stats[((long)rp * WLX_TAIL_NSTAT + sidx) * WLX_TAIL_MAXBLK + (j < nb ? j : nb - 1)];
+            }
+    } else {
+        const float4* pso = reinterpret_cast<const float4*>(st.scan_stats + ((long)rp * SC_MAXCH + lc) * SC_NSTAT);
+        ps0 = pso[0]; ps1 = pso[1];
+        const float4* pcv = reinterpret_cast<const float4*>(st.scan_cv + ((long)rp * (SC_MAXCH + 1) + lc) * WLX_MAX_CAND);
+        const int4* pci = reinterpret_cast<const int4*>(st.scan_ci + ((long)rp * (SC_MAXCH + 1) + lc) * WLX_MAX_CAND);
+#pragma unroll
+        for (int k = 0; k < PQ; ++k) { pa[k] = pcv[k]; pb[k] = pci[k]; }
+    }
     const float pcum = st.cum[rp];
     const int pnsp = st.nsp_row[rp];
     const SearchParams sp = *spp;
@@ -742,6 +764,146 @@
 
     const bool ts = sp.apply_ts_rules != 0;
     const int nc4 = (sp.ncand + 3) >> 2;
+    if constexpr (TAIL) {
+    __shared__ float4 l4v[NW][MT_CAP4];
+    __shared__ int l4i[NW][MT_CAP4];
+    __shared__ int sel_s[NW][MT_CAPB];
+    const int ncand_t = sp.ncand < MT_CAPB ? sp.ncand : MT_CAPB;
+#pragma unroll 1
+    for (int rb = wave; rb < sp.beam; rb += NW) {
+        const int r = r0 + rb;
+        float bs[WLX_TAIL_NSTAT][4];
+        float cum_r; int nsp_r;
+        if (rb == wave) {
+#pragma unroll
+            for (int sidx = 0; sidx < WLX_TAIL_NSTAT; ++sidx)
+#pragma unroll
+                for (int qd = 0; qd < 4; ++qd) bs[sidx][qd] = pt[sidx][qd];
+            cum_r = pcum; nsp_r = pnsp;
+        } else {
+#pragma unroll
+            for (int sidx = 0; sidx < WLX_TAIL_NSTAT; ++sidx)
+#pragma unroll
+                for (int qd = 0; qd < 4; ++qd) {
+                    const int j = lane + 64 * qd;
+                    bs[sidx][qd] = st.tail_stats[((long)r * WLX_TAIL_NSTAT + sidx) * WLX_TAIL_MAXBLK + (j < nb ? j : nb - 1)];
+                }
+            cum_r = st.cum[r]; nsp_r = st.nsp_row[r];
+        }
+#pragma unroll
+        for (int qd = 0; qd < 4; ++qd)
+            if (lane + 64 * qd >= nb) { bs[0][qd] = WLX_NEG_INF; bs[1][qd] = 0.f; bs[2][qd] = WLX_NEG_INF; bs[3][qd] = 0.f; bs[4][qd] = WLX_NEG_INF; bs[5][qd] = 0.f; }
+        float lmt = WLX_NEG_INF, lmts = WLX_NEG_INF, lrm = WLX_NEG_INF;
+#pragma unroll
+        for (int qd = 0; qd < 4; ++qd) { lmt = fmaxf(lmt, bs[0][qd]); lmts = fmaxf(lmts, bs[2][qd]); lrm = fmaxf(lrm, bs[4][qd]); }
+        const float Mtext = s3_wave_max(lmt), Mts = s3_wave_max(lmts);
+        if (nsp_r > 0) {
+            const float RM = s3_wave_max(lrm);
+            float a = 0.f;
+#pragma unroll
+            for (int qd = 0; qd < 4; ++qd) a += (bs[4][qd] > WLX_NEG_INF) ? bs[5][qd] * __expf(bs[4][qd] - RM) : 0.f;
+            const float RS = s3_wave_sum(a);
+            if (lane == 0) st.no_speech[item] = __expf(logits[(long)r * ldl + sp.no_speech] - RM) / RS;
+        }
+        float a_ts = 0.f;
+#pragma unroll
+        for (int qd = 0; qd < 4; ++qd) a_ts += (bs[2][qd] > WLX_NEG_INF) ? bs[3][qd] * __expf(bs[2][qd] - Mts) : 0.f;
+        const float S_ts = s3_wave_sum(a_ts);
+        const float lse_ts = (Mts > WLX_NEG_INF) ? Mts + __logf(S_ts) : WLX_NEG_INF;
+        const bool text_masked = ts && (lse_ts > Mtext);
+        float lse_sel;
+        if (text_masked) {
+            lse_sel = lse_ts;
+        } else {
+            const float mx_all = fmaxf(Mtext, Mts);
+            float a = 0.f;
+#pragma unroll
+            for (int qd = 0; qd < 4; ++qd)
+                a += ((bs[0][qd] > WLX_NEG_INF) ? bs[1][qd] * __expf(bs[0][qd] - mx_all) : 0.f) +
+                     ((bs[2][qd] > WLX_NEG_INF) ? bs[3][qd] * __expf(bs[2][qd] - mx_all) : 0.f);
+            lse_sel = mx_all + __logf(s3_wave_sum(a));
+        }
+        const float base = cum_r - lse_sel;
+        const int id_min = text_masked ? sp.ts_begin : 0;
+        float bm[4];
+#pragma unroll
+        for (int qd = 0; qd < 4; ++qd) bm[qd] = text_masked ? bs[2][qd] : fmaxf(bs[0][qd], bs[2][qd]);
+        int nsel = 0; float T = WLX_NEG_INF;
+#pragma unroll 1
+        for (int k = 0; k < ncand_t; ++k) {
+            float gv = bm[0]; int gj = lane;
+#pragma unroll
+            for (int qd = 1; qd < 4; ++qd) if (bm[qd] > gv) { gv = bm[qd]; gj = lane + 64 * qd; }
+            s3_wave_argmax(gv, gj);
+            if (!(gv > WLX_NEG_INF)) break;
+            if (lane == 0) sel_s[wave][k] = gj;
+            T = gv; nsel = k + 1;
+#pragma unroll
+            for (int qd = 0; qd < 4; ++qd) if (lane + 64 * qd == gj) bm[qd] = WLX_NEG_INF;
+        }
+        if (nsel < ncand_t) T = WLX_NEG_INF;
+        const float* wrow = st.tail_wlog + (long)r * WLX_TAIL_LD;
+        float4 t4[MT_CAPB]; int tn[MT_CAPB];
+#pragma unroll
+        for (int u = 0; u < MT_CAPB; ++u) {
+            tn[u] = sel_s[wave][u < nsel ? u : 0] * WLX_TAIL_BLK + 4 * lane;
+            if (u < nsel) t4[u] = *reinterpret_cast<const float4*>(wrow + tn[u]);
+        }
+        int n4 = 0;
+#pragma unroll
+        for (int u = 0; u < MT_CAPB; ++u) {
+            if (u < nsel) {
+                const float m4 = fmaxf(fmaxf(t4[u].x, t4[u].y), fmaxf(t4[u].z, t4[u].w));
+                const bool keep = m4 >= T && m4 > WLX_NEG_INF;
+                const unsigned long long km = __ballot(keep);
+                if (km) {
+                    const int at = n4 + __builtin_popcountll(km & ((1ull << lane) - 1ull));
+                    if (keep && at < MT_CAP4) { l4v[wave][at] = t4[u]; l4i[wave][at] = tn[u]; }
+                    n4 += __builtin_popcountll(km);
+                }
+            }
+        }
+        if (n4 > MT_CAP4) {
+            tail_rounds_slow(wrow, sel_s[wave], nsel, ncand_t, V, id_min, base, sp.eot, cand_s[rb], cand_t[rb]);
+        } else {
+            float xv[8]; int xi[8];
+#pragma unroll
+            for (int h = 0; h < 2; ++h) {
+                const int e = lane + 64 * h;
+                const bool have = e < n4;
+                const float4 x = l4v[wave][have ? e : 0];
+                const int n = l4i[wave][have ? e : 0];
+                const float xs[4] = {x.x, x.y, x.z, x.w};
+#pragma unroll
+                for (int j = 0; j < 4; ++j) {
+                    const int id = n + j;
+                    const bool ok = have && id < V && id >= id_min && xs[j] >= T && xs[j] > WLX_NEG_INF;
+                    xv[4 * h + j] = ok ? xs[j] : WLX_NEG_INF; xi[4 * h + j] = ok ? id : 0x7fffffff;
+                }
+            }
+            float bv = WLX_NEG_INF; int bi = 0x7fffffff;
+#pragma unroll
+            for (int i = 0; i < 8; ++i) if (xv[i] > bv || (xv[i] == bv && xi[i] < bi)) { bv = xv[i]; bi = xi[i]; }
+#pragma unroll 1
+            for (int k = 0; k < ncand_t; ++k) {
+                float gv = bv; int gi = bi;
+                s3_wave_argmax(gv, gi);
+                if (lane == 0) {
+                    cand_s[rb][k] = (gi < V) ? gv + base : WLX_NEG_INF;
+                    cand_t[rb][k] = (gi < V) ? gi : sp.eot;
+                }
+                if (gi != 0x7fffffff && bi == gi) {
+                    bv = WLX_NEG_INF; bi = 0x7fffffff;
+#pragma unroll
+                    for (int i = 0; i < 8; ++i) {
+                        if (xi[i] == gi) { xv[i] = WLX_NEG_INF; xi[i] = 0x7fffffff; }
+                        if (xv[i] > bv || (xv[i] == bv && xi[i] < bi)) { bv = xv[i]; bi = xi[i]; }
+                    }
+                }
+            }
+        }
+    }
+    } else {
 #pragma unroll 1
     for (int rb = wave; rb < sp.beam; rb += NW) {
         const int r = r0 + rb;
@@ -815,6 +977,7 @@
                 hi = (hp < sp.ncand) ? li[wave][lane][hp] : 0x7fffffff;
             }
         }
+    }
     }
     __syncthreads();
     WLX_TR_MARK(1);
@@ -920,7 +1083,11 @@
 
 void launch_search_merge_update3(const float* logits, long ldl, int V, const SearchParams* sp_dev, int items, int R,
                                  const SearchState& st, hipStream_t s) {
-    hipLaunchKernelGGL(search_merge_update3_kernel, dim3(items), dim3(MU3_THREADS), 0, s, logits, ldl, V, sp_dev, st, R WLX_TR_ARG("search_merge_update3"));
+    hipLaunchKernelGGL(search_merge_update3_kernel<false>, dim3(items), dim3(MU3_THREADS), 0, s, logits, ldl, V, sp_dev, st, R WLX_TR_ARG("search_merge_update3"));
+}
+void launch_search_merge_tail(const float* logits, long ldl, int V, const SearchParams* sp_dev, int items, int R,
+                              const SearchState& st, hipStream_t s) {
+    hipLaunchKernelGGL(search_merge_update3_kernel<true>, dim3(items), dim3(MU3_THREADS), 0, s, logits, ldl, V, sp_dev, st, R WLX_TR_ARG("search_merge_tail"));
 }
 
 __global__ __launch_bounds__(256) void search_reset_kernel(SearchState st, int items, int rows) {
```
